# whatshap/whatshap

Hardware: AMD Instinct MI355X
Metric: variant-columns/sec at max-coverage 20 (bipartition-costs/sec reported alongside) (higher is better)
Workload: dtype u32; 1 GPU; synthetic diploid single-individual, max-coverage 20: 1 block of 200000 SNVs (BASELINE configs[2]); blocks=1, blocks_in_flight_per_gpu=1, tables_per_launch=1, max_coverage=20, optimal_cost_checksum=1611545, rendezvous=none

## Files before the change

include/whatshap_amd_debug.h:

```cpp
#ifndef WHATSHAP_AMD_DEBUG_H
#define WHATSHAP_AMD_DEBUG_H

#include "whatshap_amd.h"

#ifdef __cplusplus
extern "C" {
#endif

whamd_status_t whamd_debug_emulate_slot_plan(const whamd_readset_view* readset, const uint32_t* recombcost, size_t n_recombcost,
                                            const whamd_pedigree_view* pedigree, int distrust_genotypes,
                                            const uint32_t* positions, size_t n_positions, int slot_l, int symmetry,
                                            uint32_t* index_out, uint32_t* score_out, uint64_t* n_run_columns_out);

whamd_status_t whamd_debug_emulate_pedslot_plan(const whamd_readset_view* readset, const uint32_t* recombcost, size_t n_recombcost,
                                               const whamd_pedigree_view* pedigree, int distrust_genotypes,
                                               const uint32_t* positions, size_t n_positions, int slot_l,
                                               uint32_t* index_out, uint32_t* transmission_out, uint32_t* score_out,
                                               uint64_t* n_run_columns_out);

whamd_status_t whamd_debug_lazy_terms_check(const whamd_readset_view* readset, const uint32_t* recombcost, size_t n_recombcost,
                                            const whamd_pedigree_view* pedigree, int distrust_genotypes,
                                            const uint32_t* positions, size_t n_positions, const uint8_t* need, int rounds,
                                            int* lazy_out, uint64_t* differences_out, uint64_t* built_before_out, uint64_t* built_after_out);

whamd_status_t whamd_debug_pedmec_heuristic_create_host(const whamd_readset_view* readset, const uint32_t* recombcost, size_t n_recombcost,
                                                        const whamd_pedigree_view* pedigree, int distrust_genotypes,
                                                        const uint32_t* positions, size_t n_positions, uint32_t row_limit, int allow_mutations,
                                                        whamd_heuristic** out);

whamd_status_t whamd_debug_realign_detect_host(const whamd_realign_alignments_view* alignments, const whamd_realign_variants_view* variants,
                                               const whamd_realign_reference_view* reference, const whamd_realign_params* params,
                                               whamd_realign** out);
whamd_status_t whamd_debug_edit_distance_host(uint64_t n_pairs, const uint64_t* query_ptr, const uint8_t* query, const uint64_t* target_ptr,
                                              const uint8_t* target, int use_affine, const float* mismatch_cost, int32_t gap_start,
                                              int32_t gap_extend, int64_t* distance_out);

whamd_status_t whamd_debug_poly_score_host(const whamd_poly_matrix_view* matrices, uint64_t n_matrices, uint32_t min_overlap, uint32_t ploidy,
                                           double err, whamd_poly_scores** out);

whamd_status_t whamd_debug_progeny_score_host(const whamd_progeny_view* problems, uint64_t n_problems, whamd_progeny_scores** out);
whamd_status_t whamd_debug_progeny_score_entries_host(const whamd_progeny_view* problem, uint64_t n_entries, const uint32_t* i, const uint32_t* j,
                                                      double* score_out, uint8_t* stored_out);
whamd_status_t whamd_debug_progeny_pair_score_host(const float* gl, uint64_t n_positions, uint32_t n_samples, uint32_t ploidy, uint64_t pos1,
                                                   uint64_t pos2, uint32_t kind, double* score_out);
whamd_status_t whamd_debug_progeny_variant_types_host(const float* gl, uint64_t n_positions, uint32_t n_samples, uint32_t ploidy, const double* priors,
                                                      const uint32_t* nodes, uint64_t n_nodes, double* llh_out, uint32_t* g0_out, uint32_t* g1_out);
whamd_status_t whamd_debug_progeny_gl_host(const whamd_progeny_depths_view* problems, uint64_t n_problems, float* const* table_out,
                                           double* const* table_f64_out);

whamd_status_t whamd_debug_haplotag_host(const whamd_haplotag_view* problems, uint64_t n_problems, whamd_haplotag_result** out);

typedef struct whamd_debug_kernel {
	const void* kernel;
	const char* name;
	int32_t large_lds_opted_in;
	int32_t debug_only;
} whamd_debug_kernel;
size_t whamd_debug_solve_kernels(whamd_debug_kernel* out, size_t capacity);

enum {
	WHAMD_LAUNCH_COLUMN = 0,
	WHAMD_LAUNCH_RUN = 1,
	WHAMD_LAUNCH_SLOT_RUN = 2,
	WHAMD_LAUNCH_BATCH = 3,
	WHAMD_LAUNCH_GROUP = 4,
	WHAMD_LAUNCH_GROUP_WALK = 5,
	WHAMD_LAUNCH_TAIL = 6,
	WHAMD_LAUNCH_WINDOW_WALK = 7,
	WHAMD_LAUNCH_TABLES = 8
};

typedef struct whamd_debug_launch {
	const void* kernel;
	uint32_t site;
	uint32_t grid_x, grid_y, block;
	uint32_t lds;
	uint32_t own_stream;
	uint32_t forward;
	int32_t lr, yflags, spec, stamps, tb, nf, ncols, threads;
	int32_t streamed, pack;
	int32_t tight, variant;
	int32_t T, n_ind, mode, wide;
	int32_t ped, sym;
	int32_t entries;
	int32_t preview;
	int32_t reserved;
	uint64_t count;
	const char* name;
} whamd_debug_launch;
whamd_status_t whamd_debug_dptable_launches(const whamd_dptable* table, whamd_debug_launch* out, size_t capacity, size_t* n_out);

typedef struct whamd_debug_preview {
	int32_t ran, continued;
	uint32_t pieces, launched_steps, agreed_steps, reserved;
	const char* why_not;
} whamd_debug_preview;
whamd_status_t whamd_debug_dptable_preview(const whamd_dptable* table, whamd_debug_preview* out);

typedef struct whamd_debug_preview_plan_result {
	uint32_t n_pieces, pieces, steps, n_steps;
	int32_t chunked_predicted, chunked, windowed, reserved;
	uint32_t n_seeds_predicted, n_seeds, stride_predicted, stride;
	uint64_t arena_predicted, arena_laid_out, exchange_predicted, exchange_laid_out;
	const char* why_not;
} whamd_debug_preview_plan_result;
whamd_status_t whamd_debug_preview_plan(const whamd_readset_view* readset, const uint32_t* recombcost, size_t n_recombcost,
                                        const whamd_pedigree_view* pedigree, int distrust_genotypes,
                                        const uint32_t* positions, size_t n_positions, uint32_t pieces, whamd_debug_preview_plan_result* out,
                                        uint64_t* rec_predicted, uint64_t* rec_laid_out, uint32_t* spec_predicted, uint32_t* spec_laid_out, size_t capacity);

typedef struct whamd_debug_genotype_run {
	uint32_t c0, ncols;
	uint32_t rescale_f, rescale_b, emit_f, emit_b;
	uint32_t n_part_out, part_out_f, part_out_b;
	uint32_t part_in_f, n_part_in_f, part_in_b, n_part_in_b;
	uint32_t reserved;
} whamd_debug_genotype_run;
whamd_status_t whamd_debug_genotype_run_plan(const whamd_readset_view* readset, const uint32_t* recombcost, size_t n_recombcost,
                                             const whamd_pedigree_view* pedigree, const uint32_t* positions, size_t n_positions,
                                             whamd_debug_genotype_run* out, size_t capacity, size_t* n_out, double* min_total_out);

#ifdef __cplusplus
}
#endif

#endif
```

whatshap_amd/_native.py:

```python

from __future__ import annotations

import ctypes as C
import os
import threading
from typing import Optional, Sequence

import numpy as np

_HERE = os.path.dirname(os.path.abspath(__file__))
LIB_PATH = os.path.join(_HERE, "libwhatshap_amd.so")
DEBUG_LIB_PATH = os.path.join(_HERE, "libwhatshap_amd_debug.so")
ABI_VERSION = 2

WHAMD_OK = 0
WHAMD_ERR_INVALID = 1
WHAMD_ERR_MENDELIAN_CONFLICT = 2
WHAMD_ERR_UNSORTED = 3
WHAMD_ERR_UNSUPPORTED = 4
WHAMD_ERR_DEVICE = 5
WHAMD_ERR_OVERFLOW = 6
WHAMD_ERR_HOST = 7
GT_OTHER = 255

# ... 584 lines not shown
        else:
            _check(L.whamd_dptable_create(*problem.call_args(), C.c_int(device), C.byref(self._h)))
        self.n_columns = int(L.whamd_dptable_column_count(self._h))
        self.n_individuals = int(L.whamd_dptable_individual_count(self._h))
        self.n_reads = int(L.whamd_dptable_read_count(self._h))
        if solve:
            self.solve()

    def set_option(self, key: str, value: str):
        _check(self._L.whamd_dptable_set_option(self._h, key.encode(), value.encode()))

    def solve(self):
        _check(self._L.whamd_dptable_solve(self._h))

    def enqueue(self):
        _check(self._L.whamd_dptable_enqueue(self._h))

    def wait(self):
        _check(self._L.whamd_dptable_wait(self._h))

    def release_device(self):
        _check(self._L.whamd_dptable_release_device(self._h))

    def close(self):
        if getattr(self, "_h", None) is not None and self._h:
            self._L.whamd_dptable_destroy(self._h)
            self._h = C.c_void_p()

    def __del__(self):
        try:
            self.close()
        except Exception:
            pass

    def positions(self) -> np.ndarray:
        out = np.zeros(self.n_columns, dtype=np.uint32)
        _check(self._L.whamd_dptable_positions(self._h, _ptr(out, C.c_uint32)))
        return out

    def optimal_score(self) -> int:
        v = C.c_uint32()
        _check(self._L.whamd_dptable_get_optimal_score(self._h, C.byref(v)))
        return int(v.value)

    def super_reads(self):
        n, ni = self.n_columns, self.n_individuals
        a0 = np.zeros((ni, n), dtype=np.uint8)
        a1 = np.zeros((ni, n), dtype=np.uint8)
        q = np.zeros((ni, n), dtype=np.uint32)
        tv = np.zeros(n, dtype=np.uint32)
        sid = np.zeros(ni, dtype=np.uint32)
        _check(self._L.whamd_dptable_get_super_reads(
            self._h, _ptr(a0, C.c_uint8), _ptr(a1, C.c_uint8), _ptr(q, C.c_uint32), _ptr(tv, C.c_uint32), _ptr(sid, C.c_uint32)))
        return a0, a1, q, tv, sid

    def partitioning(self) -> np.ndarray:
        out = np.zeros(self.n_reads, dtype=np.uint8)
        _check(self._L.whamd_dptable_get_optimal_partitioning(self._h, _ptr(out, C.c_uint8)))
        return out

    def index_path(self):
        idx = np.zeros(self.n_columns, dtype=np.uint32)
        tv = np.zeros(self.n_columns, dtype=np.uint32)
        _check(self._L.whamd_dptable_get_index_path(self._h, _ptr(idx, C.c_uint32), _ptr(tv, C.c_uint32)))
        return idx, tv

    def stats(self) -> dict:
        s = SolveStats()
        _check(self._L.whamd_dptable_get_stats(self._h, C.byref(s)))
        return s.as_dict()


def plan_summary(problem: ProblemArrays, path: str = "auto") -> dict:
    out = PlanSummary()
    _check(lib().whamd_plan_summarize(*problem.call_args(), path.encode(), C.byref(out)))
    return out.as_dict()


def emulate_slot_plan(problem: ProblemArrays, n_columns: int, slot_l: int = 11, symmetry: int = 1, slot_r: int = 2):
    if slot_r >= 3:
        slot_l += 100
    elif slot_r <= 1:
        slot_l += 200
    idx = np.zeros(max(n_columns, 1), dtype=np.uint32)
    score = C.c_uint32()
    ncols = C.c_uint64()
    D = debug_lib()
    _check(D.whamd_debug_emulate_slot_plan(*problem.call_args(), C.c_int(slot_l), C.c_int(symmetry), _ptr(idx, C.c_uint32),
                                           C.byref(score), C.byref(ncols)), D)
    return idx[:n_columns], int(score.value), int(ncols.value)


def emulate_pedslot_plan(problem: ProblemArrays, n_columns: int, slot_l: int = 0):
    idx = np.zeros(max(n_columns, 1), dtype=np.uint32)
    trans = np.zeros(max(n_columns, 1), dtype=np.uint32)
    score = C.c_uint32()
    ncols = C.c_uint64()
    D = debug_lib()
    _check(D.whamd_debug_emulate_pedslot_plan(*problem.call_args(), C.c_int(slot_l), _ptr(idx, C.c_uint32), _ptr(trans, C.c_uint32),
                                              C.byref(score), C.byref(ncols)), D)
    return idx[:n_columns], trans[:n_columns], int(score.value), int(ncols.value)


def debug_lazy_terms_check(problem: ProblemArrays, need=None, rounds: int = 1) -> dict:
    D = debug_lib()
    fn = D.whamd_debug_lazy_terms_check
    fn.restype = C.c_int
    lazy, diff, before, after = C.c_int(), C.c_uint64(), C.c_uint64(), C.c_uint64()
    need_arr = None if need is None else np.ascontiguousarray(need, dtype=np.uint8)
    _check(fn(*problem.call_args(), None if need_arr is None else _ptr(need_arr, C.c_uint8), C.c_int(int(rounds)), C.byref(lazy), C.byref(diff),
              C.byref(before), C.byref(after)), D)
    return {"lazy": bool(lazy.value), "differences": int(diff.value), "built_before": int(before.value), "built_after": int(after.value)}


class DebugGenotypeRun(C.Structure):
    _fields_ = [(name, C.c_uint32) for name in ("c0", "ncols", "rescale_f", "rescale_b", "emit_f", "emit_b", "n_part_out", "part_out_f", "part_out_b",
                                                "part_in_f", "n_part_in_f", "part_in_b", "n_part_in_b", "reserved")]


def debug_genotype_run_plan(problem: ProblemArrays):
    D = debug_lib()
    fn = D.whamd_debug_genotype_run_plan
    fn.restype = C.c_int
    a = problem.call_args()
    args = (a[0], a[1], a[2], a[3], a[5], a[6])
    n, min_total = C.c_size_t(), C.c_double()
    status = fn(*args, None, C.c_size_t(0), C.byref(n), C.byref(min_total))
    if status == WHAMD_ERR_UNSUPPORTED:
        return None
    _check(status, D)
    runs = (DebugGenotypeRun * max(n.value, 1))()
    _check(fn(*args, runs, C.c_size_t(n.value), C.byref(n), C.byref(min_total)), D)
    names = [f[0] for f in DebugGenotypeRun._fields_ if f[0] != "reserved"]
    return [{k: int(getattr(runs[i], k)) for k in names} for i in range(n.value)], float(min_total.value)


class DebugKernel(C.Structure):
    _fields_ = [("kernel", C.c_void_p), ("name", C.c_char_p), ("large_lds_opted_in", C.c_int32), ("debug_only", C.c_int32)]


LAUNCH_SITES = ("column", "run", "slot_run", "batch", "group", "group_walk", "tail", "window_walk", "tables")
LAUNCH_FACTS = ("lr", "yflags", "spec", "stamps", "tb", "nf", "ncols", "threads", "streamed", "pack", "tight", "variant", "T", "n_ind", "mode", "wide",
                "ped", "sym", "entries")


class DebugLaunch(C.Structure):
    _fields_ = ([("kernel", C.c_void_p), ("site", C.c_uint32), ("grid_x", C.c_uint32), ("grid_y", C.c_uint32), ("block", C.c_uint32), ("lds", C.c_uint32),
                 ("own_stream", C.c_uint32), ("forward", C.c_uint32)] + [(f, C.c_int32) for f in LAUNCH_FACTS] +
                [("preview", C.c_int32), ("reserved", C.c_int32), ("count", C.c_uint64), ("name", C.c_char_p)])


class DebugPreview(C.Structure):
    _fields_ = [("ran", C.c_int32), ("continued", C.c_int32), ("pieces", C.c_uint32), ("launched_steps", C.c_uint32), ("agreed_steps", C.c_uint32),
                ("reserved", C.c_uint32), ("why_not", C.c_char_p)]


def debug_preview(table) -> dict:
    D = debug_lib()
    if table._L is not D:
        raise ValueError("the preview's record exists in the debug library only (use_debug_library() before the table is made)")
    out = DebugPreview()
    _check(D.whamd_debug_dptable_preview(table._h, C.byref(out)), D)
    return {"ran": bool(out.ran), "continued": bool(out.continued), "pieces": int(out.pieces), "launched_steps": int(out.launched_steps),
            "agreed_steps": int(out.agreed_steps), "why_not": (out.why_not or b"").decode()}


class DebugPreviewPlan(C.Structure):
    _fields_ = [("n_pieces", C.c_uint32), ("pieces", C.c_uint32), ("steps", C.c_uint32), ("n_steps", C.c_uint32),
                ("chunked_predicted", C.c_int32), ("chunked", C.c_int32), ("windowed", C.c_int32), ("reserved", C.c_int32),
                ("n_seeds_predicted", C.c_uint32), ("n_seeds", C.c_uint32), ("stride_predicted", C.c_uint32), ("stride", C.c_uint32),
                ("arena_predicted", C.c_uint64), ("arena_laid_out", C.c_uint64), ("exchange_predicted", C.c_uint64), ("exchange_laid_out", C.c_uint64),
                ("why_not", C.c_char_p)]


def debug_preview_plan(problem: ProblemArrays, pieces: int = 0) -> dict:
    D = debug_lib()
    fn = D.whamd_debug_preview_plan
    fn.restype = C.c_int
    out = DebugPreviewPlan()
    _check(fn(*problem.call_args(), C.c_uint32(pieces), C.byref(out), None, None, None, None, C.c_size_t(0)), D)
    n = int(out.steps)
    arrays = {"rec_predicted": np.zeros(max(n, 1), dtype=np.uint64), "rec_laid_out": np.zeros(max(n, 1), dtype=np.uint64),
              "spec_predicted": np.zeros(max(n, 1), dtype=np.uint32), "spec_laid_out": np.zeros(max(n, 1), dtype=np.uint32)}
    _check(fn(*problem.call_args(), C.c_uint32(pieces), C.byref(out), _ptr(arrays["rec_predicted"], C.c_uint64), _ptr(arrays["rec_laid_out"], C.c_uint64),
              _ptr(arrays["spec_predicted"], C.c_uint32), _ptr(arrays["spec_laid_out"], C.c_uint32), C.c_size_t(n)), D)
    rec = {name: (getattr(out, name).decode() if name == "why_not" else int(getattr(out, name))) for name, _ in DebugPreviewPlan._fields_ if name != "reserved"}
    rec.update({k: v[:n] for k, v in arrays.items()})
    return rec


def debug_solve_kernels() -> list:
    D = debug_lib()
    n = D.whamd_debug_solve_kernels(None, 0)
    arr = (DebugKernel * n)()
    D.whamd_debug_solve_kernels(arr, n)
    return [{"kernel": k.kernel, "name": k.name.decode(), "large_lds_opted_in": bool(k.large_lds_opted_in), "debug_only": bool(k.debug_only)} for k in arr]


def debug_launches(table) -> list:
    D = debug_lib()
    if table._L is not D:
        raise ValueError("the launch ledger exists in the debug library only (use_debug_library() before the table is made)")
    n = C.c_size_t()
    _check(D.whamd_debug_dptable_launches(table._h, None, 0, C.byref(n)), D)
    arr = (DebugLaunch * max(n.value, 1))()
    _check(D.whamd_debug_dptable_launches(table._h, arr, n.value, C.byref(n)), D)
    out = []
    for r in arr[:n.value]:
        if r.name is None:
            raise RuntimeError(f"a launch of site {LAUNCH_SITES[r.site]} (grid {r.grid_x} x {r.grid_y}, block {r.block}) took a kernel the registry does not list")
        rec = {"name": r.name.decode(), "site": LAUNCH_SITES[r.site], "grid_x": r.grid_x, "grid_y": r.grid_y, "block": r.block, "lds": r.lds,
               "own_stream": bool(r.own_stream), "forward": bool(r.forward), "count": int(r.count), "preview": bool(r.preview)}
        rec.update({f: (None if getattr(r, f) < 0 else getattr(r, f)) for f in LAUNCH_FACTS})
        out.append(rec)
    return out


def _heuristic_result(L, h) -> dict:
    n = int(L.whamd_pedmec_heuristic_column_count(h))
    ns = int(L.whamd_pedmec_heuristic_sample_count(h))
    nr = int(L.whamd_pedmec_heuristic_read_count(h))
    score = C.c_float()
    bip = np.zeros(max(nr, 1), dtype=np.uint8)
    trans = np.zeros(max(n, 1), dtype=np.uint32)
    haps = np.zeros((max(ns, 1), 2, max(n, 1)), dtype=np.int8)
    mut = np.zeros((max(ns, 1), 2, max(n, 1)), dtype=np.uint8)
    sid = np.zeros(max(ns, 1), dtype=np.uint32)
    pos = np.zeros(max(n, 1), dtype=np.uint32)
    _check(L.whamd_pedmec_heuristic_get(h, C.byref(score), _ptr(bip, C.c_uint8), _ptr(trans, C.c_uint32), haps.ctypes.data_as(C.POINTER(C.c_int8)),
                                        _ptr(mut, C.c_uint8), _ptr(sid, C.c_uint32), _ptr(pos, C.c_uint32)), L)
    stats = HeuristicStats()
    _check(L.whamd_pedmec_heuristic_get_stats(h, C.byref(stats)), L)
    return {"score": float(score.value), "bipartition": bip[:nr], "transmission": trans[:n], "haplotypes": haps[:ns, :, :n], "mutated": mut[:ns, :, :n],
            "sample_ids": sid[:ns], "positions": pos[:n], "stats": stats.as_dict()}


def pedmec_heuristic(problem: ProblemArrays, row_limit: int = 256, allow_mutations: bool = True, device: int = 0, host_diagnostic: bool = False) -> dict:
    L = debug_lib() if host_diagnostic else lib()
    h = C.c_void_p()
    a = problem.call_args()
    if host_diagnostic:
        _check(L.whamd_debug_pedmec_heuristic_create_host(*a, C.c_uint32(int(row_limit)), C.c_int(1 if allow_mutations else 0), C.byref(h)), L)
    else:
        _check(L.whamd_pedmec_heuristic_create(*a, C.c_uint32(int(row_limit)), C.c_int(1 if allow_mutations else 0), C.c_int(int(device)), C.byref(h)))
    try:
        return _heuristic_result(L, h)
    finally:
        L.whamd_pedmec_heuristic_destroy(h)


class HeuristicBatch:

    def __init__(self, problems, row_limit: int = 256, allow_mutations: bool = True, device: int = 0):
        L = lib()
        problems = list(problems)
        self._L = L
        self._n = len(problems)
        self._handles = (C.c_void_p * max(self._n, 1))()
        jobs = (HeuristicJob * max(self._n, 1))()
        for i, p in enumerate(problems):
            jobs[i].readset = C.pointer(p.readset_view)
            jobs[i].recombcost = _ptr(p.recombcost, C.c_uint32)
            jobs[i].n_recombcost = p.recombcost.size
            jobs[i].pedigree = C.pointer(p.pedigree_view)
            jobs[i].distrust_genotypes = 1 if p.distrust_genotypes else 0
            jobs[i].positions = _ptr(p.positions, C.c_uint32)
            jobs[i].n_positions = 0 if p.positions is None else p.positions.size
            jobs[i].row_limit = int(row_limit)
            jobs[i].allow_mutations = 1 if allow_mutations else 0
        if self._n:
            _check(L.whamd_pedmec_heuristic_enqueue_many(jobs, self._n, C.c_int(int(device)), self._handles))

    def results(self):
        out = []
        try:
            for i in range(self._n):
                _check(self._L.whamd_pedmec_heuristic_wait(self._handles[i]))
                out.append(_heuristic_result(self._L, self._handles[i]))
        finally:
            self.close()
        return out

    def close(self):
        for i in range(self._n):
            if self._handles[i]:
                self._L.whamd_pedmec_heuristic_destroy(self._handles[i])
                self._handles[i] = None
        self._n = 0

    def __del__(self):
        try:
            self.close()
        except Exception:
            pass


def pedmec_heuristic_many(problems, row_limit: int = 256, allow_mutations: bool = True, device: int = 0):
    return HeuristicBatch(problems, row_limit, allow_mutations, device).results()


def host_pool_idle_bytes() -> int:
    fn = lib().whamd_host_pool_idle_bytes
    fn.restype = C.c_uint64
    return int(fn())


def device_count() -> int:
    return int(lib().whamd_device_count())


def device_pci_bus_id(device: int) -> str:
    buf = C.create_string_buffer(64)
    fn = lib().whamd_device_pci_bus_id
    fn.restype = C.c_int
    fn.argtypes = [C.c_int, C.c_char_p, C.c_size_t]
    _check(fn(int(device), buf, 64))
    return buf.value.decode()
# ... 45 lines not shown
```

whatshap_amd/csrc/c_api.cpp:

```cpp
#include <cstdio>
#include <cstdlib>
#include <cstring>
#include <functional>
#include <memory>
#include <new>
#include <stdexcept>
#include <string>

#include "api_guard.h"
#include "debug_build.h"
#ifdef WHAMD_DEBUG_BUILD
#include "../../include/whatshap_amd_debug.h"
#endif
#include "device_runtime.h"
#include "device_table.h"
#include "genotype.h"
#include "genotype_plan.h"
#include "heuristic.h"
#include "host_parallel.h"
#include "problem.h"
#include "resident.h"
#include "slots.h"
#include <algorithm>
#include <vector>
// ... 608 lines not shown
			const uint32_t lmax = sg.kind == 1 ? (uint32_t)PED_LMAX : (uint32_t)RES_LMAX;
			ok = ok && rc.Lb <= lmax && rc.Lf <= lmax && rc.ebits <= (uint32_t)RES_EMAX;
			ok = ok && rc.stage_off == stage;
			stage += sg.kind == 1 ? (uint64_t)rc.nwords : (uint64_t)rc.ebits * rc.nwords;
			if (rc.mode == RES_MODE_FOLDED) { s.n_folded_columns++; ok = ok && i + 1 < sg.ncols && rc.ebits == 0; }
			if (rc.mode != RES_MODE_GENERIC) s.n_vectorised_columns++;
			if (rc.nfold) ok = ok && rc.nfold <= RES_MAXFOLD && i >= rc.nfold;
			ok = ok && c + 1 < p.n_cols;
		}
		ok = ok && stage == sg.stage_words;
		const uint64_t lds = sg.kind == 1
			? (((uint64_t)sg.ncols * (PED_LDSWORDS + PED_TABLE) + (uint64_t)sg.n_terms * 2 + 3) & ~3ull) * 4 + 2 * (16ull << sg.max_l) + (uint64_t)sg.stage_words * 8
			: (uint64_t)sg.ncols * (64 + RES_TABLE) * 4 + 2 * (4ull << sg.max_l) + (uint64_t)sg.stage_words * 8;
		ok = ok && lds <= 160 * 1024;
		s.max_lds_bytes = std::max<uint64_t>(s.max_lds_bytes, lds);
		s.max_run_columns = std::max<uint64_t>(s.max_run_columns, sg.ncols);
		s.max_workgroups = std::max<uint64_t>(s.max_workgroups, 1ull << (sg.g - sg.half));
		if (sg.half) s.n_halved_runs++;
		s.n_resident_columns += sg.ncols;
		s.backtrace_bytes += (uint64_t)sg.stage_words * (1ull << sg.g) * 8;
	}
	ok = ok && expect == p.n_cols;
	for (uint32_t c = 0; c < p.n_cols; ++c) ok = ok && seen[c] == 1;
	s.invariants_ok = ok ? 1 : 0;
	*out = s;
	return WHAMD_OK;
	});
}

#ifdef WHAMD_DEBUG_BUILD
whamd_status_t whamd_debug_emulate_slot_plan(const whamd_readset_view* readset, const uint32_t* recombcost, size_t n_recombcost,
                                            const whamd_pedigree_view* pedigree, int distrust_genotypes, const uint32_t* positions,
                                            size_t n_positions, int slot_l, int symmetry, uint32_t* index_out, uint32_t* score_out,
                                            uint64_t* n_run_columns_out) {
	return guarded([&]() -> whamd_status_t {
	const int lr = slot_l >= 200 ? 1 : slot_l >= 100 ? 3 : 2;
	if (slot_l >= 100) slot_l -= slot_l >= 200 ? 200 : 100;
	Problem p;
	std::string msg;
	whamd_status_t st = build_problem(readset, recombcost, n_recombcost, pedigree, distrust_genotypes != 0, positions,
	                                  n_positions, p, msg);
	if (st != WHAMD_OK) return fail(st, msg);
	SlotPlan sp;
	if (p.T != 1 || !plan_forward_slots(p, slot_l, symmetry, sp, lr)) return fail(WHAMD_ERR_UNSUPPORTED, "slot runs apply to a single individual only");
	std::vector<uint32_t> path;
	uint32_t score = 0;
	if (!emulate_slot_plan(p, sp, path, score, msg)) return fail(WHAMD_ERR_INVALID, "slot plan inconsistent: " + msg);
	if (index_out && !path.empty()) std::memcpy(index_out, path.data(), path.size() * sizeof(uint32_t));
	if (score_out) *score_out = score;
	if (n_run_columns_out) *n_run_columns_out = sp.n_run_columns;
	return WHAMD_OK;
	});
}

whamd_status_t whamd_debug_emulate_pedslot_plan(const whamd_readset_view* readset, const uint32_t* recombcost, size_t n_recombcost,
                                               const whamd_pedigree_view* pedigree, int distrust_genotypes, const uint32_t* positions,
                                               size_t n_positions, int slot_l, uint32_t* index_out, uint32_t* transmission_out,
                                               uint32_t* score_out, uint64_t* n_run_columns_out) {
	return guarded([&]() -> whamd_status_t {
	Problem p;
	std::string msg;
	whamd_status_t st = build_problem(readset, recombcost, n_recombcost, pedigree, distrust_genotypes != 0, positions,
	                                  n_positions, p, msg);
	if (st != WHAMD_OK) return fail(st, msg);
	SlotPlan sp;
	if (p.T == 1 || !plan_forward_slots(p, slot_l > 0 ? -slot_l : 0, 0, sp) || !sp.ped)
		return fail(WHAMD_ERR_UNSUPPORTED, "pedigree slot runs apply to tables with one or two trios whose columns need at most 4 cost forms per transmission value");
	std::vector<uint32_t> path, trans;
	uint32_t score = 0;
	if (!emulate_pedslot_plan(p, sp, path, trans, score, msg)) return fail(WHAMD_ERR_INVALID, "pedigree slot plan inconsistent: " + msg);
	if (index_out && !path.empty()) std::memcpy(index_out, path.data(), path.size() * sizeof(uint32_t));
	if (transmission_out && !trans.empty()) std::memcpy(transmission_out, trans.data(), trans.size() * sizeof(uint32_t));
	if (score_out) *score_out = score;
	if (n_run_columns_out) *n_run_columns_out = sp.n_run_columns;
	return WHAMD_OK;
	});
}
whamd_status_t whamd_debug_lazy_terms_check(const whamd_readset_view* readset, const uint32_t* recombcost, size_t n_recombcost,
                                            const whamd_pedigree_view* pedigree, int distrust_genotypes, const uint32_t* positions, size_t n_positions,
                                            const uint8_t* need_in, int rounds, int* lazy_out, uint64_t* differences_out, uint64_t* built_before_out,
                                            uint64_t* built_after_out) {
	return guarded([&]() -> whamd_status_t {
	Problem eager, lazy;
	std::string msg;
	whamd_status_t st = build_problem(readset, recombcost, n_recombcost, pedigree, distrust_genotypes != 0, positions, n_positions, eager, msg);
	if (st != WHAMD_OK) return fail(st, msg);
	st = build_problem(readset, recombcost, n_recombcost, pedigree, distrust_genotypes != 0, positions, n_positions, lazy, msg, false, true);
	if (st != WHAMD_OK) return fail(st, msg);
	if (lazy_out) *lazy_out = lazy.lazy_terms ? 1 : 0;
	const uint32_t n = eager.n_cols;
	uint64_t before = 0, after = 0, diff = 0;
	for (uint32_t c = 0; c < n; ++c) before += lazy.term_end(c, lazy.T - 1) > lazy.term_begin(c, 0);
	std::vector<uint8_t> need(n, 1);
	if (need_in) for (uint32_t c = 0; c < n; ++c) need[c] = need_in[c] != 0;
	rounds = std::max(1, rounds);
	for (int r = 0; r < rounds; ++r) {
		std::vector<uint8_t> part(n, 0);
		for (uint32_t c = 0; c < n; ++c) part[c] = need[c] && (int)(c % (uint32_t)rounds) == r;
		st = fill_lazy_terms(lazy, part, msg);
		if (st != WHAMD_OK) return fail(st, msg);
	}
	for (uint32_t c = 0; c < n; ++c) {
		after += lazy.term_end(c, lazy.T - 1) > lazy.term_begin(c, 0);
		if (!need[c]) continue;
		bool same = true;
		for (uint32_t t = 0; t < eager.T && same; ++t) {
			const uint64_t a0 = eager.term_begin(c, t), a1 = eager.term_end(c, t), b0 = lazy.term_begin(c, t), b1 = lazy.term_end(c, t);
			same = a1 - a0 == b1 - b0;
			for (uint64_t i = 0; same && i < a1 - a0; ++i)
				same = eager.terms[a0 + i].c == lazy.terms[b0 + i].c && eager.terms[a0 + i].plus == lazy.terms[b0 + i].plus && eager.terms[a0 + i].minus == lazy.terms[b0 + i].minus;
		}
		diff += !same;
	}
	if (eager.fterm_kind != lazy.fterm_kind || eager.fterms.size() != lazy.fterms.size()) diff += n;
	else for (size_t i = 0; i < eager.fterms.size(); ++i) if (eager.fterms[i].c != lazy.fterms[i].c || eager.fterms[i].plus != lazy.fterms[i].plus || eager.fterms[i].minus != lazy.fterms[i].minus) { ++diff; break; }
	if (lazy.value_bound < eager.value_bound) diff += n;
	if (differences_out) *differences_out = diff;
	if (built_before_out) *built_before_out = before;
	if (built_after_out) *built_after_out = after;
	return WHAMD_OK;
	});
}

size_t whamd_debug_solve_kernels(whamd_debug_kernel* out, size_t capacity) { return DeviceTable::debug_solve_kernels(out, capacity); }

whamd_status_t whamd_debug_dptable_launches(const whamd_dptable* table, whamd_debug_launch* out, size_t capacity, size_t* n_out) {
	if (!table || !n_out) return fail(WHAMD_ERR_INVALID, "null argument");
	if (!table->solved) return fail(WHAMD_ERR_INVALID, "the table has not been solved: its ledger is read after whamd_dptable_wait");
	*n_out = table->device.debug_launches(out, capacity);
	return WHAMD_OK;
}

whamd_status_t whamd_debug_dptable_preview(const whamd_dptable* table, whamd_debug_preview* out) {
	if (!table || !out) return fail(WHAMD_ERR_INVALID, "null argument");
	table->device.debug_preview(out);
	return WHAMD_OK;
}

whamd_status_t whamd_debug_preview_plan(const whamd_readset_view* readset, const uint32_t* recombcost, size_t n_recombcost,
                                        const whamd_pedigree_view* pedigree, int distrust_genotypes,
                                        const uint32_t* positions, size_t n_positions, uint32_t pieces, whamd_debug_preview_plan_result* out,
                                        uint64_t* rec_predicted, uint64_t* rec_laid_out, uint32_t* spec_predicted, uint32_t* spec_laid_out, size_t capacity) {
	return guarded([&]() -> whamd_status_t {
	if (!out) return fail(WHAMD_ERR_INVALID, "out is NULL");
	Problem p;
	std::string msg;
	whamd_status_t st = build_problem(readset, recombcost, n_recombcost, pedigree, distrust_genotypes != 0, positions, n_positions, p, msg);
	if (st != WHAMD_OK) return fail(st, msg);
	st = DeviceTable::debug_preview_plan(p, pieces, out, rec_predicted, rec_laid_out, spec_predicted, spec_laid_out, capacity, msg);
	return st == WHAMD_OK ? WHAMD_OK : fail(st, msg);
	});
}

whamd_status_t whamd_debug_genotype_run_plan(const whamd_readset_view* readset, const uint32_t* recombcost, size_t n_recombcost,
                                             const whamd_pedigree_view* pedigree, const uint32_t* positions, size_t n_positions,
                                             whamd_debug_genotype_run* out, size_t capacity, size_t* n_out, double* min_total_out) {
	return guarded([&]() -> whamd_status_t {
	if (!n_out) return fail(WHAMD_ERR_INVALID, "n_out is NULL");
	Problem p;
	std::string msg;
	whamd_status_t st = build_problem(readset, recombcost, n_recombcost, pedigree, false, positions, n_positions, p, msg, true);
	if (st != WHAMD_OK) return fail(st, msg);
	GenotypeModel model;
	st = build_genotype_model(p, model, msg);
	if (st != WHAMD_OK) return fail(st, msg);
	GenoRunPlan pl;
	if (!geno_plan_runs(p, model, 0, pl)) return fail(WHAMD_ERR_UNSUPPORTED, "the table is not eligible for the genotyper's run path");
	*n_out = pl.runs.size();
	if (min_total_out) *min_total_out = GS_MIN_TOTAL;
	for (size_t ri = 0; out && ri < pl.runs.size() && ri < capacity; ++ri) {
		const GsRun& r = pl.runs[ri];
		whamd_debug_genotype_run o{};
		o.c0 = r.c0; o.ncols = r.ncols;
		o.rescale_f = r.n_part_in_f ? 1u : 0u; o.rescale_b = r.n_part_in_b ? 1u : 0u;
		o.emit_f = r.emit_f; o.emit_b = r.emit_b;
		o.n_part_out = 1u << r.g;
		o.part_out_f = r.part_out_f; o.part_out_b = r.part_out_b;
		o.part_in_f = r.part_in_f; o.n_part_in_f = r.n_part_in_f;
		o.part_in_b = r.part_in_b; o.n_part_in_b = r.n_part_in_b;
		out[ri] = o;
	}
	return WHAMD_OK;
	});
}
#endif

}

struct whamd_heuristic;
struct HeuristicBatchState {
	whamd::HeurBatch batch;
	std::vector<whamd_heuristic*> members;
	bool collected = false;
	whamd_status_t status = WHAMD_OK;
	std::string message;
	double t_enqueued = 0.0;
};

struct whamd_heuristic {
	whamd::HeurPlan plan;
	whamd::HeurResult result;
	whamd_heuristic_stats stats{};
	std::shared_ptr<HeuristicBatchState> batch;
	bool finished = false;
};

namespace {
whamd_status_t heuristic_collect(whamd_heuristic* h) {
	if (h->finished) return WHAMD_OK;
	if (!h->batch) return fail(WHAMD_ERR_INVALID, "whamd_pedmec_heuristic_enqueue has not run");
	std::shared_ptr<HeuristicBatchState> st = h->batch;
	if (!st->collected) {
		st->collected = true;
		std::vector<whamd::HeurResult> results(st->members.size());
		st->status = st->batch.wait(results.data(), st->message);
		if (st->status == WHAMD_OK) {
			const double t_done = now_ms();
			whamd::parallel_ranges(st->members.size(), whamd::host_threads(st->members.size(), 1), [&](uint64_t i0, uint64_t i1, uint32_t) {
				for (uint64_t i = i0; i < i1; ++i) {
					whamd_heuristic* m = st->members[i];
					const double t0 = now_ms();
					m->result = std::move(results[i]);
					whamd::heuristic_finish(m->plan, m->result);
					m->stats.max_solutions = m->result.max_solutions;
					m->stats.total_solutions = m->result.total_solutions;
					m->stats.device_ms = m->result.device_ms;
					m->stats.host_prepare_ms += std::max(0.0, (t_done - st->t_enqueued) - m->result.device_ms);
					m->stats.host_finish_ms = now_ms() - t0;
				}
			});
		}
		for (whamd_heuristic* m : st->members) { m->finished = st->status == WHAMD_OK; m->batch.reset(); }
	}
	if (st->status != WHAMD_OK) return fail(st->status, st->message);
	return WHAMD_OK;
}

whamd_status_t heuristic_enqueue_jobs(const whamd_heuristic_job* jobs, size_t n_jobs, int device, whamd_heuristic** out) {
	if (!out || (!jobs && n_jobs)) return fail(WHAMD_ERR_INVALID, "null argument");
	for (size_t i = 0; i < n_jobs; ++i) out[i] = nullptr;
	std::vector<std::unique_ptr<whamd_heuristic>> hs(n_jobs);
	std::vector<whamd_status_t> status(n_jobs, WHAMD_OK);
	std::vector<std::string> messages(n_jobs);
	std::vector<double> prepare_ms(n_jobs, 0.0);
	whamd::parallel_ranges(n_jobs, whamd::host_threads(n_jobs, 1), [&](uint64_t i0, uint64_t i1, uint32_t) {
		for (uint64_t i = i0; i < i1; ++i) {
			const double t0 = now_ms();
			hs[i].reset(new whamd_heuristic());
			const whamd_heuristic_job& j = jobs[i];
			status[i] = whamd::build_heuristic_plan(j.readset, j.recombcost, j.n_recombcost, j.pedigree, j.distrust_genotypes != 0, j.positions, j.n_positions,
			                                        j.row_limit, j.allow_mutations != 0, hs[i]->plan, messages[i]);
			prepare_ms[i] = now_ms() - t0;
		}
	});
	for (size_t i = 0; i < n_jobs; ++i) if (status[i] != WHAMD_OK) return fail(status[i], messages[i]);
	std::shared_ptr<HeuristicBatchState> st(new HeuristicBatchState());
	std::vector<const whamd::HeurPlan*> plans(n_jobs);
	for (size_t i = 0; i < n_jobs; ++i) plans[i] = &hs[i]->plan;
	std::string msg;
	st->t_enqueued = now_ms();
	const whamd_status_t es = st->batch.enqueue(plans.data(), n_jobs, device, msg);
	if (es != WHAMD_OK) return fail(es, msg);
	for (size_t i = 0; i < n_jobs; ++i) {
		whamd_heuristic* h = hs[i].get();
		h->stats.n_columns = h->plan.n_cols; h->stats.n_reads = h->plan.n_reads; h->stats.n_samples = h->plan.n_samples; h->stats.row_limit = h->plan.row_limit;
		h->stats.host_prepare_ms = prepare_ms[i];
		h->batch = st;
		st->members.push_back(h);
	}
	for (size_t i = 0; i < n_jobs; ++i) out[i] = hs[i].release();
	return WHAMD_OK;
}

whamd_status_t heuristic_create_common(const whamd_readset_view* readset, const uint32_t* recombcost, size_t n_recombcost, const whamd_pedigree_view* pedigree,
                                       int distrust_genotypes, const uint32_t* positions, size_t n_positions, uint32_t row_limit, int allow_mutations,
                                       int device, bool on_host, whamd_heuristic** out) {
	if (!out) return fail(WHAMD_ERR_INVALID, "out is NULL");
	*out = nullptr;
	if (!on_host) {
		whamd_heuristic_job job{readset, recombcost, n_recombcost, pedigree, distrust_genotypes, positions, n_positions, row_limit, allow_mutations};
		whamd_heuristic* h = nullptr;
		whamd_status_t st = heuristic_enqueue_jobs(&job, 1, device, &h);
		if (st != WHAMD_OK) return st;
		st = heuristic_collect(h);
		if (st != WHAMD_OK) { delete h; return st; }
		*out = h;
		return WHAMD_OK;
	}
#ifndef WHAMD_DEBUG_BUILD
	return fail(WHAMD_ERR_DEVICE, "the host instantiation of the heuristic exists in the debug library only");
#else
	const double t0 = now_ms();
	std::unique_ptr<whamd_heuristic> h(new whamd_heuristic());
	std::string msg;
	whamd_status_t st = whamd::build_heuristic_plan(readset, recombcost, n_recombcost, pedigree, distrust_genotypes != 0, positions, n_positions, row_limit,
	                                                allow_mutations != 0, h->plan, msg);
	if (st != WHAMD_OK) return fail(st, msg);
	const double t1 = now_ms();
	st = whamd::heuristic_solve_host(h->plan, h->result, msg);
	if (st != WHAMD_OK) return fail(st, msg);
	const double t2 = now_ms();
	whamd::heuristic_finish(h->plan, h->result);
	h->stats.n_columns = h->plan.n_cols; h->stats.n_reads = h->plan.n_reads; h->stats.max_solutions = h->result.max_solutions;
	h->stats.total_solutions = h->result.total_solutions; h->stats.device_ms = h->result.device_ms;
	h->stats.host_prepare_ms = (t1 - t0) + ((t2 - t1) - h->result.device_ms); h->stats.host_finish_ms = now_ms() - t2;
	h->stats.n_samples = h->plan.n_samples; h->stats.row_limit = h->plan.row_limit;
// ... 119 lines not shown
```

whatshap_amd/csrc/dp_device.hip:

```cpp
#include <hip/hip_runtime.h>

#include <algorithm>
#include <atomic>
#include <cctype>
#include <chrono>
#include <cstdio>
#include <cstdlib>
#include <cstring>
#include <mutex>
#include <string>
#include <vector>

#include "debug_build.h"
#ifdef WHAMD_DEBUG_BUILD
#include "../../include/whatshap_amd_debug.h"
#endif
#include "device_runtime.h"
#include "device_table.h"
#include "genotype.h"

namespace whamd {

namespace {

#include "kernels_column.h"
#include "kernels_resident.h"
#include "kernels_trio.h"
#include "kernels_slots.h"
#include "kernels_pedslots.h"
#include "kernels_backtrace.h"

using FusedFn = void (*)(DevProblem, uint32_t, const uint32_t*, uint32_t*);
using KeysFn = void (*)(DevProblem, uint32_t, const uint32_t*, uint32_t);

template <int T, int NIND>
void pick(FusedFn& ff, KeysFn& kf) {
	ff = column_step_fused<T, NIND>;
	kf = column_step_keys<T, NIND>;
}

bool select_kernels(uint32_t T, uint32_t n_ind, FusedFn& ff, KeysFn& kf) {
	const uint32_t ni = n_ind ? n_ind : 1;
	ff = nullptr;
	kf = nullptr;
#define WHAMD_CASE(TT, NN) if (T == TT && ni == NN) { pick<TT, NN>(ff, kf); return true; }
	WHAMD_CASE(1, 1) WHAMD_CASE(1, 2) WHAMD_CASE(1, 3) WHAMD_CASE(1, 4) WHAMD_CASE(1, 5) WHAMD_CASE(1, 6)
	WHAMD_CASE(4, 3) WHAMD_CASE(4, 4) WHAMD_CASE(4, 5) WHAMD_CASE(4, 6)
	WHAMD_CASE(16, 4) WHAMD_CASE(16, 5) WHAMD_CASE(16, 6)
#undef WHAMD_CASE
	return false;
}

using SegmentFn = void (*)(DevProblem, ResSegment, const uint32_t*, uint32_t*, uint32_t*);
using PedSegmentFn = void (*)(DevProblem, ResSegment, const uint32_t*, uint32_t*);
using ResBatchFn = void (*)(DevProblem, const ResBatchEntry*);
using SlotRunFn = void (*)(DevProblem, SlotRun, const uint32_t*, uint32_t*, uint32_t*);
using SlotRunXFn = void (*)(DevProblem, SlotRun, const uint32_t*, uint32_t*, uint32_t*, uint32_t);
using PedSlotRunFn = void (*)(DevProblem, SlotRun, PedSlotExtra, const uint32_t*, uint32_t*);
using SlotBatchFn = void (*)(DevProblem, const SlotBatchEntry*);
using GroupFn = void (*)(SlotGroupArgs);

enum GroupVariant : uint8_t { GV_SINGLE4 = 0, GV_PED_2_2, GV_PED_2_4, GV_PED_4_2, GV_PED_4_4, GV_PED_2_16, GV_SINGLE8, GV_TRIO_FACT, GV_X4, GV_X8, GV_QUARTET_FACT, GROUP_VARIANTS };
struct GroupVariantPair { GroupVariant plain, x; };

GroupVariantPair group_variants_of(const SlotBatchEntry& he, bool ped) {
	if (ped) {
		const GroupVariant v = he.ex.nf == (uint32_t)PSLOT_FACT4 ? GV_QUARTET_FACT : he.ex.nf == (uint32_t)PSLOT_FACT ? GV_TRIO_FACT : he.ex.nf == 16 ? GV_PED_2_16
		                       : he.ex.tb == 4 ? (he.ex.nf == 4 ? GV_PED_4_4 : GV_PED_4_2) : (he.ex.nf == 4 ? GV_PED_2_4 : GV_PED_2_2);
		return {v, v};
	}
	const GroupVariant v = he.run.lr == 3 ? GV_SINGLE8 : GV_SINGLE4;
	return {v, (he.run.yflags & 8u) ? (he.run.lr == 3 ? GV_X8 : GV_X4) : v};
}

}


namespace {

struct CreateLaps {
	using Clock = std::chrono::steady_clock;
	const bool on = getenv("WHAMD_DEBUG_TIMING") != nullptr;
	Clock::time_point last = Clock::now();
	double stage_ms[4] = {0.0, 0.0, 0.0, 0.0};
	int stage = 0;
	double take() {
		const auto now = Clock::now();
		const double ms = std::chrono::duration<double, std::milli>(now - last).count();
		last = now;
		stage_ms[stage] += ms;
		return ms;
	}
	void lap(const char* what) {
		if (on) fprintf(stderr, "[whamd timing]   upload: %s %.2f ms\n", what, take());
	}
	void next_stage() {
		if (!on) return;
		take();
		if (stage < 3) ++stage;
	}
	void summary(double arena_gb) {
		if (!on) return;
		take();
		fprintf(stderr, "[whamd timing] upload: plan %.1f ms, descriptors + copies %.1f ms, backtrace arena (%.2f GB) %.1f ms, rest %.1f ms\n", stage_ms[0], stage_ms[1], arena_gb, stage_ms[2],
		        stage_ms[3]);
	}
};

struct TableUploader {
	const int device;
	const hipStream_t stream;
	StageSession stage;
	std::vector<std::pair<void*, size_t>>& allocations;
	char* d_slab = nullptr;
	size_t slab_cap = 0, slab_used = 0, slab_flushed = 0;
	bool unstaged_copies = false;

	TableUploader(int dev, hipStream_t us, std::vector<std::pair<void*, size_t>>& table_allocations) : device(dev), stream(us), stage(us), allocations(table_allocations) {}

	hipError_t alloc(void** dptr, size_t bytes) {
		size_t got = 0;
		hipError_t e = devpool_take(device, std::max<size_t>(bytes, 16), dptr, &got);
		if (e == hipSuccess) allocations.emplace_back(*dptr, got);
		return e;
	}
	void open_block(size_t upload_bytes) {
		stage.expect(upload_bytes);
		if (upload_bytes <= STAGE_MAX && !debug_env("WHAMD_NO_UPLOAD_SLAB") && stage.begin_image(upload_bytes)) {
			void* ptr = nullptr;
			if (alloc(&ptr, upload_bytes) == hipSuccess) { d_slab = (char*)ptr; slab_cap = upload_bytes; }
			else { (void)hipGetLastError(); stage.image = false; }
		}
	}
	hipError_t flush() {
		if (!d_slab || slab_used == slab_flushed) return hipSuccess;
		const hipError_t e = debug_env("WHAMD_SKIP_SLAB_COPY") ? hipSuccess : hipMemcpyAsync(d_slab + slab_flushed, stage.base + slab_flushed, slab_used - slab_flushed, hipMemcpyHostToDevice, stream);
		stage.pending = true;
		slab_flushed = slab_used;
		return e;
	}
	hipError_t up(void** dptr, const void* src, size_t bytes) {
		const size_t padded = (bytes + 255) & ~(size_t)255;
		if (d_slab && slab_used + padded <= slab_cap) {
			*dptr = d_slab + slab_used;
			char* at = stage.base + slab_used;
			const char* from = (const char*)src;
			if (bytes >= ((size_t)4 << 20)) parallel_ranges(bytes, host_threads(bytes, (size_t)2 << 20), [at, from](uint64_t b0, uint64_t b1, uint32_t) { std::memcpy(at + b0, from + b0, b1 - b0); });
			else if (bytes) std::memcpy(at, from, bytes);
			slab_used += padded;
			stage.total += padded;
			return slab_used - slab_flushed >= ((size_t)32 << 20) ? flush() : hipSuccess;
		}
		hipError_t e = alloc(dptr, bytes);
		if (e != hipSuccess) return e;
		if (bytes) e = stage.copy(*dptr, src, bytes);
		if (bytes && stage.image) unstaged_copies = true;
		return e;
	}
	hipError_t up_pieces(void** dptr, const void* src, size_t bytes, const std::vector<std::pair<size_t, size_t>>& pieces) {
		const size_t padded = (bytes + 255) & ~(size_t)255;
		const bool in_slab = d_slab && slab_used + padded <= slab_cap;
		if (in_slab) {
			hipError_t e = flush();
			if (e != hipSuccess) return e;
			*dptr = d_slab + slab_used;
			slab_used += padded;
			slab_flushed = slab_used;
		} else {
			hipError_t e = alloc(dptr, bytes);
			if (e != hipSuccess) return e;
		}
		const size_t image_at = slab_used - padded;
		for (const auto& pc : pieces) {
			if (pc.second <= pc.first) continue;
			const char* from = (const char*)src + pc.first;
			if (in_slab) {
				std::memcpy(stage.base + image_at + pc.first, from, pc.second - pc.first);
				from = stage.base + image_at + pc.first;
				stage.pending = true;
			} else {
				unstaged_copies = true;
			}
			hipError_t e = hipMemcpyAsync((char*)*dptr + pc.first, from, pc.second - pc.first, hipMemcpyHostToDevice, stream);
			if (e != hipSuccess) return e;
		}
		return hipSuccess;
	}
};

struct TableBuild {
	CreateLaps laps;
	uint32_t n = 0;
	uint32_t tbits = 0;
	uint32_t ni = 1;
	size_t free_b = 0;
	uint64_t arena_cap = 0;
	uint64_t bt = 0;
	uint32_t max_f = 0, max_keys_f = 0;
	size_t exchange_bytes = 0;
	bool force_keys = false;
	bool ped_slots = false;
	std::vector<uint32_t> segs;
	RawVec<uint32_t> term_ptr32;
	std::vector<uint32_t> window_first_col;
	RawVec<uint32_t> slot_blob;
	std::vector<uint32_t> slot_blob_off, slot_blob_words;
	std::vector<int32_t> delta_fallback;
	const SlotRun* d_runs = nullptr;
	const PedSlotExtra* d_pextra = nullptr;
	const DevTerm* d_fterms = nullptr;
};

}


#ifdef WHAMD_DEBUG_BUILD
struct LaunchFacts : whamd_debug_launch {
	LaunchFacts() {
		std::memset(static_cast<whamd_debug_launch*>(this), 0, sizeof(whamd_debug_launch));
		lr = yflags = spec = stamps = tb = nf = ncols = threads = streamed = pack = tight = variant = T = n_ind = mode = wide = ped = sym = entries = -1;
	}
	static LaunchFacts of_run(const SlotRun& run, bool spec_v, bool stamps_v) {
		LaunchFacts f;
		f.lr = (int32_t)run.lr; f.yflags = (int32_t)run.yflags; f.ncols = (int32_t)run.ncols; f.threads = (int32_t)run.threads;
		f.spec = spec_v; f.stamps = stamps_v;
		return f;
	}
};
#define WHAMD_NOTE(table, ...) (table).note(__VA_ARGS__)
#else
#define WHAMD_NOTE(table, ...) ((void)0)
#endif

struct DeviceTable::Impl {
	int device = 0;
	hipStream_t stream = nullptr;
	hipEvent_t ev0 = nullptr, ev1 = nullptr, ev2 = nullptr, ev3 = nullptr;
	hipEvent_t ev_group = nullptr;
	hipEvent_t ev_upload = nullptr;
	std::vector<std::pair<void*, size_t>> allocations;
	void* d_arena = nullptr;
	size_t arena_bytes = 0;
	DevColumn* d_cols = nullptr;
	uint32_t* d_pr[2] = {nullptr, nullptr};
	uint32_t* d_path_index = nullptr;
	uint32_t* d_path_trans = nullptr;
	uint32_t* d_score = nullptr;
	BtUnit* d_units = nullptr;
	std::vector<BtUnit> units;
	size_t bt_lds = 0;
	RawVec<DevColumn> cols;
	ResidentPlan plan;
	DevProblem dp{};
	FusedFn fused = nullptr;
	KeysFn keysfn = nullptr;
	bool wide = false;
	size_t key_entries = 0;
	std::string path = "auto";
	int l_pref = 11;
	bool fold = true;
	int symmetry = 1;
	uint64_t bt_bytes = 0;
	uint32_t max_grid_x = 1;
	size_t h_pinned_bytes = 0;
	uint32_t* h_pinned = nullptr;
	struct Job {
		std::vector<uint32_t> steps;
		uint32_t unit_off = 0, unit_count = 0;
		bool final = false;
	};
	struct Lane {
		uint32_t* d_pr[2] = {nullptr, nullptr};
		unsigned long long* d_keys = nullptr;
		std::vector<uint32_t> jobs;
	};
	struct Single {
		uint32_t lane, step, flip;
		bool zero_prev;
		int32_t score_job;
	};
	struct SuperStep {
		uint32_t entry_off = 0, entry_count = 0, grid_x = 0, threads = 0;
		size_t lds = 0;
		bool sym = false;
		std::vector<Single> singles;
		int32_t ck_load = -1, ck_save = -1, bt_window = -1;
		uint32_t* io[2] = {nullptr, nullptr};
	};
	std::vector<Job> jobs;
	std::vector<Lane> lanes;
	std::vector<SuperStep> schedule;
	struct StepBrief { uint32_t entry_off, lds; uint16_t entry_count; uint8_t has_singles, pad; };
	struct EntryBrief { uint16_t grid_x, threads; uint32_t lds_x; GroupVariantPair variant; uint8_t pad[2]; };
	std::vector<StepBrief> step_brief;
	std::vector<EntryBrief> entry_brief;
	std::vector<ResBatchEntry> entries;
	ResBatchEntry* d_entries = nullptr;
	bool use_chunks = false;
	std::vector<BtChunk> chunks;
	BtChunk* d_chunks = nullptr;
	uint32_t* d_unit_x = nullptr;
	uint32_t* d_path2 = nullptr;
	uint32_t* d_trans2 = nullptr;
	uint32_t n_orient_max = 1;
	uint8_t* d_sel = nullptr;
	uint32_t* d_guess = nullptr;
	uint32_t* d_bt_counters = nullptr;
	uint32_t n_spec = 0;
	size_t chunk_lds = 0;
	SlotPlan splan;
	bool use_slots = false;
	int slot_l = 11;
	bool slot_l_set = false;
	int slot_lr = 2;
	int slot_lr_used = 2;
	std::vector<SlotBatchEntry> slot_entries;
	SlotBatchEntry* d_slot_entries = nullptr;
	uint64_t table_bytes = 0;
	BtJob* d_btjobs = nullptr;
	uint32_t* d_job_scores = nullptr;
	bool shared_hint = false;
	bool side_by_side = false;
	int max_lanes = 32;
	struct Window {
		uint32_t step_lo = 0, step_hi = 0;
		uint32_t unit_off = 0, unit_count = 0;
	};
	uint64_t arena_limit = 0;
	bool windowed = false;
	std::vector<Window> windows;
	uint8_t* d_checkpoints = nullptr;
	size_t checkpoint_bytes = 0;
	uint32_t* d_bt_state = nullptr;
	BtJob* d_window_jobs = nullptr;

	whamd_status_t open(int dev, std::string& msg);
	whamd_status_t choose_plan(Problem& p, TableBuild& b, std::string& msg);
	void dump_plan(const Problem& p) const;
	whamd_status_t describe_columns(const Problem& p, TableBuild& b, std::string& msg);
	whamd_status_t lay_out_arena(const Problem& p, TableBuild& b, std::string& msg);
	size_t upload_bound(const Problem& p, const TableBuild& b) const;
	whamd_status_t upload_column_arrays(const Problem& p, TableBuild& b, TableUploader& up, std::string& msg);
	void build_slot_blobs(TableBuild& b) const;
	uint64_t lay_out_slot_tables(const TableBuild& b, bool report = true);
	whamd_status_t upload_slot_arrays(TableBuild& b, TableUploader& up, std::string& msg);
	void make_jobs();
	void make_units(const TableBuild& b);
	whamd_status_t make_windows(const TableBuild& b, TableUploader& up, std::string& msg);
	whamd_status_t take_result_block(uint32_t n, TableUploader& up, std::string& msg);
	void cut_chunks(const Problem& p);
	whamd_status_t make_chunks(const Problem& p, TableUploader& up, std::string& msg);
	whamd_status_t take_solve_buffers(const Problem& p, TableBuild& b, TableUploader& up, std::string& msg);
	whamd_status_t make_lanes(const TableBuild& b, TableUploader& up, std::string& msg);
	whamd_status_t make_schedule(const TableBuild& b, std::string& msg);
	void make_briefs();
	whamd_status_t upload_entries(TableUploader& up, std::string& msg);
	whamd_status_t launch_table_kernels(const Problem& p, const TableBuild& b, TableUploader& up, std::string& msg);
	whamd_status_t arm_debug_stamps(TableUploader& up, std::string& msg);
	whamd_status_t record_group_backtrace(uint32_t n, TableUploader& up, std::string& msg);
	struct SolveInFlight {
		hipStream_t run_stream = nullptr;
		uint32_t group_tables = 1;
		bool enqueue_open = false;
		size_t next_super = 0;
		uint64_t launches = 0;
		hipStream_t tail_stream = nullptr;
		uint64_t tail_seq = 0;
		bool tail_elsewhere = false;
		bool timing_pending = false;
		static inline std::atomic<uint64_t> tails_submitted{0};
		void rewind(hipStream_t own) { enqueue_open = false; next_super = 0; run_stream = own; }
	} inflight;
#ifdef WHAMD_DEBUG_BUILD
	std::vector<whamd_debug_launch> ledger;
	void note(uint32_t site, const void* kernel, dim3 grid, dim3 block, size_t lds, hipStream_t on, bool forward, const LaunchFacts& facts);
#endif
	struct GroupSubmission;
	void launch_column_step(const Problem& p, const Step& step, const Lane& lane, const uint32_t* prev, uint32_t* cur, uint64_t& launches);
	void launch_run(const ResBatchEntry& e, uint64_t& launches);
	void launch_slot_run(const DevProblem& dp, const SlotBatchEntry& e, uint64_t& launches);
	whamd_status_t begin_solve(const Problem& p, Solution& s, std::string& msg, bool behind_preview = false);
	whamd_status_t submit_super_step(const Problem& p, const SuperStep& ss, uint64_t& launches, std::string& msg);
	whamd_status_t submit_singles(const Problem& p, const SuperStep& ss, uint64_t& launches, std::string& msg);
	whamd_status_t submit_tail(const Problem& p, std::string& msg, hipStream_t tail_stream = nullptr, bool walked_by_group = false);
	whamd_status_t report_slot_stamps(std::string& msg) const;
	whamd_status_t report_resident_stamps(std::string& msg) const;
	BtGroupEntry h_bt_entry{};
	BtGroupEntry* d_bt_entry = nullptr;
	bool device_superreads = false;
	SuperreadArgs super_args{};
	size_t super_words = 0, super_off = 0;
	bool own_stream_used = false;
	bool upload_pending = false;
	hipStream_t upload_stream = nullptr;

	enum PreviewWhy : uint32_t { PV_RAN = 0, PV_OFF, PV_NOT_CREATE, PV_NOT_SLOTS, PV_DEBUG_SWITCH, PV_SHARED, PV_THREAD_BUDGET, PV_COMPONENTS, PV_FEW_PIECES, PV_NOT_ALONE, PV_NO_LEADING_RUNS,
	                           PV_ROW_PAD, PV_ARENA, PV_WHYS };
	struct Preview {
		int mode = -1;
		uint32_t pieces_wanted = 0;
		bool thread_budget = false;
		bool counted = false;
		uint32_t why = PV_NOT_CREATE;
		uint32_t pieces = 0;
		uint32_t launched = 0;
		uint32_t agreed = 0;
		bool launching = false;
		bool pending = false;
		bool continued = false;
		bool use_chunks = false;
		uint64_t launches = 0;
		std::vector<SlotRun> runs;
		DevProblem dp{};
		uint32_t* d_pr[2] = {nullptr, nullptr};
		size_t exchange_bytes = 0;
		unsigned long long* spec_keys = nullptr;
		size_t spec_bytes = 0;
		std::vector<std::pair<void*, size_t>> allocations;
	} preview;
	static inline std::atomic<int> tables_on_device[64];
	void give_preview_block() {
		for (auto& a : preview.allocations) devpool_give(device, a.first, a.second);
		preview.allocations.clear();
	}
	struct PreviewPlan {
		uint32_t why = PV_NOT_CREATE, pieces = 0, steps = 0, end_col = 0, n_spec = 0, stride = 64, max_f = 0;
		bool chunked = false;
		uint64_t arena = 0, tab_words = 0;
		size_t ctrl_words = 0;
		std::vector<uint64_t> rec;
		std::vector<uint32_t> spec;
	};
	void plan_preview(const Problem& p, const TableBuild& b, bool from_create, PreviewPlan& out);
	whamd_status_t start_preview(const Problem& p, TableBuild& b, bool from_create, std::string& msg);
	void verify_preview();
	whamd_status_t arm_keys(std::string& msg);

	void adopt(const StreamSet& ss) { stream = ss.stream; ev0 = ss.ev[0]; ev1 = ss.ev[1]; ev2 = ss.ev[2]; ev3 = ss.ev[3]; ev_group = ss.ev[4]; ev_upload = ss.ev[5]; }
	StreamSet stream_set() const {
		StreamSet ss;
		ss.stream = stream; ss.ev[0] = ev0; ss.ev[1] = ev1; ss.ev[2] = ev2; ss.ev[3] = ev3; ss.ev[4] = ev_group; ss.ev[5] = ev_upload; ss.device = device;
		return ss;
	}

	void release_lanes() {
		max_grid_x = 1;
		lanes.clear();
		jobs.clear();
		schedule.clear();
		entries.clear();
		slot_entries.clear();
		windows.clear();
	}

	void release() {
		if (inflight.tail_elsewhere && ev3) (void)hipEventSynchronize(ev3);
		inflight.tail_elsewhere = false;
		if (upload_pending && ev_upload) (void)hipEventSynchronize(ev_upload);
		upload_pending = false;
		release_lanes();
		windowed = false;
		if (stream && own_stream_used && (!allocations.empty() || d_arena)) { (void)hipStreamSynchronize(stream); own_stream_used = false; }
		for (auto& a : allocations) devpool_give(device, a.first, a.second);
		allocations.clear();
		give_preview_block();
		if (preview.why != PV_NOT_CREATE) {
			Preview fresh;
			fresh.mode = preview.mode; fresh.pieces_wanted = preview.pieces_wanted; fresh.thread_budget = preview.thread_budget; fresh.counted = preview.counted;
			preview = std::move(fresh);
		}
		arena_give(device, d_arena, arena_bytes);
		d_arena = nullptr;
		arena_bytes = 0;
		pinned_give(h_pinned, h_pinned_bytes);
		h_pinned = nullptr;
		d_cols = nullptr;
		d_units = nullptr;
		d_pr[0] = d_pr[1] = nullptr;
		d_path_index = d_path_trans = d_score = nullptr;
	}
};

DeviceTable::DeviceTable() : impl_(new Impl()) {}

DeviceTable::~DeviceTable() {
	if (impl_) {
		release_device();
		delete impl_;
	}
}

void DeviceTable::release_device() {
	Impl& m = *impl_;
	(void)hipSetDevice(m.device);
	m.release();
	if (m.stream) {
		if (m.own_stream_used) (void)hipStreamSynchronize(m.stream);
		m.own_stream_used = false;
		streamset_give(m.stream_set());
	}
	m.adopt(StreamSet());
	if (m.preview.counted && m.device >= 0 && m.device < 64) Impl::tables_on_device[m.device].fetch_sub(1);
	m.preview.counted = false;
	m.inflight.run_stream = nullptr;
	m.inflight.timing_pending = false;
}

int DeviceTable::device_count() {
	int n = 0;
	if (hipGetDeviceCount(&n) != hipSuccess) return 0;
	return n;
}

bool DeviceTable::device_pci_bus_id(int device, std::string& out) {
	int n = 0;
	if (hipGetDeviceCount(&n) != hipSuccess || device < 0 || device >= n) return false;
	char text[64] = {0};
	if (hipDeviceGetPCIBusId(text, (int)sizeof text - 1, device) != hipSuccess) return false;
	out = text;
	for (char& ch : out) ch = (char)tolower((unsigned char)ch);
	return true;
}

static void append_segments(uint32_t mask, std::vector<uint32_t>& out, uint16_t& count) {
	uint32_t src = 0;
	count = 0;
	for (uint32_t bit = 0; bit < 32;) {
		if (!((mask >> bit) & 1u)) { ++bit; continue; }
		uint32_t len = 0;
		while (bit + len < 32 && ((mask >> (bit + len)) & 1u)) ++len;
		out.push_back(src | (bit << 8) | (len << 16));
		++count;
		src += len;
		bit += len;
	}
}

bool DeviceTable::set_path(const std::string& path) {
	if (path != "auto" && path != "column" && path != "column_keys" && path != "resident" && path != "slots") return false;
	impl_->path = path;
	return true;
}

void DeviceTable::set_l_pref(int l) { impl_->l_pref = std::max(4, std::min(l, RES_LMAX)); }
void DeviceTable::set_lanes(int n) { impl_->max_lanes = n < 1 ? 1 : (n > 64 ? 64 : n); }

void DeviceTable::set_fold(bool v) { impl_->fold = v; }
void DeviceTable::set_slot_l(int l) { impl_->slot_l = std::max(2, std::min(l, 12)); impl_->slot_l_set = true; }
void DeviceTable::set_slot_lr(int lr) { impl_->slot_lr = lr >= 3 ? 3 : (lr <= 1 ? 1 : 2); }

void DeviceTable::set_arena_limit(uint64_t bytes) { impl_->arena_limit = bytes; }
void DeviceTable::set_shared_launches(bool v) { impl_->shared_hint = v; }
void DeviceTable::set_side_by_side(bool v) { impl_->side_by_side = v; }
void DeviceTable::set_preview(int mode) { impl_->preview.mode = mode < 0 ? -1 : (mode ? 1 : 0); }
void DeviceTable::set_preview_pieces(uint32_t pieces) { impl_->preview.pieces_wanted = pieces; }
void DeviceTable::set_thread_budget(bool v) { impl_->preview.thread_budget = v; }
void DeviceTable::set_symmetry(int level) { impl_->symmetry = level < 0 ? 0 : (level > 2 ? 2 : level); }


whamd_status_t DeviceTable::Impl::open(int dev, std::string& msg) {
	Impl& m = *this;
	m.device = dev;
	const whamd_status_t opened = open_device(dev, msg);
	if (opened != WHAMD_OK) return opened;
	if (!m.stream) {
		StreamSet ss;
		if (!streamset_take(dev, ss)) { msg = "could not create the table's stream and events"; return WHAMD_ERR_DEVICE; }
		m.adopt(ss);
	}
	m.release();
	if (!m.preview.counted && dev >= 0 && dev < 64) { Impl::tables_on_device[dev].fetch_add(1); m.preview.counted = true; }
	return WHAMD_OK;
}

whamd_status_t DeviceTable::Impl::choose_plan(Problem& p, TableBuild& b, std::string& msg) {
	Impl& m = *this;
	m.wide = !select_kernels(p.T, p.n_ind, m.fused, m.keysfn);
	if (m.wide && (p.T > (uint32_t)MAX_T_WIDE || p.n_ind > (uint32_t)MAX_IND_WIDE)) {
		msg = "no device kernel for T=" + std::to_string(p.T) + ", individuals=" + std::to_string(p.n_ind);
		return WHAMD_ERR_UNSUPPORTED;
	}
	for (uint32_t c = 0; c < p.n_cols && !m.wide; ++c) m.wide = p.term_end(c, p.T - 1) - p.term_begin(c, 0) > (uint64_t)COL_MAXTERMS;
	b.force_keys = m.path == "column_keys" || m.wide;
	const bool want_resident = (m.path == "auto" || m.path == "resident") && !m.wide;
	size_t free_b = 0, total_b = 0;
	HIP_TRY(hipMemGetInfo(&free_b, &total_b));
	if (free_b < total_b / 2) {
		genotype_release_cache();
		HIP_TRY(hipMemGetInfo(&free_b, &total_b));
	}
	if (free_b < total_b / 4) {
		arena_release();
		devpool_release();
		HIP_TRY(hipMemGetInfo(&free_b, &total_b));
	}
	free_b += arena_idle_bytes(m.device);
	b.free_b = free_b;
	int slot_lr = m.slot_lr, slot_l = m.slot_l;
	if (m.shared_hint && p.T == 1 && p.max_k >= 18 && !m.slot_l_set && m.slot_lr == 2) { slot_lr = 3; slot_l = 12; }
	if (p.T == 1 && p.max_k >= 21 && p.max_k <= 22 && !m.slot_l_set && m.slot_lr == 2 && !debug_env("WHAMD_NO_WIDE_LAYOUT")) { slot_lr = 3; slot_l = 12; }
	m.slot_lr_used = slot_lr;
	m.use_slots = (m.path == "auto" || m.path == "slots") && !m.wide && plan_forward_slots(p, p.T > 1 ? (m.slot_l_set ? -m.slot_l : 0) : std::max(8, slot_l), m.symmetry, m.splan, slot_lr);
	if (m.use_slots && m.splan.ped && m.splan.table_words * 4ull > free_b / 4) m.use_slots = false;
	m.table_bytes = m.use_slots && m.splan.ped ? m.splan.table_words * 4ull : 0ull;
	if (p.lazy_terms) {
		std::vector<uint8_t> need(p.n_cols, 1);
		if (m.use_slots && m.splan.ped) for (uint32_t c = 0; c < p.n_cols; ++c) need[c] = m.splan.col_to_row[c] < 0;
		const whamd_status_t st = fill_lazy_terms(p, need, msg);
		if (st != WHAMD_OK) return st;
	}
	if (m.use_slots) {
		m.plan = ResidentPlan();
		m.plan.steps = m.splan.steps;
		m.plan.component_first_step = m.splan.component_first_step;
		m.plan.col_to_res.assign(p.n_cols, -1);
	} else {
		m.splan = SlotPlan();
		plan_forward(p, want_resident, m.l_pref, m.fold, m.plan, m.symmetry);
	}
	m.device_superreads = p.n_ind == 1 && p.T == 1 && p.P == 2 && !p.distrust && p.h2p.size() >= 2 && p.h2p[0] == 0 && p.h2p[1] == 1 && p.genotype.size() >= p.n_cols &&
	                      !debug_env("WHAMD_HOST_SUPERREADS");
	return WHAMD_OK;
}

void DeviceTable::Impl::dump_plan(const Problem& p) const {
	const Impl& m = *this;
	for (const Step& st : m.plan.steps) {
		if (st.kind == 0) { fprintf(stderr, "[plan] column %u k=%u b=%u f=%u\n", st.index, p.k[st.index], p.b[st.index], p.f[st.index]); continue; }
		if (st.kind == 2) {
			const SlotRun& r = m.splan.runs[st.index];
			fprintf(stderr, "[plan] slot run c0=%u ncols=%u g=%u L=%u half=%u ends=%u has_prev=%u in_identity=%u in_half=%u mirror_pos=%u in_occ=%x out_occ=%x mirror_out=%u\n",
			        r.c0, r.ncols, r.g, r.L, r.half, r.n_ends, r.has_prev, r.in_identity, r.in_half, r.in_mirror_pos, r.in_occ, r.out_occ, r.mirror_out);
			if (m.splan.ped) fprintf(stderr, "[plan]   pedigree run: T=%u forms per value=%u table words=%u record words per workgroup=%u\n", 1u << m.splan.pextra[st.index].tb,
			                         m.splan.pextra[st.index].nf, m.splan.pextra[st.index].s_off + r.ncols * 64u * pslot_ns(m.splan.pextra[st.index].nf), m.splan.pextra[st.index].rec_words);
			continue;
		}
		const ResSegment& sgm = m.plan.segments[st.index];
		fprintf(stderr, "[plan] run c0=%u ncols=%u g=%u threads=%u max_l=%u stage_words=%u\n", sgm.c0, sgm.ncols, sgm.g, sgm.threads, sgm.max_l, sgm.stage_words);
		for (uint32_t i = 0; i < sgm.ncols; ++i) {
			const ResColumn& rc = m.plan.columns[sgm.col_off + i];
			const ResBacktrace& rb = m.plan.backtrace[sgm.col_off + i];
			fprintf(stderr, "[plan]   col %u mode=%u nfold=%u Lb=%u Lf=%u ebits=%u epos0=%u nthr=%u stage_off=%u nwords=%u | bt layout=%u n_g=%u n_l=%u\n",
			        sgm.c0 + i, rc.mode, rc.nfold, rc.Lb, rc.Lf, rc.ebits, rc.epos[0], rc.nthr, rc.stage_off, rc.nwords, rb.layout, rb.n_g, rb.n_l);
		}
	}
}

whamd_status_t DeviceTable::Impl::describe_columns(const Problem& p, TableBuild& b, std::string& msg) {
	Impl& m = *this;
	const uint32_t n = b.n, ni = b.ni, tbits = b.tbits;
	if (p.terms.size() >= 0xFFFFFFFFull || (uint64_t)p.col_ptr[n] * ni >= 0xFFFFFFFFull) {
		msg = "problem too large for 32-bit device offsets";
		return WHAMD_ERR_UNSUPPORTED;
	}
	m.cols.resize(n);
	b.term_ptr32.resize((size_t)n * (p.T + 1));
	RawVec<uint32_t>& term_ptr32 = b.term_ptr32;
	parallel_ranges(n, host_threads(n, 16384), [&m, &p, &term_ptr32, n, ni, tbits](uint64_t c0, uint64_t c1, uint32_t) {
		for (uint32_t c = (uint32_t)c0; c < (uint32_t)c1; ++c) {
			DevColumn d{};
			d.k = p.k[c];
			d.b = p.b[c];
			d.f = p.f[c];
			d.recomb = p.recomb[c];
			d.delta_off = (uint32_t)(p.col_ptr[c] * ni);
			d.term_off = (uint32_t)((size_t)c * (p.T + 1));
			for (uint32_t t = 0; t <= p.T; ++t) term_ptr32[(size_t)c * (p.T + 1) + t] = (uint32_t)p.term_ptr[(size_t)c * p.T + t];
			d.ebits = d.k - d.f;
			d.is_last = (c + 1 == n);
			d.eloop = std::min<uint32_t>(d.ebits, QMAX);
			d.nplanes = d.ebits + tbits;
			m.cols[c] = d;
		}
	});
	return WHAMD_OK;
}

static uint32_t column_step_mode(bool force_keys, bool is_last, uint32_t f, uint32_t ebits) { return (!force_keys && !is_last && f >= 6 && ebits <= (uint32_t)QMAX) ? 0u : 1u; }
static uint64_t column_record_bytes(uint32_t mode, uint32_t T, uint32_t f, uint32_t nplanes) {
	return mode == 0 ? (uint64_t)nplanes * T * (1ull << (f - 6)) * 8ull : (uint64_t)T * (1ull << f) * 4ull;
}
static uint64_t arena_capacity(uint64_t free_b, uint32_t n, uint64_t table_bytes, uint64_t arena_limit) {
	const uint64_t reserve = (3ull << 30) + (uint64_t)n * 1024ull + table_bytes;
	uint64_t cap = free_b > reserve ? free_b - reserve : 0;
	if (arena_limit) cap = std::min<uint64_t>(cap, arena_limit);
	return cap;
}
static uint64_t arena_behind(uint64_t bt, uint64_t bytes) { return (bt + bytes + 15ull) & ~15ull; }
static uint64_t slot_run_record_bytes(const SlotRun& run) { return (uint64_t)run.n_ends * run.threads * (1ull << (run.g - run.half)); }

whamd_status_t DeviceTable::Impl::lay_out_arena(const Problem& p, TableBuild& b, std::string& msg) {
	Impl& m = *this;
	const uint32_t n = b.n;
	const bool ped_slots = b.ped_slots;
	std::vector<uint32_t>& segs = b.segs;
	uint64_t bt = 0, seg_bt = 0;
	size_t seg_cursor = 0, slot_cursor = 0;
	uint32_t max_f = 0, max_keys_f = 0;
	auto slot_record_bytes = [&m, ped_slots](size_t ri) -> uint64_t {
		const SlotRun& run = m.splan.runs[ri];
		if (ped_slots) return (uint64_t)m.splan.pextra[ri].rec_words * 4ull << run.g;
		return slot_run_record_bytes(run);
	};
	const uint64_t arena_cap = arena_capacity(b.free_b, n, m.table_bytes, m.arena_limit);
	b.arena_cap = arena_cap;
	std::vector<uint32_t>& window_first_col = b.window_first_col;
	uint64_t bt_max = 0;
	auto open_unit = [&bt, &bt_max, &window_first_col, arena_cap](uint32_t c, uint64_t bytes) -> bool {
		if (bytes + 16 > arena_cap) return false;
		if (bt + bytes + 16 > arena_cap) {
			bt_max = std::max(bt_max, bt);
			bt = 0;
			window_first_col.push_back(c);
		}
		return true;
	};
	auto unit_too_large = [&msg, &b](uint32_t c) {
		msg = "the backtrace record of the unit at column " + std::to_string(c) + " alone does not fit in the arena (" + std::to_string(b.arena_cap >> 20) +
		      " MiB of " + std::to_string(b.free_b >> 20) + " MiB free HBM)";
		return WHAMD_ERR_UNSUPPORTED;
	};
	for (uint32_t c = 0; c < n; ++c) {
		DevColumn& d = m.cols[c];
		const bool in_slot_run = m.use_slots && m.splan.col_to_row[c] >= 0;
		d.seg_off = (uint32_t)segs.size();
		const uint32_t kmask = d.k >= 32 ? 0xFFFFFFFFu : ((1u << d.k) - 1u);
		if (!in_slot_run) {
			append_segments(p.fwd_mask[c], segs, d.nseg_fwd);
			append_segments(kmask & ~p.fwd_mask[c], segs, d.nseg_end);
		}
		d.bt_off = bt;
		if (m.use_slots && m.splan.col_to_row[c] >= 0) {
			d.mode = 3;
			d.res_idx = (uint32_t)m.splan.col_to_row[c];
			if (slot_cursor < m.splan.runs.size() && m.splan.runs[slot_cursor].c0 == c) {
				SlotRun& run = m.splan.runs[slot_cursor];
				if (!open_unit(c, slot_record_bytes(slot_cursor))) return unit_too_large(c);
				run.rec_lo = (uint32_t)bt;
				run.rec_hi = (uint32_t)(bt >> 32);
				seg_bt = bt;
				bt += slot_record_bytes(slot_cursor);
				max_f = std::max(max_f, run.L + run.g);
				++slot_cursor;
			}
			d.bt_off = seg_bt;
		} else if (m.plan.col_to_res[c] >= 0) {
			d.mode = 2;
			d.res_idx = (uint32_t)m.plan.col_to_res[c];
			if (seg_cursor < m.plan.segments.size() && m.plan.segments[seg_cursor].c0 == c) {
				ResSegment& sgm = m.plan.segments[seg_cursor];
				if (!open_unit(c, (uint64_t)sgm.stage_words * (1ull << sgm.g) * 8ull)) return unit_too_large(c);
				sgm.bt_lo = (uint32_t)bt;
				sgm.bt_hi = (uint32_t)(bt >> 32);
				seg_bt = bt;
				bt += (uint64_t)sgm.stage_words * (1ull << sgm.g) * 8ull;
				++seg_cursor;
			}
			d.bt_off = seg_bt;
		} else {
			d.mode = column_step_mode(b.force_keys, d.is_last, d.f, d.ebits);
			const uint64_t bytes = column_record_bytes(d.mode, p.T, d.f, d.nplanes);
			if (!open_unit(c, bytes)) return unit_too_large(c);
			d.bt_off = bt;
			bt += bytes;
			if (d.mode != 0) max_keys_f = std::max(max_keys_f, d.f);
		}
		bt = (bt + 15ull) & ~15ull;
		max_f = std::max(max_f, d.f);
	}
	b.laps.lap("column descriptors (host)");
	bt = std::max(bt_max, bt);
	b.bt = bt;
	b.max_f = max_f;
	b.max_keys_f = max_keys_f;
// ... 612 lines not shown

whamd_status_t DeviceTable::Impl::upload_entries(TableUploader& up, std::string& msg) {
	Impl& m = *this;
	HIP_TRY(up.up((void**)&m.d_entries, m.entries.data(), m.entries.size() * sizeof(ResBatchEntry)));
	m.slot_entries.resize(m.slot_entries.size() + 2);
	HIP_TRY(up.up((void**)&m.d_slot_entries, m.slot_entries.data(), m.slot_entries.size() * sizeof(SlotBatchEntry)));
	m.slot_entries.resize(m.slot_entries.size() - 2);
	std::vector<BtJob> btjobs;
	for (const Impl::Job& job : m.jobs) btjobs.push_back(BtJob{job.unit_off, job.unit_count, job.final ? 1u : 0u, 0u});
	HIP_TRY(up.up((void**)&m.d_btjobs, btjobs.data(), btjobs.size() * sizeof(BtJob)));
	return WHAMD_OK;
}

whamd_status_t DeviceTable::Impl::launch_table_kernels(const Problem& p, const TableBuild& b, TableUploader& up, std::string& msg) {
	Impl& m = *this;
	const hipStream_t us = up.stream;
	HIP_TRY(up.flush());
	if (b.ped_slots) {
		uint32_t most = 0;
		for (size_t ri = 0; ri < m.splan.runs.size(); ++ri)
			most = std::max<uint32_t>(most, (m.splan.pextra[ri].fwn << m.splan.runs[ri].g) + (m.splan.pextra[ri].fwn << m.splan.runs[ri].lw) + m.splan.runs[ri].ncols * (64u * pslot_ns(m.splan.pextra[ri].nf) + p.T * pslot_nk(m.splan.pextra[ri].nf)));
		const uint32_t bx = std::max(1u, std::min(1024u, (most + 255u) / 256u));
		for (size_t r0 = 0; r0 < m.splan.runs.size(); r0 += 32768) {
			const uint32_t ny = (uint32_t)std::min<size_t>(32768, m.splan.runs.size() - r0);
			hipLaunchKernelGGL(pedslot_tables, dim3(bx, ny), dim3(256), 0, us, m.dp, b.d_runs + r0, b.d_pextra + r0, (uint32_t*)m.dp.pslot_tab, b.d_fterms);
		}
		HIP_TRY(hipGetLastError());
	}
	if (m.use_slots && !b.ped_slots && !m.splan.runs.empty()) {
		uint32_t most = 0;
		for (const SlotRun& run : m.splan.runs) most = std::max<uint32_t>(most, ((run.ncols + 8u) << (run.g - run.half)) + (run.ncols + 8u) * ((run.threads >> 6) + 64u));
		const uint32_t bx = std::max(1u, std::min(64u, (most + 255u) / 256u));
		for (size_t r0 = 0; r0 < m.splan.runs.size(); r0 += 32768) {
			const uint32_t ny = (uint32_t)std::min<size_t>(32768, m.splan.runs.size() - r0);
			hipLaunchKernelGGL(slot_tables, dim3(bx, ny), dim3(256), 0, us, m.dp, b.d_runs + r0, (uint32_t*)m.dp.slot_tab);
		}
		HIP_TRY(hipGetLastError());
	}
	HIP_TRY(hipEventRecord(m.ev_upload, us));
	m.upload_pending = true;
	if (debug_env("WHAMD_SYNC_UPLOAD") || up.unstaged_copies || !up.stage.image || !up.stage.park()) {
		HIP_TRY(hipStreamSynchronize(us));
		up.stage.finish();
	}
	return WHAMD_OK;
}

whamd_status_t DeviceTable::Impl::arm_debug_stamps(TableUploader& up, std::string& msg) {
	Impl& m = *this;
	m.dp.dbg = nullptr;
	if (debug_env("WHAMD_DEBUG_STAMPS") && !m.use_slots) {
		const size_t dbg_bytes = (m.plan.segments.size() + 1) * 64 + 4 * 512 * 16 + 64;
		HIP_TRY(up.alloc((void**)&m.dp.dbg, dbg_bytes));
		HIP_TRY(hipMemset(m.dp.dbg, 0, dbg_bytes));
		m.dp.dbg_wg_off = (uint32_t)((m.plan.segments.size() + 1) * 8);
		m.dp.dbg_flags = (uint32_t)atoi(debug_env("WHAMD_DEBUG_STAMPS"));
	}
	if (debug_env("WHAMD_SLOT_STAMPS") && m.use_slots) {
		const size_t dbg_bytes = (m.splan.runs.size() + 1) * 48 * 8 + 4 * 512 * 16 + 128;
		HIP_TRY(up.alloc((void**)&m.dp.dbg, dbg_bytes));
		HIP_TRY(hipMemset(m.dp.dbg, 0, dbg_bytes));
		m.dp.dbg_wg_off = (uint32_t)((m.splan.runs.size() + 1) * 48);
		for (size_t i = 0; i < m.slot_entries.size(); ++i) m.slot_entries[i].run.pad = (uint32_t)i;
	}
	if (const char* skip = debug_env("WHAMD_SLOT_SKIP")) m.dp.dbg_flags = (uint32_t)atoi(skip);
	return WHAMD_OK;
}

static const void* const* large_lds_kernels(size_t& count) {
#define K(...) reinterpret_cast<const void*>((__VA_ARGS__))
#define WHAMD_RUNX(XC, STAMPS) K(slot_runx<2, XC, STAMPS, false>), K(slot_runx<2, XC, STAMPS, true>)
#define WHAMD_PSLOT(TBV, NFV) K(pedslot_run<TBV, NFV, false, false>), K(pedslot_run<TBV, NFV, false, true>), K(pedslot_run<TBV, NFV, true, false>), K(pedslot_run<TBV, NFV, true, true>)
#define WHAMD_PSLOTX(TBV, NFV) K(pedslot_runx<TBV, NFV, 32, false>), K(pedslot_runx<TBV, NFV, 32, true>)
	static const void* const kernels[] = {
		K(resident_segment<false, false>), K(resident_segment<false, true>),
#ifdef WHAMD_DEBUG_BUILD
		K(resident_segment<true, true>),
#endif
		K(resident_batch<false>), K(resident_batch<true>), K(backtrace_kernel), K(resident_segment_ped<false>),
#ifdef WHAMD_DEBUG_BUILD
		K(resident_segment_ped<true>),
#endif
		K(resident_segment_ped<false, true>),
		WHAMD_RUNX(24, false), WHAMD_RUNX(32, false), WHAMD_RUNX(0, false), WHAMD_RUNX(8, false), WHAMD_RUNX(16, false),
		K(slot_groupx<2, false>), K(slot_groupx<3, false>),
#ifdef WHAMD_DEBUG_BUILD
		WHAMD_RUNX(24, true), WHAMD_RUNX(32, true),
		WHAMD_PSLOTX(2, 2), WHAMD_PSLOTX(2, 4), WHAMD_PSLOTX(4, 2), WHAMD_PSLOTX(4, 4), WHAMD_PSLOTX(2, 16), WHAMD_PSLOTX(2, PSLOT_FACT),
#endif
		WHAMD_PSLOT(2, 4), WHAMD_PSLOT(4, 2), WHAMD_PSLOT(4, 4),
		WHAMD_PSLOT(2, 16), K(pedslot_group<2, 16>),
		WHAMD_PSLOT(2, PSLOT_FACT), K(pedslot_group<2, PSLOT_FACT>),
		WHAMD_PSLOT(4, PSLOT_FACT4), K(pedslot_group<4, PSLOT_FACT4>),
		K(pedslot_group<2, 2>), K(pedslot_group<2, 4>), K(pedslot_group<4, 2>), K(pedslot_group<4, 4>),
	};
#undef K
#undef WHAMD_RUNX
#undef WHAMD_PSLOT
#undef WHAMD_PSLOTX
	count = sizeof(kernels) / sizeof(kernels[0]);
	return kernels;
}

static whamd_status_t opt_in_large_lds(int device, std::string& msg) {
	static std::mutex attr_mu;
	static unsigned long long attr_done = 0;
	std::lock_guard<std::mutex> lock(attr_mu);
	if (device < 64 && ((attr_done >> device) & 1ull)) return WHAMD_OK;
	size_t count = 0;
	const void* const* kernels = large_lds_kernels(count);
	for (size_t i = 0; i < count; ++i) HIP_TRY(hipFuncSetAttribute(kernels[i], hipFuncAttributeMaxDynamicSharedMemorySize, 160 * 1024));
	if (device < 64) attr_done |= 1ull << device;
	return WHAMD_OK;
}

whamd_status_t DeviceTable::Impl::record_group_backtrace(uint32_t n, TableUploader& up, std::string& msg) {
	Impl& m = *this;
	m.d_bt_entry = nullptr;
	if (!m.use_chunks) return WHAMD_OK;
	BtGroupEntry& e = m.h_bt_entry;
	e = BtGroupEntry{};
	e.P = m.dp;
	e.units = m.d_units; e.chunks = m.d_chunks;
	e.n_chunks = (uint32_t)m.chunks.size(); e.n_units = (uint32_t)m.units.size(); e.n_orient_max = m.n_orient_max; e.n_cols = n;
	e.path2 = m.d_path2; e.trans2 = m.d_trans2; e.out_score = m.d_score; e.unit_x2 = m.d_unit_x; e.guess = m.d_guess; e.sel = m.d_sel; e.counters = m.d_bt_counters;
	e.path_index = m.d_path_index; e.path_trans = m.d_path_trans;
	if (m.device_superreads) e.super = m.super_args;
	void* d_entry = nullptr;
	HIP_TRY(up.alloc(&d_entry, sizeof(BtGroupEntry)));
	HIP_TRY(hipMemcpyAsync(d_entry, &m.h_bt_entry, sizeof(BtGroupEntry), hipMemcpyHostToDevice, up.stream));
	HIP_TRY(hipEventRecord(m.ev_upload, up.stream));
	m.d_bt_entry = (BtGroupEntry*)d_entry;
	return WHAMD_OK;
}

void DeviceTable::Impl::plan_preview(const Problem& p, const TableBuild& b, bool from_create, PreviewPlan& out) {
	Impl& m = *this;
	const Preview& pv = m.preview;
	const uint32_t n = b.n, n_pieces = slot_plan_pieces(n);
	out = PreviewPlan();
	auto none = [&out](uint32_t why) { out.why = why; };
	if (pv.mode == 0 || debug_env("WHAMD_NO_PREVIEW")) return none(PV_OFF);
	if (!from_create) return none(PV_NOT_CREATE);
	if (!m.use_slots || m.splan.ped || p.T != 1) return none(PV_NOT_SLOTS);
	if (debug_env("WHAMD_DEBUG_STAMPS") || debug_env("WHAMD_SLOT_STAMPS") || debug_env("WHAMD_SLOT_SKIP")) return none(PV_DEBUG_SWITCH);
	if (m.shared_hint || m.side_by_side) return none(PV_SHARED);
	if (m.plan.component_first_step.size() != 1) return none(PV_COMPONENTS);
	if (n_pieces < 2) return none(PV_FEW_PIECES);
	if (pv.mode < 0) {
		if (pv.thread_budget) return none(PV_THREAD_BUDGET);
		if (n_pieces < 8) return none(PV_FEW_PIECES);
		if (m.device < 0 || m.device >= 64 || Impl::tables_on_device[m.device].load() != 1) return none(PV_NOT_ALONE);
	}
	out.pieces = std::min(n_pieces - 1, pv.pieces_wanted ? pv.pieces_wanted : std::max(1u, n_pieces / 6));
	const uint32_t col_limit = slot_plan_piece_begin(n, out.pieces);
	const std::vector<Step>& steps = m.plan.steps;
	const std::vector<SlotRun>& runs = m.splan.runs;
	uint32_t S = 0;
	while (S < steps.size() && steps[S].kind == 2 && steps[S].index == S && runs[S].c0 + runs[S].ncols <= col_limit) ++S;
	if (S == 0 || S >= steps.size()) return none(PV_NO_LEADING_RUNS);
	out.end_col = runs[S - 1].c0 + runs[S - 1].ncols;
	if ((size_t)out.end_col + SLOT_ROW_PAD > m.splan.rows.size()) return none(PV_ROW_PAD);
	const uint64_t tab_words_all = m.lay_out_slot_tables(b, false);
	out.tab_words = (S < runs.size() ? runs[S].tab_g : tab_words_all) + (uint64_t)SLOT_XCOLS * 64u;
	out.ctrl_words = (size_t)runs[S - 1].ctrl_off + SLOT_CTRL_WORDS;
	if (tab_words_all >= 0xFFFFFFFFull || out.ctrl_words > m.splan.ctrl.size()) return none(PV_NO_LEADING_RUNS);
	out.rec.assign(S, 0);
	uint64_t bt = 0;
	{
		const uint64_t cap = arena_capacity(b.free_b, n, m.table_bytes, m.arena_limit);
		for (size_t k = 0; k < steps.size(); ++k) {
			uint64_t bytes = 0;
			if (steps[k].kind == 2) bytes = slot_run_record_bytes(runs[steps[k].index]);
			else {
				const uint32_t c = steps[k].index, f = p.f[c], ebits = p.k[c] - f;
				bytes = column_record_bytes(column_step_mode(b.force_keys, c + 1 == n, f, ebits), p.T, f, ebits + b.tbits);
			}
			if (bt + bytes + 16 > cap) return none(PV_ARENA);
			if (k < S) out.rec[k] = bt;
			bt = arena_behind(bt, bytes);
		}
		if (bt + (1ull << 31) > b.free_b) return none(PV_ARENA);
	}
	out.arena = bt;
	out.spec.assign(S, 0);
	out.stride = 64;
	out.chunked = backtrace_is_chunked(true, 1, false, steps.size());
	if (out.chunked)
		out.n_spec = cut_chunk_starts(steps.size(), [&steps](size_t u) { return steps[steps.size() - 1 - u].kind == 2; },
			[&](size_t u, uint32_t id) {
				const size_t k = steps.size() - 1 - u;
				out.stride = seed_stride_of(out.stride, runs[steps[k].index]);
				if (k < S) out.spec[k] = id;
			});
	out.max_f = p.max_k;
	for (const SlotRun& run : runs) out.max_f = std::max(out.max_f, run.L + run.g);
	out.steps = S;
	out.why = PV_RAN;
}

whamd_status_t DeviceTable::Impl::start_preview(const Problem& p, TableBuild& b, bool from_create, std::string& msg) {
	Impl& m = *this;
	Preview& pv = m.preview;
	PreviewPlan pp;
	m.plan_preview(p, b, from_create, pp);
	pv.why = pp.why;
	if (pp.why != PV_RAN) return WHAMD_OK;
	const uint32_t n = b.n, S = pp.steps, pieces = pp.pieces, end_col = pp.end_col, n_spec = pp.n_spec, stride = pp.stride, max_f = pp.max_f;
	const uint64_t bt = pp.arena, tab_words = pp.tab_words;
	const size_t ctrl_words = pp.ctrl_words;
	const bool chunked = pp.chunked;
	const std::vector<uint64_t>& rec = pp.rec;
	const std::vector<uint32_t>& spec = pp.spec;
	const std::vector<SlotRun>& runs = m.splan.runs;
	b.laps.lap("preview: steps, offsets, seeds (host)");
	auto take = [&m](void** out, size_t bytes) {
		size_t got = 0;
		const hipError_t e = devpool_take(m.device, std::max<size_t>(bytes, 16), out, &got);
		if (e == hipSuccess) m.allocations.emplace_back(*out, got);
		return e;
	};
	{
		size_t got = 0;
		void* d_bt = arena_take(m.device, bt, got);
		if (!d_bt) {
			HIP_TRY(hipMalloc(&d_bt, std::max<size_t>(bt, 16)));
			got = std::max<size_t>(bt, 16);
		}
		m.d_arena = d_bt;
		m.arena_bytes = got;
	}
	pv.exchange_bytes = (size_t)(1ull << max_f) * p.T * 4;
	HIP_TRY(take((void**)&pv.d_pr[0], pv.exchange_bytes));
	HIP_TRY(take((void**)&pv.d_pr[1], pv.exchange_bytes));
	pv.spec_bytes = chunked ? ((size_t)n_spec + 1) * stride * 8 : 0;
	if (chunked) HIP_TRY(take((void**)&pv.spec_keys, pv.spec_bytes));
	DevProblem hdp{};
	hdp.n_cols = n; hdp.T = p.T; hdp.tbits = b.tbits; hdp.n_ind = p.n_ind;
	{
		const hipStream_t us = m.upload_stream;
		TableUploader up(m.device, us, pv.allocations);
		const size_t row_count = (size_t)end_col + SLOT_ROW_PAD;
		up.open_block(row_count * sizeof(SlotRow) + ctrl_words * 4 + (size_t)S * sizeof(SlotRun) + 4096);
		const SlotRun* d_runs = nullptr;
		HIP_TRY(up.up((void**)&hdp.slot_rows, m.splan.rows.data(), row_count * sizeof(SlotRow)));
		HIP_TRY(up.up((void**)&hdp.slot_ctrl, m.splan.ctrl.data(), ctrl_words * 4));
		HIP_TRY(up.up((void**)&d_runs, runs.data(), (size_t)S * sizeof(SlotRun)));
		HIP_TRY(up.alloc((void**)&hdp.slot_tab, tab_words * 4));
		HIP_TRY(up.flush());
		uint32_t most = 0;
		for (uint32_t k = 0; k < S; ++k) most = std::max<uint32_t>(most, ((runs[k].ncols + 8u) << (runs[k].g - runs[k].half)) + (runs[k].ncols + 8u) * ((runs[k].threads >> 6) + 64u));
		const uint32_t bx = std::max(1u, std::min(64u, (most + 255u) / 256u));
		for (uint32_t r0 = 0; r0 < S; r0 += 32768) hipLaunchKernelGGL(slot_tables, dim3(bx, std::min<uint32_t>(32768, S - r0)), dim3(256), 0, us, hdp, d_runs + r0, (uint32_t*)hdp.slot_tab);
		HIP_TRY(hipGetLastError());
		HIP_TRY(hipEventRecord(m.ev_upload, us));
		if (up.unstaged_copies || !up.stage.image || !up.stage.park()) {
			HIP_TRY(hipStreamSynchronize(us));
			up.stage.finish();
		}
	}
	b.laps.lap("preview: rows, control words, tables: allocations + copies");
	{
		const whamd_status_t opted = opt_in_large_lds(m.device, msg);
		if (opted != WHAMD_OK) return opted;
	}
	const hipStream_t rs = m.stream;
	m.inflight.run_stream = rs;
	m.own_stream_used = true;
	HIP_TRY(hipStreamWaitEvent(rs, m.ev_upload, 0));
	hdp.bt = (uint8_t*)m.d_arena;
	hdp.spec_keys = pv.spec_keys;
	hdp.spec_stride = stride;
	if (chunked) HIP_TRY(hipMemsetAsync(pv.spec_keys, 0xFF, pv.spec_bytes, rs));
	m.inflight.timing_pending = false;
	HIP_TRY(hipEventRecord(m.ev0, rs));
	m.use_chunks = chunked;
#ifdef WHAMD_DEBUG_BUILD
	m.ledger.clear();
#endif
	pv.runs.resize(S);
	uint64_t launches = 0;
	pv.launching = true;
	for (uint32_t k = 0; k < S; ++k) {
		SlotBatchEntry e{};
		e.run = runs[k];
		if (k == 0) e.run.has_prev = 0;
		e.run.rec_lo = (uint32_t)rec[k];
		e.run.rec_hi = (uint32_t)(rec[k] >> 32);
		e.run.spec_id = spec[k];
		e.prev = pv.d_pr[k & 1u];
		e.cur = pv.d_pr[(k & 1u) ^ 1u];
		pv.runs[k] = e.run;
		m.launch_slot_run(hdp, e, launches);
	}
	pv.launching = false;
	HIP_TRY(hipGetLastError());
	HIP_TRY(hipEventRecord(m.ev3, rs));
	pv.dp = hdp;
	pv.use_chunks = chunked;
	pv.why = PV_RAN;
	pv.pieces = pieces;
	pv.launched = S;
	pv.launches = launches;
	pv.pending = true;
	b.laps.lap("preview: launches submitted");
	return WHAMD_OK;
}

void DeviceTable::Impl::verify_preview() {
	Impl& m = *this;
	Preview& pv = m.preview;
	pv.agreed = 0;
	if (!pv.launched) return;
	const bool same_ground = m.use_slots && !m.windowed && m.jobs.size() == 1 && m.lanes.size() == 1 && m.dp.bt == pv.dp.bt && m.dp.spec_keys == pv.dp.spec_keys &&
	                         m.use_chunks == pv.use_chunks && (!m.use_chunks || m.dp.spec_stride == pv.dp.spec_stride) && !m.dp.dbg && !m.dp.dbg_flags &&
	                         m.d_pr[0] == pv.d_pr[0] && m.d_pr[1] == pv.d_pr[1] && !m.side_by_side;
	for (uint32_t k = 0; same_ground && k < pv.launched && k + 1 < m.schedule.size(); ++k) {
		const Impl::SuperStep& ss = m.schedule[k];
		if (ss.entry_count != 1 || !ss.singles.empty() || ss.ck_load >= 0 || ss.ck_save >= 0 || ss.bt_window >= 0) break;
		const SlotBatchEntry& e = m.slot_entries[ss.entry_off];
		if (std::memcmp(&e.run, &pv.runs[k], sizeof(SlotRun)) != 0 || e.prev != pv.d_pr[k & 1u] || e.cur != pv.d_pr[(k & 1u) ^ 1u] || e.score_out) break;
		++pv.agreed;
	}
	if (const char* at = debug_env("WHAMD_PREVIEW_MISMATCH_AT")) pv.agreed = std::min<uint32_t>(pv.agreed, (uint32_t)std::max(0, atoi(at)));
	if (getenv("WHAMD_DEBUG_TIMING"))
		fprintf(stderr, "[whamd timing] preview: %u plan pieces, %u steps launched, %u agree with the schedule\n", pv.pieces, pv.launched, pv.agreed);
}

whamd_status_t DeviceTable::upload(Problem& p, int device, std::string& msg, bool from_create) {
	Impl& m = *impl_;
	whamd_status_t st = m.open(device, msg);
	if (st != WHAMD_OK || p.n_cols == 0) return st;
	TableBuild b;
	b.n = p.n_cols;
	b.tbits = 2 * p.n_triples;
	b.ni = std::max<uint32_t>(p.n_ind, 1);
	m.dp.n_cols = b.n;
	m.dp.T = p.T;
	m.dp.tbits = b.tbits;
	m.dp.n_ind = p.n_ind;
	if ((st = m.choose_plan(p, b, msg)) != WHAMD_OK) return st;
	b.ped_slots = m.use_slots && m.splan.ped;
	b.laps.next_stage();
	if (debug_env("WHAMD_DEBUG_PLAN")) m.dump_plan(p);
	m.upload_stream = debug_env("WHAMD_UPLOAD_ON_TABLE_STREAM") ? nullptr : upload_stream_of(device);
	if (!m.upload_stream) m.upload_stream = m.stream;
	if (m.upload_stream == m.stream) m.own_stream_used = true;
	if ((st = m.start_preview(p, b, from_create, msg)) != WHAMD_OK) return st;
	if ((st = m.describe_columns(p, b, msg)) != WHAMD_OK) return st;
	if ((st = m.lay_out_arena(p, b, msg)) != WHAMD_OK) return st;
	TableUploader up(device, m.upload_stream, m.allocations);
	b.laps.lap("staging area taken");
	up.open_block(m.upload_bound(p, b));
	b.laps.lap("staging image sized, device block taken");
	if ((st = m.upload_column_arrays(p, b, up, msg)) != WHAMD_OK) return st;
	if ((st = m.upload_slot_arrays(b, up, msg)) != WHAMD_OK) return st;
	m.make_jobs();
	m.make_units(b);
	if ((st = m.make_windows(b, up, msg)) != WHAMD_OK) return st;
	if ((st = m.take_result_block(b.n, up, msg)) != WHAMD_OK) return st;
	if ((st = m.make_chunks(p, up, msg)) != WHAMD_OK) return st;
	if ((st = m.take_solve_buffers(p, b, up, msg)) != WHAMD_OK) return st;
	if ((st = m.make_lanes(b, up, msg)) != WHAMD_OK) return st;
	if ((st = m.make_schedule(b, msg)) != WHAMD_OK) return st;
	m.make_briefs();
	if ((st = m.upload_entries(up, msg)) != WHAMD_OK) return st;
	if ((st = m.launch_table_kernels(p, b, up, msg)) != WHAMD_OK) return st;
	b.laps.summary((double)b.bt / 1e9);
	if ((st = m.arm_debug_stamps(up, msg)) != WHAMD_OK) return st;
	if ((st = opt_in_large_lds(device, msg)) != WHAMD_OK) return st;
	if ((st = m.record_group_backtrace(b.n, up, msg)) != WHAMD_OK) return st;
	m.verify_preview();
	return WHAMD_OK;
}

namespace {

SegmentFn segment_kernel(bool stamps, bool sym) {
#ifdef WHAMD_DEBUG_BUILD
	if (stamps) return resident_segment<true, true>;
#endif
	return sym ? resident_segment<false, true> : resident_segment<false, false>;
}

PedSegmentFn ped_segment_kernel(bool stamps, bool spec) {
#ifdef WHAMD_DEBUG_BUILD
	if (stamps) return resident_segment_ped<true>;
#endif
	return spec ? resident_segment_ped<false, true> : resident_segment_ped<false>;
}

ResBatchFn resident_batch_kernel(bool sym) { return sym ? resident_batch<true> : resident_batch<false>; }

#ifdef WHAMD_DEBUG_BUILD
PedSlotRunFn pedslot_runx_kernel(uint32_t tb, uint32_t nf, uint32_t xc, bool spec) {
#define WHAMD_ROW(TB, NF) { pedslot_runx<TB, NF, 16, true>, pedslot_runx<TB, NF, 16, false>, pedslot_runx<TB, NF, 32, true>, pedslot_runx<TB, NF, 32, false> }
	static const PedSlotRunFn table[6][4] = {WHAMD_ROW(2, PSLOT_FACT), WHAMD_ROW(2, 16), WHAMD_ROW(2, 2), WHAMD_ROW(2, 4), WHAMD_ROW(4, 2), WHAMD_ROW(4, 4)};
#undef WHAMD_ROW
	const int row = tb == 2 ? (nf == (uint32_t)PSLOT_FACT ? 0 : nf == 16 ? 1 : nf == 2 ? 2 : 3) : (nf == 2 ? 4 : 5);
	return table[row][(xc == 16 ? 0 : 2) + (spec ? 0 : 1)];
}
#endif

PedSlotRunFn pedslot_run_kernel(uint32_t tb, uint32_t nf, bool spec, bool packed) {
#define WHAMD_ROW(TB, NF) { pedslot_run<TB, NF, true, true>, pedslot_run<TB, NF, true, false>, pedslot_run<TB, NF, false, true>, pedslot_run<TB, NF, false, false> }
	static const PedSlotRunFn table[7][4] = {WHAMD_ROW(2, PSLOT_FACT), WHAMD_ROW(4, PSLOT_FACT4), WHAMD_ROW(2, 16), WHAMD_ROW(2, 2), WHAMD_ROW(2, 4), WHAMD_ROW(4, 2), WHAMD_ROW(4, 4)};
#undef WHAMD_ROW
	const int row = tb == 2 && nf == (uint32_t)PSLOT_FACT ? 0 : tb == 4 && nf == (uint32_t)PSLOT_FACT4 ? 1 : tb == 2 ? (nf == 16 ? 2 : nf == 2 ? 3 : 4) : (nf == 2 ? 5 : 6);
	return table[row][(spec ? 0 : 2) + (packed ? 0 : 1)];
}

SlotRunXFn slot_runx_kernel(uint32_t xc, bool stamps, bool spec) {
#define WHAMD_PAIR(XC, STAMPS) { slot_runx<2, XC, STAMPS, true>, slot_runx<2, XC, STAMPS, false> }
#ifdef WHAMD_DEBUG_BUILD
	static const SlotRunXFn stamped[2][2] = {WHAMD_PAIR(24, true), WHAMD_PAIR(32, true)};
	if (stamps && xc) return stamped[xc == 24 ? 0 : 1][spec ? 0 : 1];
#endif
	static const SlotRunXFn table[5][2] = {WHAMD_PAIR(0, false), WHAMD_PAIR(8, false), WHAMD_PAIR(16, false), WHAMD_PAIR(24, false), WHAMD_PAIR(32, false)};
#undef WHAMD_PAIR
	return table[xc / 8][spec ? 0 : 1];
}

SlotRunFn slot_run_kernel(uint32_t lr, bool yform, bool stamps, bool spec) {
#ifdef WHAMD_DEBUG_BUILD
#define WHAMD_ROW(LR, YF) { slot_run<LR, true, true, YF>, slot_run<LR, true, false, YF>, slot_run<LR, false, true, YF>, slot_run<LR, false, false, YF> }
#else
#define WHAMD_ROW(LR, YF) { nullptr, nullptr, slot_run<LR, false, true, YF>, slot_run<LR, false, false, YF> }
#endif
	static const SlotRunFn table[5][4] = {WHAMD_ROW(3, true), WHAMD_ROW(3, false), WHAMD_ROW(1, false), WHAMD_ROW(2, true), WHAMD_ROW(2, false)};
#undef WHAMD_ROW
	const int row = lr == 3 ? (yform ? 0 : 1) : lr == 1 ? 2 : (yform ? 3 : 4);
	return table[row][(stamps ? 0 : 2) + (spec ? 0 : 1)];
}

SlotBatchFn slot_batch_kernel(int lr) {
	if (lr == 1) return slot_batch<1>;
	if (lr == 3) return slot_batch<3>;
	return slot_batch<2>;
}

GroupFn group_kernel(GroupVariant v, bool dbg, bool tight) {
	switch (v) {
		case GV_SINGLE4:
#ifdef WHAMD_DEBUG_BUILD
			if (dbg) return slot_group<2, true, false>;
#endif
			return tight ? slot_group<2, false, true> : slot_group<2, false, false>;
		case GV_PED_2_2: return pedslot_group<2, 2>;
		case GV_PED_2_4: return pedslot_group<2, 4>;
		case GV_PED_4_2: return pedslot_group<4, 2>;
		case GV_PED_4_4: return pedslot_group<4, 4>;
		case GV_PED_2_16: return pedslot_group<2, 16>;
		case GV_SINGLE8: return tight ? slot_group<3, false, true> : slot_group<3, false, false>;
		case GV_TRIO_FACT: return pedslot_group<2, PSLOT_FACT>;
		case GV_X4: return slot_groupx<2, false>;
		case GV_X8: return slot_groupx<3, false>;
		case GV_QUARTET_FACT: return pedslot_group<4, PSLOT_FACT4>;
		case GROUP_VARIANTS: break;
	}
	return nullptr;
}

}

whamd_status_t DeviceTable::solve(const Problem& p, Solution& s, whamd_solve_stats& st, std::string& msg) {
	whamd_status_t status = enqueue(p, s, msg);
	if (status != WHAMD_OK) return status;
	return wait(p, s, st, msg);
}

whamd_status_t DeviceTable::enqueue(const Problem& p, Solution& s, std::string& msg) {
	bool done = false;
	whamd_status_t status = WHAMD_OK;
	while (status == WHAMD_OK && !done) status = enqueue_some(p, s, ~0ull, done, msg);
	return status;
}

void DeviceTable::Impl::launch_column_step(const Problem& p, const Step& step, const Lane& lane, const uint32_t* prev, uint32_t* cur,
                                           uint64_t& launches) {
	Impl& m = *this;
	const hipStream_t rs = m.inflight.run_stream;
	DevProblem dp = m.dp;
	dp.keys = lane.d_keys;
	const uint32_t c = step.index;
	const DevColumn& d = m.cols[c];
#ifdef WHAMD_DEBUG_BUILD
	const auto column_facts = [&m](const Problem& pr, const DevColumn& col) { LaunchFacts f; f.T = (int32_t)pr.T; f.n_ind = (int32_t)m.dp.n_ind; f.mode = (int32_t)col.mode; f.wide = m.wide; return f; };
#endif
	if (d.mode == 0) {
		const uint32_t threads = 1u << d.f;
		const uint32_t block = std::min<uint32_t>(256, threads);
		hipLaunchKernelGGL(m.fused, dim3(threads / block), dim3(block), 0, rs, dp, c, prev, cur);
		WHAMD_NOTE(m, WHAMD_LAUNCH_COLUMN, (const void*)m.fused, dim3(threads / block), dim3(block), 0, rs, true, column_facts(p, d));
		launches += 1;
	} else {
		const uint64_t total = (1ull << (d.f + d.ebits - d.eloop)) * (m.wide ? p.T : 1u);
		const uint32_t block = (uint32_t)std::min<uint64_t>(256, (total + 63) / 64 * 64);
		if (m.wide) hipLaunchKernelGGL(column_step_wide, dim3((uint32_t)((total + block - 1) / block)), dim3(block), 0, rs, dp, c, prev, (uint32_t)total);
		else hipLaunchKernelGGL(m.keysfn, dim3((uint32_t)((total + block - 1) / block)), dim3(block), 0, rs, dp, c, prev, (uint32_t)total);
		WHAMD_NOTE(m, WHAMD_LAUNCH_COLUMN, m.wide ? (const void*)column_step_wide : (const void*)m.keysfn, dim3((uint32_t)((total + block - 1) / block)), dim3(block), 0, rs, true, column_facts(p, d));
		const uint32_t entries = (1u << d.f) * p.T;
// ... 613 lines not shown
		const uint32_t* c = m.h_pinned + 2 * (size_t)n + m.jobs.size();
		st.bt_chunks = (uint32_t)m.chunks.size();
		st.bt_missed = c[0];
		st.bt_rewalked = c[1];
		if (debug_env("WHAMD_BT_STATS")) fprintf(stderr, "[whamd backtrace] %zu chunks, %u guesses missed (%u of them only in the transmission value), %u units walked again (of %zu)\n", m.chunks.size(), c[0], c[2], c[1], m.units.size());
	}
	whamd_status_t reported = m.dp.dbg && m.use_slots ? m.report_slot_stamps(msg) : WHAMD_OK;
	if (reported == WHAMD_OK && m.dp.dbg && !m.plan.segments.empty()) reported = m.report_resident_stamps(msg);
	return reported;
}

#ifdef WHAMD_DEBUG_BUILD
namespace {

template <int T, int NIND>
const void* column_pair(bool keys) {
	FusedFn ff;
	KeysFn kf;
	pick<T, NIND>(ff, kf);
	return keys ? reinterpret_cast<const void*>(kf) : reinterpret_cast<const void*>(ff);
}

const std::vector<whamd_debug_kernel>& solve_kernels() {
#define K(...) {reinterpret_cast<const void*>((__VA_ARGS__)), #__VA_ARGS__, 0, 0}
#define D(...) {reinterpret_cast<const void*>((__VA_ARGS__)), #__VA_ARGS__, 0, 1}
#define WHAMD_COLUMN(T, NIND) {column_pair<T, NIND>(false), "column_step_fused<" #T ", " #NIND ">", 0, 0}, {column_pair<T, NIND>(true), "column_step_keys<" #T ", " #NIND ">", 0, 0}
#define WHAMD_PSLOT(TB, NF) K(pedslot_run<TB, NF, true, true>), K(pedslot_run<TB, NF, true, false>), K(pedslot_run<TB, NF, false, true>), K(pedslot_run<TB, NF, false, false>)
#define WHAMD_PSLOTX(TB, NF) D(pedslot_runx<TB, NF, 16, true>), D(pedslot_runx<TB, NF, 16, false>), D(pedslot_runx<TB, NF, 32, true>), D(pedslot_runx<TB, NF, 32, false>)
#define WHAMD_RUNX(XC) K(slot_runx<2, XC, false, true>), K(slot_runx<2, XC, false, false>)
#define WHAMD_RUN(LR, YF) K(slot_run<LR, false, true, YF>), K(slot_run<LR, false, false, YF>), D(slot_run<LR, true, true, YF>), D(slot_run<LR, true, false, YF>)
	static const std::vector<whamd_debug_kernel> table = [] {
		std::vector<whamd_debug_kernel> t = {
			WHAMD_COLUMN(1, 1), WHAMD_COLUMN(1, 2), WHAMD_COLUMN(1, 3), WHAMD_COLUMN(1, 4), WHAMD_COLUMN(1, 5), WHAMD_COLUMN(1, 6),
			WHAMD_COLUMN(4, 3), WHAMD_COLUMN(4, 4), WHAMD_COLUMN(4, 5), WHAMD_COLUMN(4, 6),
			WHAMD_COLUMN(16, 4), WHAMD_COLUMN(16, 5), WHAMD_COLUMN(16, 6),
			K(column_step_wide), K(column_finalize),
			K(ped_tables), K(resident_tables),
			K(resident_segment<false, false>), K(resident_segment<false, true>), D(resident_segment<true, true>),
			K(resident_segment_ped<false>), K(resident_segment_ped<false, true>), D(resident_segment_ped<true>),
			K(resident_batch<false>), K(resident_batch<true>),
			WHAMD_RUN(1, false), WHAMD_RUN(2, false), WHAMD_RUN(2, true), WHAMD_RUN(3, false), WHAMD_RUN(3, true),
			WHAMD_RUNX(0), WHAMD_RUNX(8), WHAMD_RUNX(16), WHAMD_RUNX(24), WHAMD_RUNX(32),
			D(slot_runx<2, 24, true, true>), D(slot_runx<2, 24, true, false>), D(slot_runx<2, 32, true, true>), D(slot_runx<2, 32, true, false>),
			K(slot_batch<1>), K(slot_batch<2>), K(slot_batch<3>),
			WHAMD_PSLOT(2, 2), WHAMD_PSLOT(2, 4), WHAMD_PSLOT(4, 2), WHAMD_PSLOT(4, 4), WHAMD_PSLOT(2, 16), WHAMD_PSLOT(2, PSLOT_FACT), WHAMD_PSLOT(4, PSLOT_FACT4),
			WHAMD_PSLOTX(2, 2), WHAMD_PSLOTX(2, 4), WHAMD_PSLOTX(4, 2), WHAMD_PSLOTX(4, 4), WHAMD_PSLOTX(2, 16), WHAMD_PSLOTX(2, PSLOT_FACT),
			K(slot_group<2, false, false>), K(slot_group<2, false, true>), K(slot_group<3, false, false>), K(slot_group<3, false, true>), D(slot_group<2, true, false>),
			K(slot_groupx<2, false>), K(slot_groupx<3, false>),
			K(pedslot_group<2, 2>), K(pedslot_group<2, 4>), K(pedslot_group<4, 2>), K(pedslot_group<4, 4>), K(pedslot_group<2, 16>),
			K(pedslot_group<2, PSLOT_FACT>), K(pedslot_group<4, PSLOT_FACT4>),
			K(backtrace_kernel), K(backtrace_chunks), K(backtrace_gather), K(superreads_single),
			K(backtrace_chunks_group), K(backtrace_gather_group), K(superreads_group),
		};
		size_t count = 0;
		const void* const* opted = large_lds_kernels(count);
		for (whamd_debug_kernel& k : t) k.large_lds_opted_in = std::find(opted, opted + count, k.kernel) != opted + count;
		return t;
	}();
#undef K
#undef D
#undef WHAMD_COLUMN
#undef WHAMD_PSLOT
#undef WHAMD_PSLOTX
#undef WHAMD_RUNX
#undef WHAMD_RUN
	return table;
}

}

size_t DeviceTable::debug_solve_kernels(whamd_debug_kernel* out, size_t capacity) {
	const std::vector<whamd_debug_kernel>& t = solve_kernels();
	for (size_t i = 0; out && i < t.size() && i < capacity; ++i) out[i] = t[i];
	return t.size();
}

size_t DeviceTable::debug_launches(whamd_debug_launch* out, size_t capacity) const {
	const std::vector<whamd_debug_launch>& ledger = impl_->ledger;
	for (size_t i = 0; out && i < ledger.size() && i < capacity; ++i) {
		out[i] = ledger[i];
		for (const whamd_debug_kernel& k : solve_kernels())
			if (k.kernel == ledger[i].kernel) { out[i].name = k.name; break; }
	}
	return ledger.size();
}

static const char* const* preview_why_lines() {
	static const char* const why[13] = {
		"", "no preview: switched off", "no preview: not inside whamd_dptable_create", "no preview: not a single-individual table on slot runs", "no preview: a debug switch changes the launches",
		"no preview: the table shares its launches", "no preview: the create is held to a thread budget", "no preview: more than one connected component", "no preview: too few plan pieces",
		"no preview: not alone", "no preview: the table does not begin with slot runs", "no preview: too close to the table's end", "no preview: the backtrace arena does not fit one window"};
	return why;
}

whamd_status_t DeviceTable::debug_preview_plan(Problem& p, uint32_t pieces, whamd_debug_preview_plan_result* out, uint64_t* rec_predicted, uint64_t* rec_laid_out,
                                               uint32_t* spec_predicted, uint32_t* spec_laid_out, size_t capacity, std::string& msg) {
	Impl m;
	TableBuild b;
	b.n = p.n_cols;
	b.tbits = 2 * p.n_triples;
	b.ni = std::max<uint32_t>(p.n_ind, 1);
	b.free_b = (size_t)1 << 40;
	if (p.T != 1 || p.n_cols == 0) { msg = "a single-individual table expected"; return WHAMD_ERR_UNSUPPORTED; }
	m.wide = !select_kernels(p.T, p.n_ind, m.fused, m.keysfn);
	m.use_slots = plan_forward_slots(p, std::max(8, m.slot_l), m.symmetry, m.splan, m.slot_lr);
	if (!m.use_slots) { msg = "the table is not planned on slot runs"; return WHAMD_ERR_UNSUPPORTED; }
	m.plan = ResidentPlan();
	m.plan.steps = m.splan.steps;
	m.plan.component_first_step = m.splan.component_first_step;
	m.plan.col_to_res.assign(p.n_cols, -1);
	m.preview.mode = 1;
	m.preview.pieces_wanted = pieces;
	Impl::PreviewPlan pp;
	m.plan_preview(p, b, true, pp);
	whamd_status_t st = m.describe_columns(p, b, msg);
	if (st == WHAMD_OK) st = m.lay_out_arena(p, b, msg);
	if (st != WHAMD_OK) return st;
	m.build_slot_blobs(b);
	m.lay_out_slot_tables(b, false);
	m.make_jobs();
	m.make_units(b);
	m.cut_chunks(p);
	static const char* const* why = preview_why_lines();
	*out = whamd_debug_preview_plan_result{};
	out->n_pieces = slot_plan_pieces(p.n_cols);
	out->pieces = pp.pieces;
	out->steps = pp.steps;
	out->n_steps = (uint32_t)m.plan.steps.size();
	out->why_not = why[pp.why < Impl::PV_WHYS ? pp.why : 0];
	out->chunked_predicted = pp.chunked; out->chunked = m.use_chunks;
	out->n_seeds_predicted = pp.n_spec; out->n_seeds = m.n_spec;
	out->stride_predicted = pp.stride; out->stride = m.use_chunks ? m.dp.spec_stride : 64u;
	out->arena_predicted = pp.arena; out->arena_laid_out = b.bt;
	out->windowed = m.windowed;
	out->exchange_predicted = (uint64_t)(1ull << pp.max_f) * p.T * 4; out->exchange_laid_out = b.exchange_bytes;
	for (uint32_t k = 0; k < pp.steps && k < capacity; ++k) {
		const SlotRun& run = m.splan.runs[m.plan.steps[k].index];
		if (rec_predicted) rec_predicted[k] = pp.rec[k];
		if (rec_laid_out) rec_laid_out[k] = ((uint64_t)run.rec_hi << 32) | run.rec_lo;
		if (spec_predicted) spec_predicted[k] = pp.spec[k];
		if (spec_laid_out) spec_laid_out[k] = run.spec_id;
	}
	return WHAMD_OK;
}

void DeviceTable::debug_preview(whamd_debug_preview* out) const {
	static const char* const* why = preview_why_lines();
	const Impl::Preview& pv = impl_->preview;
	out->ran = pv.why == Impl::PV_RAN;
	out->continued = pv.continued;
	out->pieces = pv.pieces;
	out->launched_steps = pv.launched;
	out->agreed_steps = pv.agreed;
	out->why_not = why[pv.why < Impl::PV_WHYS ? pv.why : 0];
}

void DeviceTable::Impl::note(uint32_t site, const void* kernel, dim3 grid, dim3 block, size_t lds, hipStream_t on, bool forward, const LaunchFacts& facts) {
	whamd_debug_launch rec = facts;
	rec.kernel = kernel;
	rec.site = site;
	rec.grid_x = grid.x; rec.grid_y = grid.y; rec.block = block.x;
	rec.lds = (uint32_t)lds;
	rec.own_stream = on == stream ? 1u : 0u;
	rec.forward = forward ? 1u : 0u;
	rec.preview = preview.launching ? 1 : 0;
	rec.reserved = 0;
	rec.count = 0;
	rec.name = nullptr;
	for (whamd_debug_launch& have : ledger)
		if (std::memcmp(&have, &rec, offsetof(whamd_debug_launch, count)) == 0) { have.count += 1; return; }
	rec.count = 1;
	ledger.push_back(rec);
}
#endif


}
```

whatshap_amd/csrc/slot_plan.cpp:

```cpp
#include <algorithm>
#include <cstdlib>
#include <cstring>
#include <chrono>
#include <iterator>
#include <cstdio>
#include <thread>

#include "debug_build.h"
#include "slots.h"
#include "genotype_plan.h"

namespace whamd {

namespace {

struct RunDraft {
	uint32_t c0 = 0, ncols = 0, g = 0, L = 0, lw = 0;
	std::vector<int32_t> entry_read;
	std::vector<int32_t> exit_read;
	bool symmetric = true;
};

inline uint32_t parity32(uint32_t v) { return (uint32_t)__builtin_popcount(v) & 1u; }

}

bool plan_forward_slots(const Problem& p, int l_pref, int use_symmetry, SlotPlan& plan, int lr, bool genotype_mode) {
	const auto tp0 = std::chrono::steady_clock::now();
	const long pf0 = thread_minor_faults();
	plan = SlotPlan();
	const uint32_t n = p.n_cols;
	const bool ped = p.T > 1 || genotype_mode;
	const uint32_t TB = p.T == 4 ? 2u : (p.T == 16 ? 4u : 0u);
	if (ped && !genotype_mode && (TB == 0 || p.n_ind < 3)) return false;
	if (genotype_mode && p.T != 1 && TB == 0) return false;
	if (!ped && !(p.T == 1 && p.n_ind == 1)) return false;
	if (!genotype_mode && !(p.value_bound < 1073741824.0)) return false;
	plan.ped = ped;
	const uint32_t fact_nf = (ped && !genotype_mode && !p.fterms.empty()) ? (TB == 2 && p.fterm_kind == 1 ? (uint32_t)PSLOT_FACT : (TB == 4 && p.fterm_kind == 2 ? (uint32_t)PSLOT_FACT4 : 0u)) : 0u;
	const bool fact = fact_nf != 0;
	lr = ped ? 0 : std::max(1, std::min(lr, SLOT_LR));
	const int n_lane = ped ? 6 - (int)TB : SLOT_LANE;
	plan.col_to_row.assign(n, -1);
	const int LMIN = lr + n_lane, LMAX = lr + n_lane + SLOT_LWMAX;
	if (ped) l_pref = l_pref < 0 ? -l_pref : LMAX;
	l_pref = std::max(LMIN, std::min(l_pref, LMAX));
	const uint32_t max_run_cols = ped ? (uint32_t)PSLOT_MAXCOLS : (uint32_t)SLOT_MAXCOLS;
	const std::vector<uint32_t>& last_col = p.read_last_col;
	std::vector<int32_t>& col_to_row = plan.col_to_row;
	if (ped) plan.prows.resize(n);
	else {
		plan.rows.reserve((size_t)n + SLOT_ROW_PAD);
		plan.rows.resize(n);
	}
	plan.bt_cols.resize(n);
	auto& rows_g = plan.rows;
	auto& prows_g = plan.prows;
	auto& btc_g = plan.bt_cols;
	auto plan_range = [&](const uint32_t c_begin, const uint32_t c_end, SlotPlan& plan, std::vector<RunDraft>& drafts) {
	std::vector<int8_t> slot_of(p.n_reads, -1);
	SlotRow scratch_row{};
	PedSlotRow scratch_prow{};
	uint32_t c = c_begin;
	while (c < c_end) {
		auto column_step = [&]() { plan.steps.push_back(Step{0, c}); ++c; };
		if (c + 1 >= n && !genotype_mode) { column_step(); continue; }
		const uint32_t b0 = p.b[c];
		const ColumnEntry* first = p.col_begin(c);
		constexpr uint32_t LOOK = 12;
		uint32_t kmax_at[LOOK], n_look = 0;
		for (uint32_t cc = c; cc < std::min(n, c + LOOK); ++cc) {
			if (cc > c && p.b[cc] == 0) break;
			kmax_at[n_look] = std::max<uint32_t>(n_look ? kmax_at[n_look - 1] : 0u, p.k[cc]);
			++n_look;
		}
		const uint32_t kmax = kmax_at[std::min<uint32_t>(n_look, genotype_mode ? 6u : LOOK) - 1];
		const uint32_t L = std::min<uint32_t>((uint32_t)l_pref, std::max<uint32_t>((uint32_t)LMIN, kmax));
		uint32_t g = kmax > L ? kmax - L : 0;
		if (genotype_mode) g = std::min(g, b0);
		std::vector<uint32_t> order(b0);
		for (uint32_t j = 0; j < b0; ++j) order[j] = j;
		std::stable_sort(order.begin(), order.end(), [&](uint32_t a, uint32_t bb) {
			const uint32_t ea = last_col[first[a].read_id], eb = last_col[first[bb].read_id];
			if (ea != eb) return ea > eb;
			return a > bb;
		});
		if (!genotype_mode) {
			auto probe = [&](uint32_t gg) -> uint32_t {
				uint32_t grid_end = 0xFFFFFFFFu;
				for (uint32_t i = 0; i < gg; ++i) grid_end = std::min(grid_end, last_col[first[order[i]].read_id]);
				uint32_t n_free = L - (b0 - gg), ends = 0, c1 = c;
				for (; c1 < n && c1 - c < max_run_cols; ++c1) {
					if (c1 + 1 == n || c1 >= grid_end || c1 >= c_end || (c1 > c && p.b[c1] == 0)) break;
					const uint32_t kc = p.k[c1], bc = c1 == c ? b0 : p.b[c1], n_new = kc - bc, n_end = kc - p.f[c1];
					if (n_end > (uint32_t)(ped ? PSLOT_MAXEND : SLOT_MAXEND) || ends + n_end > (uint32_t)SLOT_MAXENDS_RUN || n_new > n_free) break;
					n_free = n_free - n_new + n_end;
					ends += n_end;
				}
				return c1 - c;
			};
			uint32_t best_g = 0xFFFFFFFFu, best_len = 0, last_g = 0xFFFFFFFFu;
			for (uint32_t q = 0; q < n_look; ++q) {
				const uint32_t gg = kmax_at[q] > L ? kmax_at[q] - L : 0;
				if (gg == last_g) continue;
				last_g = gg;
				if (gg > b0 || gg > (uint32_t)SLOT_GMAX || p.k[c] > L + gg || b0 - gg > L) continue;
				const uint32_t len = probe(gg);
				if (len > best_len) { best_len = len; best_g = gg; }
			}
			if (best_g == 0xFFFFFFFFu) { column_step(); continue; }
			g = best_g;
		}
		if (g > b0 || g > (uint32_t)SLOT_GMAX || p.k[c] > L + g) { column_step(); continue; }
		if (genotype_mode) {
			while (g > 0 && c + 1 < n && last_col[first[order[g - 1]].read_id] <= c) --g;
			if (p.k[c] > L + g) { column_step(); continue; }
		}
		RunDraft d;
		d.c0 = c; d.g = g; d.L = L; d.lw = L - (uint32_t)LMIN;
		const uint32_t nslots = L + g;
		d.entry_read.assign(nslots, -1);
		uint32_t grid_end = 0xFFFFFFFFu;
		{
			std::vector<uint32_t> grid_reads;
			for (uint32_t i = 0; i < g; ++i) {
				grid_reads.push_back(first[order[i]].read_id);
				grid_end = std::min(grid_end, last_col[first[order[i]].read_id]);
			}
			std::stable_sort(grid_reads.begin(), grid_reads.end(), [&](uint32_t a, uint32_t bb) {
				if (last_col[a] != last_col[bb]) return last_col[a] < last_col[bb];
				return a < bb;
			});
			if (g >= 5) {
				d.entry_read[L + g - 1] = (int32_t)grid_reads[g - 1];
				for (uint32_t i = 0; i < 3; ++i) d.entry_read[L + i] = (int32_t)grid_reads[g - 4 + i];
				for (uint32_t i = 3; i + 1 < g; ++i) d.entry_read[L + i] = (int32_t)grid_reads[i - 3];
			} else {
				for (uint32_t i = 0; i < g; ++i) d.entry_read[L + i] = (int32_t)grid_reads[i];
			}
			uint32_t s = 0;
			for (uint32_t i = b0; i-- > g;) d.entry_read[s++] = (int32_t)first[order[i]].read_id;
		}
		std::vector<int32_t> cur = d.entry_read;
		auto release_marks = [&]() {
			for (int32_t r : d.entry_read) if (r >= 0) slot_of[r] = -1;
			for (int32_t r : cur) if (r >= 0) slot_of[r] = -1;
		};
		for (uint32_t s = 0; s < nslots; ++s) if (cur[s] >= 0) slot_of[cur[s]] = (int8_t)s;
		const size_t rows_mark = c, ends_mark = plan.end_slots.size(), starts_mark = plan.start_slots.size();
		std::vector<int32_t> started;
		uint32_t c1 = c, n_ends = 0;
		bool symmetric = true;
		uint32_t run_forms = 2;
		while (c1 < n && c1 - c < max_run_cols) {
			if (c1 + 1 == n && !genotype_mode) break;
			if (c1 >= grid_end && !(genotype_mode && c1 + 1 == n)) break;
			if (c1 >= c_end) break;
			if (c1 > c && p.b[c1] == 0) break;
			const ColumnEntry* col = p.col_begin(c1);
			const uint32_t kc = p.k[c1], bc = c1 == c ? b0 : p.b[c1];
			const uint32_t n_new = kc - bc, n_end = kc - p.f[c1];
			if (!genotype_mode && (n_end > (uint32_t)(ped ? PSLOT_MAXEND : SLOT_MAXEND) || n_ends + n_end > (uint32_t)SLOT_MAXENDS_RUN)) break;
			if (genotype_mode && n_ends + n_end > 250u) break;
			if (genotype_mode && c1 > c && run_lds_bytes(64u << d.lw, c1 - c + 1, p.T, 2u * p.P, 1u << p.P) > GS_MAX_LDS) break;
			uint32_t n_free = 0;
			for (uint32_t s = 0; s < L; ++s) n_free += cur[s] < 0;
			if (n_new > n_free) break;
			bool ok = true;
			if (!ped) {
				const int32_t* dcol = p.delta.data() + (size_t)p.col_ptr[c1];
				uint32_t bad = 0;
				for (uint32_t j = 0; j < kc; ++j) bad |= (uint32_t)(std::abs(dcol[j]) >= SLOT_DELTA_LIMIT);
				for (uint32_t j = 0; j < bc; ++j) bad |= (uint32_t)(slot_of[col[j].read_id] < 0);
				ok = bad == 0;
			}
			if (ped && !genotype_mode) {
				uint32_t most = 0;
				for (uint32_t t = 0; t < p.T; ++t) most = std::max<uint32_t>(most, (uint32_t)(p.term_end(c1, t) - p.term_begin(c1, t)));
				if (!fact && (most > (uint32_t)PSLOT_MAXFORMS || (most > 4u && TB != 2u))) {
					if (debug_env("WHAMD_DEBUG_PLAN")) fprintf(stderr, "[plan] column %u: %u cost forms per transmission value: no pedigree run\n", c1, most);
// ... 83 lines not shown
					if (en < 3) bc_rec.slot[25 + en] = (uint8_t)s; else bc_rec.pad[1] = (uint8_t)s;
				}
				plan.end_slots.push_back((uint8_t)s);
				++en;
			}
			if (!ok) break;
			row.n_end = en;
			prow.n_end = en;
			if (ped) bc_rec.pad[0] = (uint8_t)en;
			if (genotype_mode) {
				prow.pad[0] = n_new;
				prow.pad[1] = (uint32_t)(plan.start_slots.size() - starts_mark) - n_new;
			}
			for (uint32_t rest = ending_bits; rest; rest &= rest - 1u) cur[slot_of[col[__builtin_ctz(rest)].read_id]] = -1;
			n_ends += en;
			col_to_row[c1] = (int32_t)c1;
			btc_g[c1] = bc_rec;
			++c1;
		}
		{
			size_t keep = 0;
			for (size_t i = rows_mark; i < c1; ++i) keep += ped ? prows_g[i].n_end : rows_g[i].n_end;
			plan.end_slots.resize(ends_mark + keep);
			if (genotype_mode) {
				size_t keep_starts = 0;
				for (size_t i = rows_mark; i < c1; ++i) keep_starts += prows_g[i].pad[0];
				plan.start_slots.resize(starts_mark + keep_starts);
			}
		}
		if (c1 - c < (genotype_mode ? 1u : 2u)) {
			for (uint32_t cc = c; cc < c1; ++cc) col_to_row[cc] = -1;
			plan.end_slots.resize(ends_mark);
			plan.start_slots.resize(starts_mark);
			release_marks();
			for (int32_t r : started) slot_of[r] = -1;
			column_step();
			continue;
		}
		d.exit_read.assign(nslots, -1);
		{
			const ColumnEntry* col = p.col_begin(c1 - 1);
			for (uint32_t j = 0; j < p.k[c1 - 1]; ++j)
				if ((p.fwd_mask[c1 - 1] >> j) & 1u) d.exit_read[btc_g[c1 - 1].slot[j]] = (int32_t)col[j].read_id;
		}
		release_marks();
		for (int32_t r : started) slot_of[r] = -1;
		d.ncols = c1 - c;
		d.symmetric = symmetric;
		SlotRun run{};
		run.c0 = c; run.ncols = d.ncols; run.g = g; run.L = L; run.lw = d.lw;
		run.ctrl_off = (uint32_t)plan.ctrl.size();
		plan.ctrl.resize(plan.ctrl.size() + SLOT_CTRL_WORDS, 0);
		uint32_t exchanges = 0;
		for (uint32_t i = 0; i < d.ncols; ++i) {
			if (!ped) {
				SlotRow& xrow = rows_g[rows_mark + i];
				for (uint32_t k = 0; k < std::min<uint32_t>(xrow.n_end, SLOT_MAXEND); ++k) {
					if ((xrow.end[k].info & 31u) < (uint32_t)(lr + SLOT_LANE)) continue;
					if (exchanges & 1u) xrow.end[k].info |= 1u << 16;
					++exchanges;
				}
			}
			const uint32_t ne = ped ? prows_g[rows_mark + i].n_end : rows_g[rows_mark + i].n_end;
			const uint32_t s0 = ped ? prows_g[rows_mark + i].info0 : (rows_g[rows_mark + i].end[0].info & 31u);
			const uint32_t byte = std::min(ne, 3u) | ((ne ? (s0 & 31u) : 0u) << 2);
			if (ped) plan.ctrl[run.ctrl_off + (i >> 2)] |= byte << ((i & 3u) * 8u);
			else {
				const uint32_t qm = ne ? ((rows_g[rows_mark + i].end[0].info >> 8) & 255u) : 0u;
				const uint32_t xbuf = ne ? ((rows_g[rows_mark + i].end[0].info >> 16) & 1u) : 0u;
				plan.ctrl[run.ctrl_off + (i >> 1)] |= (byte | (qm << 7) | (xbuf << 15)) << ((i & 1u) * 16u);
			}
		}
		run.lr = (uint32_t)lr;
		run.row_off = (uint32_t)rows_mark;
		run.n_ends = 0;
		for (size_t i = rows_mark; i < c1; ++i) run.n_ends += ped ? prows_g[i].n_end : rows_g[i].n_end;
		if (ped) {
			PedSlotExtra ex{};
			ex.tb = TB;
			ex.nf = 2;
			for (uint32_t i = 0; i < d.ncols && !genotype_mode; ++i)
				for (uint32_t t = 0; t < p.T; ++t) {
					const uint32_t cnt = (uint32_t)(p.term_end(c + i, t) - p.term_begin(c + i, t));
					ex.nf = std::max(ex.nf, cnt > 4 ? 16u : (cnt > 2 ? 4u : 2u));
				}
			if (fact) ex.nf = fact_nf;
			if (fact_nf == (uint32_t)PSLOT_FACT4) { ex.pad[0] = p.fact4_roles[0]; ex.pad[1] = p.fact4_roles[1]; }
			ex.fwn = d.ncols * pslot_ta(ex.nf, p.T) * pslot_na(ex.nf);
			ex.arow = (ex.fwn + 3u) & ~3u;
			ex.rec_words = ((d.ncols + 3u) / 4u) * (64u << d.lw);
			plan.pextra.push_back(ex);
		}
		run.threads = 64u << d.lw;
		run.has_prev = c > 0;
		run.half = (use_symmetry > 0 && symmetric && g >= 1) ? 1u : 0u;
		for (uint32_t s = 0; s < nslots; ++s) {
			if (d.entry_read[s] >= 0) run.in_occ |= 1u << s;
			if (d.exit_read[s] >= 0) run.out_occ |= 1u << s;
		}
		plan.steps.push_back(Step{2, (uint32_t)plan.runs.size()});
		plan.runs.push_back(run);
		plan.end_off.push_back((uint32_t)ends_mark);
		plan.start_off.push_back((uint32_t)starts_mark);
		drafts.push_back(d);
		plan.n_run_columns += d.ncols;
		c = c1;
	}
	};
	std::vector<RunDraft> drafts;
	const auto tp1 = std::chrono::steady_clock::now();
	const long pf1 = thread_minor_faults();
	long pf2 = pf1;
	auto tp2 = tp1;
	{
		const uint32_t n_pieces = slot_plan_pieces(n);
		std::vector<SlotPlan> parts(n_pieces);
		std::vector<std::vector<RunDraft>> part_drafts(n_pieces);
		std::vector<uint32_t> bounds(n_pieces + 1);
		for (uint32_t t = 0; t <= n_pieces; ++t) bounds[t] = slot_plan_piece_begin(n, t);
		parallel_ranges(n_pieces, host_threads(n_pieces, 1), [&](uint64_t q0, uint64_t q1, uint32_t) {
			for (uint64_t q = q0; q < q1; ++q) plan_range(bounds[q], bounds[q + 1], parts[q], part_drafts[q]);
		});
		tp2 = std::chrono::steady_clock::now();
		pf2 = thread_minor_faults();
		const uint32_t n_threads = n_pieces;
		{
			size_t n_steps = 0, n_runs = 0, n_ends_all = 0, n_starts = 0, n_ctrl = 0, n_extra = 0;
			for (const SlotPlan& q : parts) {
				n_steps += q.steps.size(); n_runs += q.runs.size(); n_ends_all += q.end_slots.size(); n_starts += q.start_slots.size();
				n_ctrl += q.ctrl.size(); n_extra += q.pextra.size();
			}
			plan.steps.reserve(n_steps); plan.runs.reserve(n_runs); plan.end_off.reserve(n_runs); plan.start_off.reserve(n_runs);
			plan.end_slots.reserve(n_ends_all); plan.start_slots.reserve(n_starts); plan.ctrl.reserve(n_ctrl); plan.pextra.reserve(n_extra);
			drafts.reserve(n_runs);
		}
		for (uint32_t t = 0; t < n_threads; ++t) {
			const SlotPlan& q = parts[t];
			const uint32_t run_base = (uint32_t)plan.runs.size();
			const uint32_t end_base = (uint32_t)plan.end_slots.size(), ctrl_base = (uint32_t)plan.ctrl.size();
			for (Step st : q.steps) { if (st.kind == 2) st.index += run_base; plan.steps.push_back(st); }
			for (SlotRun run : q.runs) { run.ctrl_off += ctrl_base; plan.runs.push_back(run); }
			plan.pextra.insert(plan.pextra.end(), q.pextra.begin(), q.pextra.end());
			for (uint32_t off : q.end_off) plan.end_off.push_back(off + end_base);
			for (uint32_t off : q.start_off) plan.start_off.push_back(off + (uint32_t)plan.start_slots.size());
			plan.start_slots.insert(plan.start_slots.end(), q.start_slots.begin(), q.start_slots.end());
			plan.end_slots.insert(plan.end_slots.end(), q.end_slots.begin(), q.end_slots.end());
			plan.ctrl.insert(plan.ctrl.end(), q.ctrl.begin(), q.ctrl.end());
			plan.n_run_columns += q.n_run_columns;
			drafts.insert(drafts.end(), std::make_move_iterator(part_drafts[t].begin()), std::make_move_iterator(part_drafts[t].end()));
		}
	}
	const auto tp3 = std::chrono::steady_clock::now();
	const long pf3 = thread_minor_faults();
	for (size_t si = 0; si < plan.steps.size(); ++si) {
		const uint32_t c0 = plan.steps[si].kind == 2 ? plan.runs[plan.steps[si].index].c0 : plan.steps[si].index;
		if (!ped && (si == 0 || p.b[c0] == 0)) plan.component_first_step.push_back((uint32_t)si);
	}
	if (!ped && (lr == 2 || lr == 3) && !debug_env("WHAMD_NO_YFORM")) {
		std::vector<uint8_t> pure(n, 0);
		std::vector<uint64_t> B((size_t)n + 1, 0);
		parallel_ranges(n, host_threads(n, 8192), [&](uint64_t c_lo, uint64_t c_hi, uint32_t) {
			for (uint32_t c = (uint32_t)c_lo; c < (uint32_t)c_hi; ++c) {
				uint64_t kstar = 0;
				uint32_t Cp = RES_ABSENT, Cm = RES_ABSENT, Cc = INF;
				for (uint64_t q = p.term_begin(c, 0); q < p.term_end(c, 0); ++q) {
					const CostTerm& t = p.terms[q];
					if (t.plus) Cp = t.c; else if (t.minus) Cm = t.c; else Cc = std::min(Cc, t.c);
				}
				pure[c] = Cp != RES_ABSENT && Cm != RES_ABSENT && Cc == INF;
				if (pure[c]) {
					kstar = (uint64_t)(uint32_t)(Cp + Cm);
				} else {
					uint64_t dabs = 0, ub = ~0ull;
					const int32_t* dl = p.delta.data() + (size_t)p.col_ptr[c];
					for (uint32_t j = 0; j < p.k[c]; ++j) dabs += (uint64_t)std::abs((int64_t)dl[j]);
					for (uint64_t q = p.term_begin(c, 0); q < p.term_end(c, 0); ++q) {
						const CostTerm& t = p.terms[q];
						ub = std::min<uint64_t>(ub, (uint64_t)t.c + ((t.plus || t.minus) ? dabs : 0));
					}
					kstar = 2 * (ub == ~0ull ? 0 : ub);
				}
				B[c + 1] = kstar;
			}
		});
		for (uint32_t c = 0; c < n; ++c) B[c + 1] += B[c];
		if (B[n] < 0xFFFFFFF0ull) {
			std::vector<uint8_t> yrun(plan.runs.size(), 0);
			parallel_ranges(plan.runs.size(), host_threads(plan.runs.size(), 512), [&](uint64_t r_lo, uint64_t r_hi, uint32_t) {
				for (size_t ri = r_lo; ri < r_hi; ++ri) {
					const SlotRun& run = plan.runs[ri];
					bool ok = run.lr == 2 || run.lr == 3;
					for (uint32_t i = 0; i < run.ncols && ok; ++i) ok = pure[run.c0 + i];
					yrun[ri] = ok;
				}
			});
			parallel_ranges(plan.steps.size(), host_threads(plan.steps.size(), 256), [&](uint64_t s_lo, uint64_t s_hi, uint32_t) {
			for (size_t si = s_lo; si < s_hi; ++si) {
				if (plan.steps[si].kind != 2 || !yrun[plan.steps[si].index]) continue;
				SlotRun& run = plan.runs[plan.steps[si].index];
				auto y_neighbour = [&](size_t sj) { return plan.steps[sj].kind == 2 && yrun[plan.steps[sj].index]; };
				const bool in = si > 0 && p.b[run.c0] != 0 && y_neighbour(si - 1);
				bool out = false;
				if (si + 1 < plan.steps.size() && y_neighbour(si + 1)) out = p.b[plan.runs[plan.steps[si + 1].index].c0] != 0;
				run.yflags = 1u | (in ? 2u : 0u) | (out ? 4u : 0u);
				run.base_in = (uint32_t)B[run.c0];
				run.base_out = (uint32_t)B[run.c0 + run.ncols];
				for (uint32_t i = 0; i < run.ncols; ++i) {
					SlotRow& row = plan.rows[run.row_off + i];
					const uint32_t K = row.K, dreg[3] = {(uint32_t)row.dreg[0], (uint32_t)row.dreg[1], (uint32_t)row.dreg[2]};
					uint32_t* words = reinterpret_cast<uint32_t*>(&row);
					for (uint32_t r = 0; r < (1u << run.lr); ++r) {
						uint32_t dsum = 0;
						for (uint32_t sb = 0; sb < run.lr; ++sb) if ((r >> sb) & 1u) dsum += dreg[sb];
						words[r] = K - 2u * dsum + SLOT_YBIAS;
					}
				}
			}
			});
		}
	}
	if (ped && !genotype_mode) {
		if (plan.n_run_columns * 2 < n) return false;
		uint64_t words = 0;
		for (size_t ri = 0; ri < plan.runs.size(); ++ri) {
			const SlotRun& run = plan.runs[ri];
			PedSlotExtra& ex = plan.pextra[ri];
			ex.g_lo = (uint32_t)words;
			ex.g_hi = (uint32_t)(words >> 32);
			if (p.value_bound < (double)((1u << (31u - TB)) - 1u) && !debug_env("WHAMD_NO_PED_KEYS")) plan.runs[ri].yflags |= 16u;
			const uint64_t gsz = ((uint64_t)1 << run.g) * ex.fwn;
			ex.w_off = (uint32_t)gsz;
			ex.s_off = (uint32_t)(gsz + ((uint64_t)1 << run.lw) * ex.fwn);
			words += (uint64_t)ex.s_off + (uint64_t)run.ncols * 64u * pslot_ns(ex.nf) + (uint64_t)run.ncols * p.T * pslot_nk(ex.nf);
			if (run.ncols <= (uint32_t)SLOT_XCOLS && run.n_ends <= (uint32_t)SLOT_XENDS && ex.nf != (uint32_t)PSLOT_FACT4 && debug_env("WHAMD_PED_XRUN") && !debug_env("WHAMD_NO_XRUN")) {
				plan.runs[ri].yflags |= 8u;
				ex.x_off = (uint32_t)(words - (((uint64_t)ex.g_hi << 32) | ex.g_lo));
				words += (pslotx_words(run.ncols, run.threads, run.g) + 3u) & ~(uint64_t)3;
			}
		}
		if (debug_env("WHAMD_PED_XRUN")) words += 65536;
		plan.table_words = words;
	}
	plan.f_exit.assign(plan.runs.size(), 0);
	plan.exit_slot.assign(plan.runs.size(), std::vector<uint8_t>());
	parallel_ranges(plan.runs.size(), host_threads(plan.runs.size(), 512), [&](uint64_t r_begin, uint64_t r_end, uint32_t) {
	for (size_t ri = r_begin; ri < r_end; ++ri) {
		const SlotRun& run = plan.runs[ri];
		const uint32_t cl = run.c0 + run.ncols - 1;
		const SlotBtCol& bc = plan.bt_cols[run.row_off + run.ncols - 1];
		for (uint32_t j = 0; j < p.k[cl]; ++j)
			if ((p.fwd_mask[cl] >> j) & 1u) plan.exit_slot[ri].push_back(bc.slot[j]);
		plan.f_exit[ri] = (uint32_t)plan.exit_slot[ri].size();
	}
	});
	parallel_ranges(plan.steps.size(), host_threads(plan.steps.size(), 512), [&](uint64_t s_begin, uint64_t s_end, uint32_t) {
	for (size_t si = s_begin; si < s_end; ++si) {
		if (plan.steps[si].kind != 2) continue;
		const uint32_t ri = plan.steps[si].index;
		SlotRun& B = plan.runs[ri];
		const RunDraft& db = drafts[ri];
		const bool prev_is_run = si > 0 && plan.steps[si - 1].kind == 2 && B.has_prev;
		if (prev_is_run) {
		} else if (B.has_prev) {
			const ColumnEntry* first = p.col_begin(B.c0);
			std::memset(B.in_pos, 0, sizeof B.in_pos);
			for (uint32_t j = 0; j < p.b[B.c0]; ++j) {
				for (uint32_t s = 0; s < B.L + B.g; ++s)
					if (db.entry_read[s] == (int32_t)first[j].read_id) slot_set_pos(B.in_pos, s, j);
			}
			B.in_fullmask = p.b[B.c0] >= 32 ? 0xFFFFFFFFu : ((1u << p.b[B.c0]) - 1u);
		}
		const bool next_is_run = si + 1 < plan.steps.size() && plan.steps[si + 1].kind == 2 &&
		                         plan.runs[plan.steps[si + 1].index].has_prev;
		if (next_is_run) {
			SlotRun& C = plan.runs[plan.steps[si + 1].index];
			const RunDraft& dc = drafts[plan.steps[si + 1].index];
			const uint32_t nb = B.L + B.g, nc = C.L + C.g;
			std::vector<std::pair<uint32_t, uint32_t>> local_keys;
			std::vector<int> slot_in_b(nc, -1);
			for (uint32_t t = 0; t < nc; ++t) {
				if (dc.entry_read[t] < 0) continue;
				for (uint32_t s2 = 0; s2 < nb; ++s2) if (db.exit_read[s2] == dc.entry_read[t]) slot_in_b[t] = (int)s2;
			}
			for (uint32_t t = 0; t < C.L; ++t) {
				if (dc.entry_read[t] < 0) continue;
				const uint32_t s2 = (uint32_t)slot_in_b[t];
				uint32_t key = s2;
				if (s2 >= B.L) {
					const uint32_t gi = s2 - B.L;
					key = (B.g >= 5 && gi + 1 == B.g) ? 3000u : ((B.g >= 5 && gi < 3) ? 2000u + gi : 1000u + gi);
				}
				local_keys.push_back({key, t});
			}
			std::sort(local_keys.begin(), local_keys.end());
			const uint32_t n_loc = (uint32_t)local_keys.size();
			std::memset(C.in_pos, 0, sizeof C.in_pos);
			for (uint32_t i = 0; i < n_loc; ++i) slot_set_pos(C.in_pos, local_keys[i].second, i);
			for (uint32_t i = 0; i < C.g; ++i) slot_set_pos(C.in_pos, C.L + i, n_loc + i);
			C.in_identity = 1;
			for (uint32_t t = 0; t < nc; ++t) if (dc.entry_read[t] >= 0 && slot_pos(C.in_pos, t) != t) C.in_identity = 0;
			C.in_fullmask = (n_loc + C.g) >= 32 ? 0xFFFFFFFFu : ((1u << (n_loc + C.g)) - 1u);
			for (uint32_t t = 0; t < nc; ++t) if (slot_in_b[t] >= 0) slot_set_pos(B.out_pos, (uint32_t)slot_in_b[t], slot_pos(C.in_pos, t));
			B.out_fullmask = C.in_fullmask;
			if (B.half) {
				C.in_half = 1;
				C.in_mirror_pos = slot_pos(B.out_pos, B.L + B.g - 1);
			}
		} else {
			for (uint32_t j = 0; j < plan.f_exit[ri]; ++j) slot_set_pos(B.out_pos, plan.exit_slot[ri][j], j);
			B.out_fullmask = plan.f_exit[ri] >= 32 ? 0xFFFFFFFFu : ((1u << plan.f_exit[ri]) - 1u);
			B.mirror_out = B.half;
		}
	}
	});
	if (getenv("WHAMD_DEBUG_TIMING")) {
		auto ms = [](std::chrono::steady_clock::time_point a, std::chrono::steady_clock::time_point b) { return std::chrono::duration<double, std::milli>(b - a).count(); };
		fprintf(stderr, "[whamd timing] slot plan: setup %.1f ms, column ranges %.1f ms, concatenation %.1f ms, layouts %.1f ms (page faults of this thread: %ld, %ld, %ld, %ld)\n",
		        ms(tp0, tp1), ms(tp1, tp2), ms(tp2, tp3), ms(tp3, std::chrono::steady_clock::now()), pf1 - pf0, pf2 - pf1, pf3 - pf2, thread_minor_faults() - pf3);
	}
	return true;
}

}
```

whatshap_amd/csrc/slots.h:

```cpp
#pragma once
#include <cstdint>
#include <memory>
#include <string>
#include <utility>
#include <vector>

#include "problem.h"
#include "host_parallel.h"
#include "resident.h"

namespace whamd {

constexpr int SLOT_LR = 3;
constexpr int SLOT_LANE = 6;
constexpr int SLOT_LWMAX = 3;
constexpr int SLOT_GMAX = 12;
constexpr int SLOT_MAXSLOTS = 26;
constexpr int SLOT_MAXCOLS = 64;
constexpr int SLOT_MAXEND = 8;
constexpr int PSLOT_MAXEND = 4;
constexpr int SLOT_MAXENDS_RUN = 96;
constexpr int32_t SLOT_DELTA_LIMIT = 1 << 22;

struct SlotRow {
	uint32_t K;
	uint32_t Cc;
	int32_t dreg[SLOT_LR];
	int32_t dlane[SLOT_LANE];
	uint32_t n_end;
	struct End {
		uint32_t info;
		uint32_t M;
	} end[SLOT_MAXEND];
	uint32_t pad2[4];
	int32_t dslot[SLOT_MAXSLOTS];
	uint32_t Cp;
	uint32_t pad3[5];
};
static_assert(SLOT_LR == 3 && SLOT_LANE == 6 && SLOT_MAXEND == 8, "hot layout of SlotRow: 2 + 3 + 6 + 1 + 4 dwords in the first line, six more ending reads in the second");
static_assert(sizeof(SlotRow) == 256, "SlotRow must stay 64 dwords");
constexpr int SLOT_CTRL_WORDS = 32;
constexpr uint32_t SLOT_YBIAS = 0x80000000u;
constexpr int SLOT_XCOLS = 32;
constexpr int SLOT_XENDS = 32;
constexpr int SLOT_XPAD = 8;
constexpr int SLOT_ROW_PAD = 64;

struct SlotRun {
	uint32_t c0, ncols, g, L;
	uint32_t lw, half, has_prev, row_off;
	uint32_t n_ends, rec_lo, rec_hi, threads;
	uint32_t in_occ, in_identity, in_half, in_mirror_pos;
	uint32_t in_fullmask, out_occ, mirror_out, out_fullmask;
	uint32_t spec_id, lr, ctrl_off, pad;
	uint32_t in_pos[8];
	uint32_t out_pos[8];
	uint32_t tab_g, tab_w, tab_sl, tab_kr;
	uint32_t yflags, base_in, base_out, tab_par;
};
inline size_t slot_run_lds_bytes(uint32_t threads, uint32_t lr, uint32_t ncols) {
	return (size_t)2 * threads * ((size_t)1 << lr) * 4 + (size_t)(ncols + 8) * 64 + 8 * 64 * 4 + (size_t)(ncols + 8) * 64 * 4;
}
inline size_t slotx_lds_bytes(uint32_t threads, uint32_t ncols) { return (size_t)(2 + (ncols + 3) / 4 + 3) * threads * 16; }
inline uint32_t slot_pos(const uint32_t (&w)[8], uint32_t s) { return (w[s >> 2] >> ((s & 3u) * 8u)) & 255u; }
inline void slot_set_pos(uint32_t (&w)[8], uint32_t s, uint32_t pos) {
	w[s >> 2] = (w[s >> 2] & ~(255u << ((s & 3u) * 8u))) | (pos << ((s & 3u) * 8u));
}
static_assert(sizeof(SlotRun) == 192, "SlotRun layout");

constexpr int PSLOT_MAXCOLS = 32;
constexpr int PSLOT_MAXFORMS = 16;
constexpr int PSLOT_FORMWORDS = 1024;
constexpr int PSLOT_FACT = 1;
constexpr uint32_t PSLOT_NK = 12;
constexpr int PSLOT_FACT4 = 3;
constexpr uint32_t PSLOT_NK4 = 16;
constexpr uint32_t PSLOT_FSTRIDE4 = 20;
constexpr bool pslot_is_fact(uint32_t nf) { return nf == (uint32_t)PSLOT_FACT || nf == (uint32_t)PSLOT_FACT4; }
constexpr uint32_t pslot_na(uint32_t nf) { return pslot_is_fact(nf) ? 4u : nf; }
constexpr uint32_t pslot_ns(uint32_t nf) { return pslot_is_fact(nf) ? 4u : nf; }
constexpr uint32_t pslot_nk(uint32_t nf) { return nf == (uint32_t)PSLOT_FACT ? PSLOT_NK : (nf == (uint32_t)PSLOT_FACT4 ? 1u : 0u); }
constexpr uint32_t pslot_ta(uint32_t nf, uint32_t T) { return nf == (uint32_t)PSLOT_FACT4 ? 1u : T; }
#if defined(__HIPCC__)
#define WHAMD_HD __host__ __device__
#else
#define WHAMD_HD
#endif
WHAMD_HD inline uint32_t pslot_min2(uint32_t a, uint32_t b) { return a < b ? a : b; }
WHAMD_HD inline uint32_t pslot_fact4_cost(uint32_t LX, uint32_t LY, uint32_t L1, uint32_t L2, const uint32_t (&k)[16], bool u1, bool v1, bool same_u, bool same_v) {
	constexpr uint32_t BIG = 0x40000000u;
	const uint32_t mo01 = k[1] + LX, mo10 = k[2] - LX, fa01 = k[5] + LY, fa10 = k[6] - LY;
	const uint32_t c1[2][2] = {{k[8], k[9] + L1}, {k[10] - L1, k[11]}}, c2[2][2] = {{k[12], k[13] + L2}, {k[14] - L2, k[15]}};
	const uint32_t m01 = u1 ? mo10 : mo01, m10 = u1 ? mo01 : mo10;
	const uint32_t f01 = v1 ? fa10 : fa01, f10 = v1 ? fa01 : fa10;
	const uint32_t F0 = pslot_min2(k[4], f01), F1 = pslot_min2(f10, k[7]);
	const uint32_t fs00 = same_v ? F0 : k[4], fs01 = same_v ? BIG : f01, fs10 = same_v ? BIG : f10, fs11 = same_v ? F1 : k[7];
	uint32_t H[2][2];
	for (int q = 0; q < 2; ++q) {
		const uint32_t z0 = pslot_min2(fs00 + c2[q][0], fs01 + c2[q][1]), z1 = pslot_min2(fs10 + c2[q][0], fs11 + c2[q][1]);
		for (int p = 0; p < 2; ++p) H[p][q] = pslot_min2(c1[p][0] + z0, c1[p][1] + z1);
	}
	const uint32_t h01 = same_u ? H[0][0] : H[0][1], h10 = same_u ? H[1][1] : H[1][0];
	return pslot_min2(pslot_min2(k[0] + H[0][0], k[3] + H[1][1]), pslot_min2(m01 + h01, m10 + h10));
}
struct PedSlotRow {
	uint32_t recomb;
	uint32_t M0;
	uint32_t info1, M1, info2, M2;
	uint32_t n_end, info0;
	int32_t dslot[SLOT_MAXSLOTS];
	uint8_t ind[SLOT_MAXSLOTS + 2];
	uint32_t pad[7];
};
static_assert(sizeof(PedSlotRow) == 192, "PedSlotRow must stay 48 words");
struct PedSlotExtra {
	uint32_t tb, nf, fwn, arow;
	uint32_t g_lo, g_hi, w_off, s_off;
	uint32_t rec_words, x_off, pad[2];
};
constexpr uint64_t pslotx_words(uint32_t ncols, uint32_t threads, uint32_t g) { return (uint64_t)2 * (ncols + SLOT_XPAD) + threads + ((uint64_t)1 << g); }
static_assert(sizeof(PedSlotExtra) == 48, "PedSlotExtra layout");
inline size_t pedslot_lds_bytes(uint32_t threads, uint32_t ncols, const PedSlotExtra& ex) {
	return ((size_t)2 * threads + (PSLOT_MAXCOLS + 4) * 8 + (size_t)(threads >> 6) * (ex.arow + (4u << ex.tb) * pslot_na(ex.nf)) + (size_t)(ncols + 4) * 64 * pslot_ns(ex.nf) +
	        ((size_t)(ncols + 4) << ex.tb) * pslot_nk(ex.nf)) * 4;
}

struct SlotBatchEntry {
	SlotRun run;
	PedSlotExtra ex;
	const uint32_t* prev;
	uint32_t* cur;
	uint32_t* score_out;
	uint64_t pad;
	const uint32_t* tab;
	const void* rows;
	const uint32_t* ctrl;
	uint8_t* bt;
	unsigned long long* spec_keys;
	uint32_t spec_stride, pad2;
};
static_assert(sizeof(SlotBatchEntry) == 320 && sizeof(SlotBatchEntry) % 64 == 0, "entries are fetched with wide scalar loads, whole 64-byte lines");

constexpr int SLOT_GROUP_MAX = 248;
struct SlotGroupArgs {
	uint32_t n, pad;
	const SlotBatchEntry* entry[SLOT_GROUP_MAX];
};

struct SlotBtCol {
	uint8_t k, kf, pad[2];
	uint8_t slot[28];
};
static_assert(sizeof(SlotBtCol) == 32, "SlotBtCol must stay 8 dwords");

struct SlotBtUnit {
	uint32_t kind, c0, ncols, blob_off;
	uint32_t g, L, n_ends, threads;
	uint32_t bt_lo, bt_hi, half, blob_words;
	uint32_t f_exit, lr, pad0[2];
	uint8_t exit_slot[32];
	uint8_t exit_pos[32];
};
static_assert(sizeof(SlotBtUnit) == 128, "SlotBtUnit must stay 32 words");

template <class T>
using NoInitAllocator = NoInitAlloc<T>;

struct SlotPlan {
	std::vector<Step> steps;
	std::vector<SlotRun> runs;
	std::vector<SlotRow, NoInitAllocator<SlotRow>> rows;
	std::vector<SlotBtCol, NoInitAllocator<SlotBtCol>> bt_cols;
	std::vector<uint8_t> end_slots;
	std::vector<uint32_t> end_off;
	std::vector<uint32_t> f_exit;
	std::vector<std::vector<uint8_t>> exit_slot;
	std::vector<uint32_t> ctrl;
	std::vector<int32_t> col_to_row;
	std::vector<uint32_t> component_first_step;
	uint64_t n_run_columns = 0;
	bool ped = false;
	std::vector<uint8_t> start_slots;
	std::vector<uint32_t> start_off;
	std::vector<PedSlotRow, NoInitAllocator<PedSlotRow>> prows;
	std::vector<PedSlotExtra> pextra;
	uint64_t table_words = 0;
};

constexpr uint32_t PLAN_PIECE = 8192;
inline uint32_t slot_plan_pieces(uint32_t n_cols) { return n_cols / PLAN_PIECE > 1 ? n_cols / PLAN_PIECE : 1; }
inline uint32_t slot_plan_piece_begin(uint32_t n_cols, uint32_t piece) { return (uint32_t)((uint64_t)n_cols * piece / slot_plan_pieces(n_cols)); }

bool plan_forward_slots(const Problem& p, int l_pref, int use_symmetry, SlotPlan& plan, int lr = 2, bool genotype_mode = false);

bool emulate_slot_plan(const Problem& p, const SlotPlan& plan, std::vector<uint32_t>& path_index, uint32_t& score, std::string& msg);
bool emulate_pedslot_plan(const Problem& p, const SlotPlan& plan, std::vector<uint32_t>& path_index, std::vector<uint32_t>& path_trans,
                          uint32_t& score, std::string& msg);
uint32_t pedslot_table_entry(const Problem& p, const SlotPlan& plan, uint32_t run_index, int kind, uint32_t unit, uint32_t c, uint32_t t, uint32_t f);

}
```

Baseline: 2.313 million variant-columns/s.

## Start the preview launch from the slot planner's head hook

The slot planner now finishes the Y-form row rewrite, exit slots and layout linking for the leading steps first. It then calls a hook that adopts the steps and starts the device preview on those head runs, and only afterwards finishes the remaining steps. The aim is to overlap host planning of the tail with GPU work on the head instead of waiting for the whole plan. The upload stream is now set up before choose_plan so the hook can launch, and timing laps and a debug entry point are added. Risks include the preview reading plan state that is later mutated, and extra complexity in the create path.

```diff
diff --git a/include/whatshap_amd_debug.h b/include/whatshap_amd_debug.h
--- a/include/whatshap_amd_debug.h
+++ b/include/whatshap_amd_debug.h
@@ -92,7 +92,7 @@
 
 typedef struct whamd_debug_preview {
 	int32_t ran, continued;
-	uint32_t pieces, launched_steps, agreed_steps, reserved;
+	uint32_t pieces, launched_steps, agreed_steps, from_hook;
 	const char* why_not;
 } whamd_debug_preview;
 whamd_status_t whamd_debug_dptable_preview(const whamd_dptable* table, whamd_debug_preview* out);
@@ -108,6 +108,16 @@
                                         const whamd_pedigree_view* pedigree, int distrust_genotypes,
                                         const uint32_t* positions, size_t n_positions, uint32_t pieces, whamd_debug_preview_plan_result* out,
                                         uint64_t* rec_predicted, uint64_t* rec_laid_out, uint32_t* spec_predicted, uint32_t* spec_laid_out, size_t capacity);
+
+typedef struct whamd_debug_head_plan_result {
+	uint32_t n_pieces, head_steps, n_steps, hook_calls;
+	uint64_t digest, head_digest_in_hook, head_digest;
+	uint32_t edge_yflags[2];
+	uint32_t n_runs, n_components;
+} whamd_debug_head_plan_result;
+whamd_status_t whamd_debug_head_first_plan(const whamd_readset_view* readset, const uint32_t* recombcost, size_t n_recombcost,
+                                           const whamd_pedigree_view* pedigree, int distrust_genotypes,
+                                           const uint32_t* positions, size_t n_positions, uint32_t head_pieces, whamd_debug_head_plan_result* out);
 
 typedef struct whamd_debug_genotype_run {
 	uint32_t c0, ncols;
diff --git a/whatshap_amd/_native.py b/whatshap_amd/_native.py
--- a/whatshap_amd/_native.py
+++ b/whatshap_amd/_native.py
@@ -760,7 +760,7 @@
 
 class DebugPreview(C.Structure):
     _fields_ = [("ran", C.c_int32), ("continued", C.c_int32), ("pieces", C.c_uint32), ("launched_steps", C.c_uint32), ("agreed_steps", C.c_uint32),
-                ("reserved", C.c_uint32), ("why_not", C.c_char_p)]
+                ("from_hook", C.c_uint32), ("why_not", C.c_char_p)]
 
 
 def debug_preview(table) -> dict:
@@ -770,7 +770,24 @@
     out = DebugPreview()
     _check(D.whamd_debug_dptable_preview(table._h, C.byref(out)), D)
     return {"ran": bool(out.ran), "continued": bool(out.continued), "pieces": int(out.pieces), "launched_steps": int(out.launched_steps),
-            "agreed_steps": int(out.agreed_steps), "why_not": (out.why_not or b"").decode()}
+            "agreed_steps": int(out.agreed_steps), "from_hook": bool(out.from_hook), "why_not": (out.why_not or b"").decode()}
+
+
+class DebugHeadPlan(C.Structure):
+    _fields_ = [("n_pieces", C.c_uint32), ("head_steps", C.c_uint32), ("n_steps", C.c_uint32), ("hook_calls", C.c_uint32),
+                ("digest", C.c_uint64), ("head_digest_in_hook", C.c_uint64), ("head_digest", C.c_uint64),
+                ("edge_yflags", C.c_uint32 * 2), ("n_runs", C.c_uint32), ("n_components", C.c_uint32)]
+
+
+def debug_head_first_plan(problem: ProblemArrays, head_pieces: int = 0) -> dict:
+    D = debug_lib()
+    fn = D.whamd_debug_head_first_plan
+    fn.restype = C.c_int
+    out = DebugHeadPlan()
+    _check(fn(*problem.call_args(), C.c_uint32(head_pieces), C.byref(out)), D)
+    rec = {name: int(getattr(out, name)) for name, _ in DebugHeadPlan._fields_ if name != "edge_yflags"}
+    rec["edge_yflags"] = tuple(None if v == 0xFFFFFFFF else int(v) for v in out.edge_yflags)
+    return rec
 
 
 class DebugPreviewPlan(C.Structure):
diff --git a/whatshap_amd/csrc/c_api.cpp b/whatshap_amd/csrc/c_api.cpp
--- a/whatshap_amd/csrc/c_api.cpp
+++ b/whatshap_amd/csrc/c_api.cpp
@@ -784,6 +784,73 @@
 	});
 }
 
+whamd_status_t whamd_debug_head_first_plan(const whamd_readset_view* readset, const uint32_t* recombcost, size_t n_recombcost,
+                                           const whamd_pedigree_view* pedigree, int distrust_genotypes,
+                                           const uint32_t* positions, size_t n_positions, uint32_t head_pieces, whamd_debug_head_plan_result* out) {
+	return guarded([&]() -> whamd_status_t {
+	if (!out) return fail(WHAMD_ERR_INVALID, "out is NULL");
+	Problem p;
+	std::string msg;
+	whamd_status_t st = build_problem(readset, recombcost, n_recombcost, pedigree, distrust_genotypes != 0, positions, n_positions, p, msg);
+	if (st != WHAMD_OK) return fail(st, msg);
+	if (p.T != 1) return fail(WHAMD_ERR_UNSUPPORTED, "the head hook applies to a single individual only");
+	*out = whamd_debug_head_plan_result{};
+	auto mix = [](uint64_t& h, const void* data, size_t bytes) {
+		const unsigned char* b = static_cast<const unsigned char*>(data);
+		for (size_t i = 0; i < bytes; ++i) h = (h ^ b[i]) * 1099511628211ull;
+	};
+	auto runs_digest = [&mix](const SlotPlan& sp, size_t n_runs) {
+		uint64_t h = 1469598103934665603ull;
+		for (size_t ri = 0; ri < n_runs; ++ri) {
+			const SlotRun& run = sp.runs[ri];
+			mix(h, &run, sizeof run);
+			mix(h, sp.rows.data() + run.row_off, (size_t)run.ncols * sizeof(SlotRow));
+			mix(h, sp.bt_cols.data() + run.row_off, (size_t)run.ncols * sizeof(SlotBtCol));
+			mix(h, sp.ctrl.data() + run.ctrl_off, (size_t)SLOT_CTRL_WORDS * 4);
+			mix(h, sp.end_slots.data() + sp.end_off[ri], run.n_ends);
+		}
+		return h;
+	};
+	SlotPlan sp;
+	SlotPlanHead head;
+	const uint32_t n_pieces = slot_plan_pieces(p.n_cols);
+	head.col_limit = slot_plan_piece_begin(p.n_cols, std::min(head_pieces, n_pieces));
+	uint32_t calls = 0, head_steps = 0;
+	uint64_t in_hook = 0;
+	head.at_head = [&](uint32_t n_head) {
+		++calls;
+		head_steps = n_head;
+		in_hook = runs_digest(sp, n_head);
+	};
+	if (!plan_forward_slots(p, 11, 1, sp, 2, false, head_pieces ? &head : nullptr)) return fail(WHAMD_ERR_UNSUPPORTED, "the table is not eligible for slot runs");
+	out->n_pieces = n_pieces;
+	out->head_steps = head_steps;
+	out->n_steps = (uint32_t)sp.steps.size();
+	out->hook_calls = calls;
+	out->head_digest_in_hook = in_hook;
+	out->head_digest = runs_digest(sp, head_steps);
+	out->n_runs = (uint32_t)sp.runs.size();
+	out->n_components = (uint32_t)sp.component_first_step.size();
+	uint64_t h = runs_digest(sp, sp.runs.size());
+	mix(h, sp.steps.data(), sp.steps.size() * sizeof(Step));
+	mix(h, sp.end_off.data(), sp.end_off.size() * 4);
+	mix(h, sp.start_slots.data(), sp.start_slots.size());
+	mix(h, sp.start_off.data(), sp.start_off.size() * 4);
+	mix(h, sp.f_exit.data(), sp.f_exit.size() * 4);
+	for (const std::vector<uint8_t>& e : sp.exit_slot) mix(h, e.data(), e.size());
+	mix(h, sp.col_to_row.data(), sp.col_to_row.size() * 4);
+	mix(h, sp.component_first_step.data(), sp.component_first_step.size() * 4);
+	mix(h, &sp.n_run_columns, sizeof sp.n_run_columns);
+	out->digest = h;
+	out->edge_yflags[0] = out->edge_yflags[1] = 0xFFFFFFFFu;
+	if (head_steps) {
+		out->edge_yflags[0] = sp.runs[head_steps - 1].yflags;
+		if (head_steps < sp.steps.size() && sp.steps[head_steps].kind == 2) out->edge_yflags[1] = sp.runs[sp.steps[head_steps].index].yflags;
+	}
+	return WHAMD_OK;
+	});
+}
+
 whamd_status_t whamd_debug_genotype_run_plan(const whamd_readset_view* readset, const uint32_t* recombcost, size_t n_recombcost,
                                              const whamd_pedigree_view* pedigree, const uint32_t* positions, size_t n_positions,
                                              whamd_debug_genotype_run* out, size_t capacity, size_t* n_out, double* min_total_out) {
diff --git a/whatshap_amd/csrc/dp_device.hip b/whatshap_amd/csrc/dp_device.hip
--- a/whatshap_amd/csrc/dp_device.hip
+++ b/whatshap_amd/csrc/dp_device.hip
@@ -81,7 +81,9 @@
 struct CreateLaps {
 	using Clock = std::chrono::steady_clock;
 	const bool on = getenv("WHAMD_DEBUG_TIMING") != nullptr;
-	Clock::time_point last = Clock::now();
+	const Clock::time_point origin = Clock::now();
+	Clock::time_point last = origin;
+	double since_origin_ms() const { return std::chrono::duration<double, std::milli>(Clock::now() - origin).count(); }
 	double stage_ms[4] = {0.0, 0.0, 0.0, 0.0};
 	int stage = 0;
 	double take() {
@@ -335,7 +337,7 @@
 	BtJob* d_window_jobs = nullptr;
 
 	whamd_status_t open(int dev, std::string& msg);
-	whamd_status_t choose_plan(Problem& p, TableBuild& b, std::string& msg);
+	whamd_status_t choose_plan(Problem& p, TableBuild& b, bool from_create, std::string& msg);
 	void dump_plan(const Problem& p) const;
 	whamd_status_t describe_columns(const Problem& p, TableBuild& b, std::string& msg);
 	whamd_status_t lay_out_arena(const Problem& p, TableBuild& b, std::string& msg);
@@ -406,6 +408,8 @@
 		uint32_t launched = 0;
 		uint32_t agreed = 0;
 		bool launching = false;
+		bool tried = false;
+		bool from_hook = false;
 		bool pending = false;
 		bool continued = false;
 		bool use_chunks = false;
@@ -573,14 +577,19 @@
 	return WHAMD_OK;
 }
 
-whamd_status_t DeviceTable::Impl::choose_plan(Problem& p, TableBuild& b, std::string& msg) {
-	Impl& m = *this;
+static uint32_t preview_pieces_of(uint32_t wanted, uint32_t n_pieces) { return wanted ? wanted : std::max(1u, n_pieces / 6); }
+
+whamd_status_t DeviceTable::Impl::choose_plan(Problem& p, TableBuild& b, bool from_create, std::string& msg) {
+	Impl& m = *this;
+	m.preview.tried = false;
+	m.preview.from_hook = false;
 	m.wide = !select_kernels(p.T, p.n_ind, m.fused, m.keysfn);
 	if (m.wide && (p.T > (uint32_t)MAX_T_WIDE || p.n_ind > (uint32_t)MAX_IND_WIDE)) {
 		msg = "no device kernel for T=" + std::to_string(p.T) + ", individuals=" + std::to_string(p.n_ind);
 		return WHAMD_ERR_UNSUPPORTED;
 	}
 	for (uint32_t c = 0; c < p.n_cols && !m.wide; ++c) m.wide = p.term_end(c, p.T - 1) - p.term_begin(c, 0) > (uint64_t)COL_MAXTERMS;
+	b.laps.lap("plan: kernels chosen, term counts scanned");
 	b.force_keys = m.path == "column_keys" || m.wide;
 	const bool want_resident = (m.path == "auto" || m.path == "resident") && !m.wide;
 	size_t free_b = 0, total_b = 0;
@@ -596,11 +605,45 @@
 	}
 	free_b += arena_idle_bytes(m.device);
 	b.free_b = free_b;
+	b.laps.lap("plan: free device memory asked");
 	int slot_lr = m.slot_lr, slot_l = m.slot_l;
 	if (m.shared_hint && p.T == 1 && p.max_k >= 18 && !m.slot_l_set && m.slot_lr == 2) { slot_lr = 3; slot_l = 12; }
 	if (p.T == 1 && p.max_k >= 21 && p.max_k <= 22 && !m.slot_l_set && m.slot_lr == 2 && !debug_env("WHAMD_NO_WIDE_LAYOUT")) { slot_lr = 3; slot_l = 12; }
 	m.slot_lr_used = slot_lr;
-	m.use_slots = (m.path == "auto" || m.path == "slots") && !m.wide && plan_forward_slots(p, p.T > 1 ? (m.slot_l_set ? -m.slot_l : 0) : std::max(8, slot_l), m.symmetry, m.splan, slot_lr);
+	whamd_status_t head_status = WHAMD_OK;
+	bool steps_adopted = false;
+	auto adopt_steps = [&]() {
+		m.plan = ResidentPlan();
+		m.plan.steps = m.splan.steps;
+		m.plan.component_first_step = m.splan.component_first_step;
+		m.plan.col_to_res.assign(p.n_cols, -1);
+		steps_adopted = true;
+	};
+	SlotPlanHead head;
+	{
+		const uint32_t n_pieces = slot_plan_pieces(p.n_cols);
+		const uint32_t pieces = std::min(n_pieces - 1, preview_pieces_of(m.preview.pieces_wanted, n_pieces));
+		head.col_limit = slot_plan_piece_begin(p.n_cols, pieces);
+		head.at_head = [&](uint32_t n_head) {
+			if (n_head == 0) return;
+			m.use_slots = true;
+			m.table_bytes = 0;
+			adopt_steps();
+			b.laps.lap("plan: the planner up to the head's callback");
+			m.preview.tried = true;
+			m.preview.from_hook = true;
+			head_status = m.start_preview(p, b, from_create, msg);
+			if (m.preview.why != PV_RAN) m.preview.from_hook = false;
+		};
+	}
+	bool head_first = from_create && p.T == 1 && m.preview.mode != 0 && slot_plan_pieces(p.n_cols) >= 2 && !m.shared_hint && !m.side_by_side && !debug_env("WHAMD_NO_PREVIEW") &&
+	                  !debug_env("WHAMD_NO_HEAD_FIRST");
+	if (head_first && m.preview.mode < 0)
+		head_first = !m.preview.thread_budget && slot_plan_pieces(p.n_cols) >= 8 && m.device >= 0 && m.device < 64 && Impl::tables_on_device[m.device].load() == 1;
+	m.use_slots = (m.path == "auto" || m.path == "slots") && !m.wide &&
+	              plan_forward_slots(p, p.T > 1 ? (m.slot_l_set ? -m.slot_l : 0) : std::max(8, slot_l), m.symmetry, m.splan, slot_lr, false, head_first ? &head : nullptr);
+	if (head_status != WHAMD_OK) return head_status;
+	b.laps.lap("plan: the planner");
 	if (m.use_slots && m.splan.ped && m.splan.table_words * 4ull > free_b / 4) m.use_slots = false;
 	m.table_bytes = m.use_slots && m.splan.ped ? m.splan.table_words * 4ull : 0ull;
 	if (p.lazy_terms) {
@@ -610,16 +653,14 @@
 		if (st != WHAMD_OK) return st;
 	}
 	if (m.use_slots) {
-		m.plan = ResidentPlan();
-		m.plan.steps = m.splan.steps;
-		m.plan.component_first_step = m.splan.component_first_step;
-		m.plan.col_to_res.assign(p.n_cols, -1);
+		if (!steps_adopted) adopt_steps();
 	} else {
 		m.splan = SlotPlan();
 		plan_forward(p, want_resident, m.l_pref, m.fold, m.plan, m.symmetry);
 	}
 	m.device_superreads = p.n_ind == 1 && p.T == 1 && p.P == 2 && !p.distrust && p.h2p.size() >= 2 && p.h2p[0] == 0 && p.h2p[1] == 1 && p.genotype.size() >= p.n_cols &&
 	                      !debug_env("WHAMD_HOST_SUPERREADS");
+	b.laps.lap("plan: steps adopted, lazy terms");
 	return WHAMD_OK;
 }
 
@@ -1538,7 +1579,7 @@
 		if (n_pieces < 8) return none(PV_FEW_PIECES);
 		if (m.device < 0 || m.device >= 64 || Impl::tables_on_device[m.device].load() != 1) return none(PV_NOT_ALONE);
 	}
-	out.pieces = std::min(n_pieces - 1, pv.pieces_wanted ? pv.pieces_wanted : std::max(1u, n_pieces / 6));
+	out.pieces = std::min(n_pieces - 1, preview_pieces_of(pv.pieces_wanted, n_pieces));
 	const uint32_t col_limit = slot_plan_piece_begin(n, out.pieces);
 	const std::vector<Step>& steps = m.plan.steps;
 	const std::vector<SlotRun>& runs = m.splan.runs;
@@ -1667,6 +1708,9 @@
 	pv.runs.resize(S);
 	uint64_t launches = 0;
 	pv.launching = true;
+	if (b.laps.on)
+		fprintf(stderr, "[whamd timing] preview: first launch %.2f ms after the create's upload began, at t = %.2f ms (%s)\n", b.laps.since_origin_ms(), timing_stamp_ms(),
+		        pv.from_hook ? "from the planner's head hook" : "behind the plan");
 	for (uint32_t k = 0; k < S; ++k) {
 		SlotBatchEntry e{};
 		e.run = runs[k];
@@ -1725,14 +1769,14 @@
 	m.dp.T = p.T;
 	m.dp.tbits = b.tbits;
 	m.dp.n_ind = p.n_ind;
-	if ((st = m.choose_plan(p, b, msg)) != WHAMD_OK) return st;
+	m.upload_stream = debug_env("WHAMD_UPLOAD_ON_TABLE_STREAM") ? nullptr : upload_stream_of(device);
+	if (!m.upload_stream) m.upload_stream = m.stream;
+	if (m.upload_stream == m.stream) m.own_stream_used = true;
+	if ((st = m.choose_plan(p, b, from_create, msg)) != WHAMD_OK) return st;
 	b.ped_slots = m.use_slots && m.splan.ped;
 	b.laps.next_stage();
 	if (debug_env("WHAMD_DEBUG_PLAN")) m.dump_plan(p);
-	m.upload_stream = debug_env("WHAMD_UPLOAD_ON_TABLE_STREAM") ? nullptr : upload_stream_of(device);
-	if (!m.upload_stream) m.upload_stream = m.stream;
-	if (m.upload_stream == m.stream) m.own_stream_used = true;
-	if ((st = m.start_preview(p, b, from_create, msg)) != WHAMD_OK) return st;
+	if (!m.preview.tried && (st = m.start_preview(p, b, from_create, msg)) != WHAMD_OK) return st;
 	if ((st = m.describe_columns(p, b, msg)) != WHAMD_OK) return st;
 	if ((st = m.lay_out_arena(p, b, msg)) != WHAMD_OK) return st;
 	TableUploader up(device, m.upload_stream, m.allocations);
@@ -2652,6 +2696,7 @@
 	out->pieces = pv.pieces;
 	out->launched_steps = pv.launched;
 	out->agreed_steps = pv.agreed;
+	out->from_hook = pv.why == Impl::PV_RAN && pv.from_hook ? 1u : 0u;
 	out->why_not = why[pv.why < Impl::PV_WHYS ? pv.why : 0];
 }
 
diff --git a/whatshap_amd/csrc/slot_plan.cpp b/whatshap_amd/csrc/slot_plan.cpp
--- a/whatshap_amd/csrc/slot_plan.cpp
+++ b/whatshap_amd/csrc/slot_plan.cpp
@@ -25,7 +25,7 @@
 
 }
 
-bool plan_forward_slots(const Problem& p, int l_pref, int use_symmetry, SlotPlan& plan, int lr, bool genotype_mode) {
+bool plan_forward_slots(const Problem& p, int l_pref, int use_symmetry, SlotPlan& plan, int lr, bool genotype_mode, const SlotPlanHead* head) {
 	const auto tp0 = std::chrono::steady_clock::now();
 	const long pf0 = thread_minor_faults();
 	plan = SlotPlan();
@@ -415,13 +415,31 @@
 	}
 	const auto tp3 = std::chrono::steady_clock::now();
 	const long pf3 = thread_minor_faults();
-	for (size_t si = 0; si < plan.steps.size(); ++si) {
+	const bool timing = getenv("WHAMD_DEBUG_TIMING") != nullptr;
+	const double concatenated_at = timing ? timing_stamp_ms() : 0.0;
+	double lap_ms[7] = {0, 0, 0, 0, 0, 0, 0};
+	auto lap_from = tp3;
+	auto lap = [&](int which) {
+		if (!timing) return;
+		const auto now = std::chrono::steady_clock::now();
+		lap_ms[which] += std::chrono::duration<double, std::milli>(now - lap_from).count();
+		lap_from = now;
+	};
+	const size_t n_steps = plan.steps.size();
+	for (size_t si = 0; si < n_steps; ++si) {
 		const uint32_t c0 = plan.steps[si].kind == 2 ? plan.runs[plan.steps[si].index].c0 : plan.steps[si].index;
 		if (!ped && (si == 0 || p.b[c0] == 0)) plan.component_first_step.push_back((uint32_t)si);
 	}
+	lap(0);
+	const bool head_first = head && head->at_head && !ped && !genotype_mode;
+	size_t n_head = 0;
+	if (head_first)
+		while (n_head < n_steps && plan.steps[n_head].kind == 2 && plan.steps[n_head].index == n_head && plan.runs[n_head].c0 + plan.runs[n_head].ncols <= head->col_limit) ++n_head;
+	std::vector<uint64_t> B;
+	std::vector<uint8_t> yrun;
 	if (!ped && (lr == 2 || lr == 3) && !debug_env("WHAMD_NO_YFORM")) {
 		std::vector<uint8_t> pure(n, 0);
-		std::vector<uint64_t> B((size_t)n + 1, 0);
+		B.assign((size_t)n + 1, 0);
 		parallel_ranges(n, host_threads(n, 8192), [&](uint64_t c_lo, uint64_t c_hi, uint32_t) {
 			for (uint32_t c = (uint32_t)c_lo; c < (uint32_t)c_hi; ++c) {
 				uint64_t kstar = 0;
@@ -447,8 +465,9 @@
 			}
 		});
 		for (uint32_t c = 0; c < n; ++c) B[c + 1] += B[c];
+		lap(1);
 		if (B[n] < 0xFFFFFFF0ull) {
-			std::vector<uint8_t> yrun(plan.runs.size(), 0);
+			yrun.assign(plan.runs.size(), 0);
 			parallel_ranges(plan.runs.size(), host_threads(plan.runs.size(), 512), [&](uint64_t r_lo, uint64_t r_hi, uint32_t) {
 				for (size_t ri = r_lo; ri < r_hi; ++ri) {
 					const SlotRun& run = plan.runs[ri];
@@ -457,31 +476,35 @@
 					yrun[ri] = ok;
 				}
 			});
-			parallel_ranges(plan.steps.size(), host_threads(plan.steps.size(), 256), [&](uint64_t s_lo, uint64_t s_hi, uint32_t) {
-			for (size_t si = s_lo; si < s_hi; ++si) {
-				if (plan.steps[si].kind != 2 || !yrun[plan.steps[si].index]) continue;
-				SlotRun& run = plan.runs[plan.steps[si].index];
-				auto y_neighbour = [&](size_t sj) { return plan.steps[sj].kind == 2 && yrun[plan.steps[sj].index]; };
-				const bool in = si > 0 && p.b[run.c0] != 0 && y_neighbour(si - 1);
-				bool out = false;
-				if (si + 1 < plan.steps.size() && y_neighbour(si + 1)) out = p.b[plan.runs[plan.steps[si + 1].index].c0] != 0;
-				run.yflags = 1u | (in ? 2u : 0u) | (out ? 4u : 0u);
-				run.base_in = (uint32_t)B[run.c0];
-				run.base_out = (uint32_t)B[run.c0 + run.ncols];
-				for (uint32_t i = 0; i < run.ncols; ++i) {
-					SlotRow& row = plan.rows[run.row_off + i];
-					const uint32_t K = row.K, dreg[3] = {(uint32_t)row.dreg[0], (uint32_t)row.dreg[1], (uint32_t)row.dreg[2]};
-					uint32_t* words = reinterpret_cast<uint32_t*>(&row);
-					for (uint32_t r = 0; r < (1u << run.lr); ++r) {
-						uint32_t dsum = 0;
-						for (uint32_t sb = 0; sb < run.lr; ++sb) if ((r >> sb) & 1u) dsum += dreg[sb];
-						words[r] = K - 2u * dsum + SLOT_YBIAS;
-					}
-				}
-			}
-			});
-		}
-	}
+		}
+		lap(2);
+	}
+	auto rewrite_rows = [&](const size_t s_first, const size_t s_last) {
+		if (yrun.empty()) return;
+		parallel_ranges(s_last - s_first, host_threads(s_last - s_first, 256), [&](uint64_t s_lo, uint64_t s_hi, uint32_t) {
+		for (size_t si = s_first + s_lo; si < s_first + s_hi; ++si) {
+			if (plan.steps[si].kind != 2 || !yrun[plan.steps[si].index]) continue;
+			SlotRun& run = plan.runs[plan.steps[si].index];
+			auto y_neighbour = [&](size_t sj) { return plan.steps[sj].kind == 2 && yrun[plan.steps[sj].index]; };
+			const bool in = si > 0 && p.b[run.c0] != 0 && y_neighbour(si - 1);
+			bool out = false;
+			if (si + 1 < n_steps && y_neighbour(si + 1)) out = p.b[plan.runs[plan.steps[si + 1].index].c0] != 0;
+			run.yflags = 1u | (in ? 2u : 0u) | (out ? 4u : 0u);
+			run.base_in = (uint32_t)B[run.c0];
+			run.base_out = (uint32_t)B[run.c0 + run.ncols];
+			for (uint32_t i = 0; i < run.ncols; ++i) {
+				SlotRow& row = plan.rows[run.row_off + i];
+				const uint32_t K = row.K, dreg[3] = {(uint32_t)row.dreg[0], (uint32_t)row.dreg[1], (uint32_t)row.dreg[2]};
+				uint32_t* words = reinterpret_cast<uint32_t*>(&row);
+				for (uint32_t r = 0; r < (1u << run.lr); ++r) {
+					uint32_t dsum = 0;
+					for (uint32_t sb = 0; sb < run.lr; ++sb) if ((r >> sb) & 1u) dsum += dreg[sb];
+					words[r] = K - 2u * dsum + SLOT_YBIAS;
+				}
+			}
+		}
+		});
+	};
 	if (ped && !genotype_mode) {
 		if (plan.n_run_columns * 2 < n) return false;
 		uint64_t words = 0;
@@ -506,8 +529,11 @@
 	}
 	plan.f_exit.assign(plan.runs.size(), 0);
 	plan.exit_slot.assign(plan.runs.size(), std::vector<uint8_t>());
-	parallel_ranges(plan.runs.size(), host_threads(plan.runs.size(), 512), [&](uint64_t r_begin, uint64_t r_end, uint32_t) {
-	for (size_t ri = r_begin; ri < r_end; ++ri) {
+	auto exit_slots = [&](const size_t s_first, const size_t s_last) {
+	parallel_ranges(s_last - s_first, host_threads(s_last - s_first, 512), [&](uint64_t s_begin, uint64_t s_end, uint32_t) {
+	for (size_t si = s_first + s_begin; si < s_first + s_end; ++si) {
+		if (plan.steps[si].kind != 2) continue;
+		const size_t ri = plan.steps[si].index;
 		const SlotRun& run = plan.runs[ri];
 		const uint32_t cl = run.c0 + run.ncols - 1;
 		const SlotBtCol& bc = plan.bt_cols[run.row_off + run.ncols - 1];
@@ -516,8 +542,10 @@
 		plan.f_exit[ri] = (uint32_t)plan.exit_slot[ri].size();
 	}
 	});
-	parallel_ranges(plan.steps.size(), host_threads(plan.steps.size(), 512), [&](uint64_t s_begin, uint64_t s_end, uint32_t) {
-	for (size_t si = s_begin; si < s_end; ++si) {
+	};
+	auto link_layouts = [&](const size_t s_first, const size_t s_last) {
+	parallel_ranges(s_last - s_first, host_threads(s_last - s_first, 512), [&](uint64_t s_begin, uint64_t s_end, uint32_t) {
+	for (size_t si = s_first + s_begin; si < s_first + s_end; ++si) {
 		if (plan.steps[si].kind != 2) continue;
 		const uint32_t ri = plan.steps[si].index;
 		SlotRun& B = plan.runs[ri];
@@ -576,10 +604,35 @@
 		}
 	}
 	});
-	if (getenv("WHAMD_DEBUG_TIMING")) {
+	};
+	auto finish_steps = [&](const size_t s_first, const size_t s_last) {
+		rewrite_rows(s_first, s_last);
+		lap(3);
+		exit_slots(s_first, s_last);
+		lap(4);
+		link_layouts(s_first, s_last);
+		lap(5);
+	};
+	double head_done_at = 0.0;
+	if (head_first) {
+		finish_steps(0, n_head);
+		head_done_at = timing ? timing_stamp_ms() : 0.0;
+		head->at_head((uint32_t)n_head);
+		lap(6);
+		finish_steps(n_head, n_steps);
+	} else {
+		finish_steps(0, n_steps);
+	}
+	if (timing) {
 		auto ms = [](std::chrono::steady_clock::time_point a, std::chrono::steady_clock::time_point b) { return std::chrono::duration<double, std::milli>(b - a).count(); };
+		const double inside = head_first ? lap_ms[6] : 0.0;
 		fprintf(stderr, "[whamd timing] slot plan: setup %.1f ms, column ranges %.1f ms, concatenation %.1f ms, layouts %.1f ms (page faults of this thread: %ld, %ld, %ld, %ld)\n",
-		        ms(tp0, tp1), ms(tp1, tp2), ms(tp2, tp3), ms(tp3, std::chrono::steady_clock::now()), pf1 - pf0, pf2 - pf1, pf3 - pf2, thread_minor_faults() - pf3);
+		        ms(tp0, tp1), ms(tp1, tp2), ms(tp2, tp3), ms(tp3, std::chrono::steady_clock::now()) - inside, pf1 - pf0, pf2 - pf1, pf3 - pf2, thread_minor_faults() - pf3);
+		fprintf(stderr, "[whamd timing] slot plan layouts: component list %.2f ms, Y form per column + prefix sum %.2f ms, runs in Y form %.2f ms, rows rewritten %.2f ms, exit slots %.2f ms, "
+		        "entry / exit layouts %.2f ms; concatenation done at t = %.2f ms\n", lap_ms[0], lap_ms[1], lap_ms[2], lap_ms[3], lap_ms[4], lap_ms[5], concatenated_at);
+		if (head_first)
+			fprintf(stderr, "[whamd timing] slot plan head: %zu of %zu steps finished %.2f ms behind the concatenation, %.2f ms inside the callback\n", n_head, n_steps,
+			        head_done_at - concatenated_at, inside);
 	}
 	return true;
 }
diff --git a/whatshap_amd/csrc/slots.h b/whatshap_amd/csrc/slots.h
--- a/whatshap_amd/csrc/slots.h
+++ b/whatshap_amd/csrc/slots.h
@@ -1,5 +1,8 @@
 #pragma once
+#include <chrono>
+#include <cmath>
 #include <cstdint>
+#include <functional>
 #include <memory>
 #include <string>
 #include <utility>
@@ -191,7 +194,12 @@
 inline uint32_t slot_plan_pieces(uint32_t n_cols) { return n_cols / PLAN_PIECE > 1 ? n_cols / PLAN_PIECE : 1; }
 inline uint32_t slot_plan_piece_begin(uint32_t n_cols, uint32_t piece) { return (uint32_t)((uint64_t)n_cols * piece / slot_plan_pieces(n_cols)); }
 
-bool plan_forward_slots(const Problem& p, int l_pref, int use_symmetry, SlotPlan& plan, int lr = 2, bool genotype_mode = false);
+struct SlotPlanHead {
+	uint32_t col_limit = 0;
+	std::function<void(uint32_t)> at_head;
+};
+bool plan_forward_slots(const Problem& p, int l_pref, int use_symmetry, SlotPlan& plan, int lr = 2, bool genotype_mode = false, const SlotPlanHead* head = nullptr);
+inline double timing_stamp_ms() { return std::fmod(std::chrono::duration<double, std::milli>(std::chrono::steady_clock::now().time_since_epoch()).count(), 1e6); }
 
 bool emulate_slot_plan(const Problem& p, const SlotPlan& plan, std::vector<uint32_t>& path_index, uint32_t& score, std::string& msg);
 bool emulate_pedslot_plan(const Problem& p, const SlotPlan& plan, std::vector<uint32_t>& path_index, std::vector<uint32_t>& path_trans,
```

Result: faster. 2.357 million variant-columns/s, median of 6 (+1.9%).
